# DavidLBick/espnet-1

Hardware: AMD Instinct MI355X
Metric: utterances/sec + step-time, Conformer-L T=1000 batch=32 @1/2/4/8 GPU (higher is better)
Workload: dtype bf16; 1 GPU; C3 Conformer-L (12x512, 8 heads, ff 2048, cnn 31) + 6-layer Transformer decoder, hybrid CTC/att 0.3/0.7, lsm 0.1, V=5000, T=1000 frames x 80, L=40, dropout 0.1, Adam+WarmupLR+clip 5; global_batch=32, seq_len=1000, parallelism=dp1

## Files before the change

espnet-1_amd/csrc/gemm_grouped.hip:

```cpp
#include "gemm_kern.h"

namespace {
struct GroupProbD {
  const bf16* A;
  const bf16* B;
  float* C;
  int lda, ldb, ldc;
  int M, N, K;
  int tiles_n, tile0;
  float beta;
};
constexpr int EA_GROUP_CHUNK = 60;
struct GroupChunk {
  int first, n;
  GroupProbD pr[EA_GROUP_CHUNK];
};
static_assert(sizeof(GroupChunk) <= 4000, "kernel argument space");

__global__ void group_upload(GroupChunk c, GroupProbD* table, int* map) {
  for (int i = threadIdx.x; i < c.n; i += blockDim.x) table[c.first + i] = c.pr[i];
  for (int i = 0; i < c.n; ++i) {
    const GroupProbD& d = c.pr[i];
    const int nt = ea_cdiv(d.M, 256) * d.tiles_n;
    for (int t = threadIdx.x; t < nt; t += blockDim.x) map[d.tile0 + t] = c.first + i;
  }
}

template <bool AK, bool BKM, int NS = 4>
__global__ __launch_bounds__(512, 1) void gemm_grouped(const GroupProbD* __restrict__ table,
                                                       const int* __restrict__ map, int ntiles, int xchunk) {
  using PC = PipeT<256, NS>;
  __shared__ __attribute__((aligned(1024))) char smem[PC::SMEM];
  const int nt = ntiles;
  const int bid = blockIdx.x;
  const int xcd = bid % 8;
  int t;
  if (xchunk > 0) {
    const int G = xchunk, full = nt / (8 * G) * (8 * G);
    const int j = bid / 8;
    t = bid < full ? ((j / G) * 8 + xcd) * G + j % G : bid;
  } else {
    const int q8 = nt / 8, r8 = nt % 8;
    t = (xcd < r8 ? xcd * (q8 + 1) : r8 * (q8 + 1) + (xcd - r8) * q8) + bid / 8;
  }
  const GroupProbD q = table[__builtin_amdgcn_readfirstlane(map[t])];
  const int lt = t - q.tile0;
  const int tm = lt / q.tiles_n, tn = lt - tm * q.tiles_n;
  const int m0 = tm * 256, n0 = tn * 256;
  GemmP p{};
  p.M = q.M; p.N = q.N; p.K = q.K;
  p.A = q.A; p.lda = q.lda;
  p.B = q.B; p.ldb = q.ldb;
  p.nh = 1; p.splitk = 1; p.kchunk = q.K;
  p.C = q.C; p.c_dtype = EA_F32; p.ldc = q.ldc;
  p.epi.kind = EA_EPI_STORE; p.epi.alpha = 1.f; p.epi.beta = q.beta; p.epi.post_scale = 1.f;
  p.epi.rscale = 1.f;
  p.vec_c = 1;
  p.vec8 = q.N % 8 == 0 && q.ldc % 8 == 0;
  const int lane = threadIdx.x & 63, w = threadIdx.x >> 6;
  const int wm = PC::wm(w), wn = PC::wn(w);
  f32x4 acc[8][4];
#pragma unroll
  for (int i = 0; i < 8; ++i)
#pragma unroll
    for (int j = 0; j < 4; ++j) acc[i][j] = (f32x4){0.f, 0.f, 0.f, 0.f};
  pipe_tile<AK, BKM, 0, 256, NS>(p, tile_ov(p), smem, q.A, q.B, m0, n0, 0, q.K, acc);
  const EpiK ek = make_epik(p);
  epi_wave<EA_EPI_STORE, 8, 4>(p, ek, smem, 0, 0, 0, m0 + wm, n0 + wn, lane, w, acc);
}

}

static int g_xcd_chunk = [] { const char* e = std::getenv("EA_GROUPED_XCD_CHUNK"); return e ? std::atoi(e) : 4; }();

extern "C" int ea_gemm_grouped_set_xcd_chunk(int chunk) {
  EA_ENTRY();
  EA_CHECK_ARG(chunk >= 0 && chunk <= 64);
  g_xcd_chunk = chunk;
  return 0;
}

static long grouped_ws_bytes(int n, long ntiles) { return (long)n * (long)sizeof(GroupProbD) + 4 * ntiles + 256; }

extern "C" int ea_gemm_grouped_ws_bytes(int n, long ntiles, long* bytes) {
  EA_CHECK_ARG(n >= 0 && ntiles >= 0 && bytes != nullptr);
  *bytes = grouped_ws_bytes(n, ntiles);
  return 0;
}

extern "C" int ea_gemm_grouped(int a_kmajor, int b_kmajor, int n, const ea_group_gemm* probs, void* ws,
                               long ws_bytes, void* stream) {
  EA_ENTRY();
  EA_CHECK_ARG(n >= 0 && (n == 0 || (probs != nullptr && ws != nullptr)));
  if (n == 0) return 0;
  hipStream_t st = (hipStream_t)stream;
  long ntiles = 0;
  for (int i = 0; i < n; ++i) {
    const ea_group_gemm& e = probs[i];
    EA_CHECK_ARG(e.M > 0 && e.N > 0 && e.K > 0 && e.A && e.B && e.C);
    EA_CHECK_ARG(e.lda % 8 == 0 && e.ldb % 8 == 0 && ((uintptr_t)e.A % 16) == 0 && ((uintptr_t)e.B % 16) == 0);
    EA_CHECK_ARG(e.N % 4 == 0 && e.ldc % 4 == 0 && ((uintptr_t)e.C % 16) == 0);
    EA_CHECK_ARG(e.ldc >= e.N && e.lda >= (a_kmajor ? e.K : e.M) && e.ldb >= (b_kmajor ? e.K : e.N));
    EA_CHECK_ARG(e.lda < (1L << 31) && e.ldb < (1L << 31) && e.ldc < (1L << 31));
    const double a_ext = 2.0 * ((a_kmajor ? (double)e.M : (double)e.K) * e.lda);
    const double b_ext = 2.0 * ((b_kmajor ? (double)e.N : (double)e.K) * e.ldb);
    EA_CHECK_ARG(a_ext < 4.0e9 && b_ext < 4.0e9);
    ntiles += (long)ea_cdiv(e.M, 256) * ea_cdiv(e.N, 256);
  }
  EA_CHECK_ARG(ntiles < (1L << 30) && grouped_ws_bytes(n, ntiles) <= ws_bytes);
  GroupProbD* table = (GroupProbD*)ws;
  int* map = (int*)((char*)ws + (long)n * sizeof(GroupProbD));
  GroupChunk c{};
  int tile0 = 0;
  for (int i = 0; i < n; ++i) {
    const ea_group_gemm& e = probs[i];
    GroupProbD& d = c.pr[c.n++];
    d.A = (const bf16*)e.A; d.B = (const bf16*)e.B; d.C = e.C;
    d.lda = (int)e.lda; d.ldb = (int)e.ldb; d.ldc = (int)e.ldc;
    d.M = e.M; d.N = e.N; d.K = e.K;
    d.tiles_n = ea_cdiv(e.N, 256);
    d.tile0 = tile0;
    d.beta = e.beta;
    tile0 += ea_cdiv(e.M, 256) * d.tiles_n;
    if (c.n == EA_GROUP_CHUNK || i == n - 1) {
      hipLaunchKernelGGL(group_upload, dim3(1), dim3(256), 0, st, c, table, map);
      EA_LAUNCH_CHECK();
      c.first += c.n;
      c.n = 0;
    }
  }
  const dim3 grid((unsigned)ntiles), block(512);
  if (a_kmajor && b_kmajor) hipLaunchKernelGGL((gemm_grouped<true, true>), grid, block, 0, st, table, map, (int)ntiles, g_xcd_chunk);
  else if (a_kmajor) hipLaunchKernelGGL((gemm_grouped<true, false>), grid, block, 0, st, table, map, (int)ntiles, g_xcd_chunk);
  else if (b_kmajor) hipLaunchKernelGGL((gemm_grouped<false, true>), grid, block, 0, st, table, map, (int)ntiles, g_xcd_chunk);
  else hipLaunchKernelGGL((gemm_grouped<false, false>), grid, block, 0, st, table, map, (int)ntiles, g_xcd_chunk);
  EA_LAUNCH_CHECK();
  return 0;
}
```

espnet-1_amd/csrc/gemm_kern.h:

```cpp
#pragma once
#include "common.h"


namespace eag {

constexpr int BM = 128, BN = 128, NT = 256;
constexpr int TILE_BYTES = 16384;

template <typename T> struct KCfg;
template <> struct KCfg<bf16> { static constexpr int KT = 64, KS = 32, E = 8, NKS = 2; };
template <> struct KCfg<float> { static constexpr int KT = 32, KS = 4, E = 4, NKS = 8; };

struct GemmP {
  int M, N, K;
  const void* A; long lda, sAb, sAh;
  const void* B; long ldb, sBb, sBh;
  int nh, splitk, kchunk;
  void* C; int c_dtype; long ldc, sCb, sCh;
  ea_epilogue epi;
  float* ws;
  int tiles_m, tiles_n;
  int vec_a, vec_b;
  int vec_c;
  int vec8;
// ... 864 lines not shown
        bk = (const char*)(B + ((long)(kh * 3 + kw) * p.g.C + c0) * p.g.C);
      }
    } else {
#pragma unroll
      for (int i = 0; i < ACH; ++i)
        __builtin_amdgcn_global_load_lds((__attribute__((address_space(1))) void*)(ak + aoff[i]),
                                         (__attribute__((address_space(3))) void*)(base + (i * NW + w) * 1024), 16, 0, 0);
    }
    if constexpr (MODE == EA_CONV_WGRAD) {
#pragma unroll
      for (int i = 0; i < BCH; ++i) {
        const int off = wpix[i] < p.g.P ? wbase[i] + ((wb[i] * wnI[i] + wt[i]) * wnJ[i] + wf[i]) * p.g.C
                                        : (int)p.g.zero + (lane & 63) * p.g.C + (wbase[i] % p.g.C);
        __builtin_amdgcn_global_load_lds((__attribute__((address_space(1))) void*)((const char*)B + (long)off * 2),
                                         (__attribute__((address_space(3))) void*)(base + A_BYTES + (i * NW + w) * 1024),
                                         16, 0, 0);
        wpix[i] += BK;
        wf[i] += dF;
        wt[i] += dT;
        if (wf[i] >= p.g.F2) { wf[i] -= p.g.F2; ++wt[i]; }
        while (wt[i] >= p.g.T2) { wt[i] -= p.g.T2; ++wb[i]; }
      }
    } else {
#pragma unroll
      for (int i = 0; i < BCH; ++i)
        __builtin_amdgcn_global_load_lds((__attribute__((address_space(1))) void*)(bk + boff[i]),
                                         (__attribute__((address_space(3))) void*)(base + A_BYTES + (i * NW + w) * 1024),
                                         16, 0, 0);
    }
  };

  f32x4 acc[MI][NJ];
#pragma unroll
  for (int i = 0; i < MI; ++i)
#pragma unroll
    for (int j = 0; j < NJ; ++j) acc[i][j] = (f32x4){0.f, 0.f, 0.f, 0.f};

  auto compute = [&](int stg) {
    const char* la = smem + stg * STAGE_BYTES;
    const char* lb = la + A_BYTES;
    if constexpr (DB) {
      bf16x8 fa0[MI], fb0[NJ], fa1[MI], fb1[NJ];
#pragma unroll
      for (int i = 0; i < MI; ++i) fa0[i] = frag_img<AK>(la, wm + i * 16, 0, lane);
#pragma unroll
      for (int j = 0; j < NJ; ++j) fb0[j] = frag_img<BKM>(lb, wn + j * 16, 0, lane);
#pragma unroll
      for (int i = 0; i < MI; ++i) fa1[i] = frag_img<AK>(la, wm + i * 16, 1, lane);
#pragma unroll
      for (int j = 0; j < NJ; ++j) fb1[j] = frag_img<BKM>(lb, wn + j * 16, 1, lane);
#pragma unroll
      for (int i = 0; i < MI; ++i)
#pragma unroll
        for (int j = 0; j < NJ; ++j)
          acc[i][j] = __builtin_amdgcn_mfma_f32_16x16x32_bf16(fa0[i], fb0[j], acc[i][j], 0, 0, 0);
#pragma unroll
      for (int i = 0; i < MI; ++i)
#pragma unroll
        for (int j = 0; j < NJ; ++j)
          acc[i][j] = __builtin_amdgcn_mfma_f32_16x16x32_bf16(fa1[i], fb1[j], acc[i][j], 0, 0, 0);
    } else {
#pragma unroll
      for (int ks = 0; ks < 2; ++ks) {
        bf16x8 fb[NJ];
#pragma unroll
        for (int j = 0; j < NJ; ++j) fb[j] = frag_img<BKM>(lb, wn + j * 16, ks, lane);
#pragma unroll
        for (int i = 0; i < MI; ++i) {
          const bf16x8 fa = frag_img<AK>(la, wm + i * 16, ks, lane);
#pragma unroll
          for (int j = 0; j < NJ; ++j)
            acc[i][j] = __builtin_amdgcn_mfma_f32_16x16x32_bf16(fa, fb[j], acc[i][j], 0, 0, 0);
        }
      }
    }
  };

  const int npre = min(STAGES - 1, nfull);
  for (int kt = 0; kt < npre; ++kt) issue(kt, kt);
  for (int kt = 0; kt < nfull; ++kt) {
    const int after = min(STAGES - 2, nfull - 1 - kt);
    if (after >= 2) wait_vmcnt<2 * GPT>();
    else if (after == 1) wait_vmcnt<GPT>();
    else wait_vmcnt<0>();
    lds_barrier();
    if (kt + STAGES - 1 < nfull) issue(kt + STAGES - 1, (kt + STAGES - 1) % STAGES);
    compute(kt % STAGES);
  }
  if (tail) {
    uint4 ra[BM_ * 8 / NTT], rb[BN_ * 8 / NTT];
    const int k0 = kbeg + nfull * BK;
    load_tile_r<AK, BM_, NTT>(A, p.lda, m0, p.M, k0, kend, ra);
    load_tile_r<BKM, BN_, NTT>(B, p.ldb, n0, p.N, k0, kend, rb);
    __syncthreads();
    char* base = smem + (nfull % STAGES) * STAGE_BYTES;
    store_tile_r<AK, BM_, NTT>(base, ra);
    store_tile_r<BKM, BN_, NTT>(base + A_BYTES, rb);
    __syncthreads();
    compute(nfull % STAGES);
  }

  __syncthreads();
  const EpiK ek = make_epik(p);
  switch (p.splitk > 1 ? EA_EPI_STORE : p.epi.kind) {
    case EA_EPI_STORE: epi_wave<EA_EPI_STORE, MI, NJ>(p, ek, smem, z, zb, zh, m0 + wm, n0 + wn, lane, w, acc, sk); break;
    case EA_EPI_ACT: epi_wave<EA_EPI_ACT, MI, NJ>(p, ek, smem, z, zb, zh, m0 + wm, n0 + wn, lane, w, acc, sk); break;
    case EA_EPI_RESID: epi_wave<EA_EPI_RESID, MI, NJ>(p, ek, smem, z, zb, zh, m0 + wm, n0 + wn, lane, w, acc, sk); break;
    default: epi_wave<EA_EPI_DACT, MI, NJ>(p, ek, smem, z, zb, zh, m0 + wm, n0 + wn, lane, w, acc, sk); break;
  }
  probe_end(p);
}

template <int OFF>
EA_DEV bf16x8 ds_read_b128_at(uint32_t addr) {
  bf16x8 v;
  asm volatile("ds_read_b128 %0, %1 offset:%2" : "=v"(v) : "v"(addr), "i"(OFF) : "memory");
  return v;
}

template <int S>
__global__ __launch_bounds__(512, 1) void gemm_k128(GemmP p) {
  constexpr int BK = 64, NTT = 512, NW = 8, MI = 4, NJ = 4;
  constexpr int A_BYTES = 128 * BK * 2, B_BYTES = 128 * BK * 2, STAGE = A_BYTES + B_BYTES;
  constexpr int ACH = A_BYTES / (NTT * 16), BCH = B_BYTES / (NTT * 16), G = ACH + BCH;
  constexpr int EPI_BYTES = 4 * 4 * 16 * EPI_LDT * 4;
  constexpr int HAND = EPI_BYTES;
  constexpr int SMEM = S * STAGE > HAND + 65536 ? S * STAGE : HAND + 65536;
  static_assert(S >= 3 && S <= 4, "ring depth");
  __shared__ __attribute__((aligned(1024))) char smem[SMEM];
  probe_start(p);

  const TileIdx ti = tile_index(p);
  const int m0 = ti.tm * 128, n0 = ti.tn * 128;
  const int z = ti.z, sk = ti.sk;
  const int zb = z / p.nh, zh = z % p.nh;
  const bf16* A = (const bf16*)p.A + zb * p.sAb + zh * p.sAh;
  const bf16* B = (const bf16*)p.B + zb * p.sBb + zh * p.sBh;
  const int kbeg = sk * p.kchunk;
  const int kend = min(p.K, kbeg + p.kchunk);
  const int nt = max(0, (kend - kbeg) / BK);
  const int tid = threadIdx.x, lane = tid & 63;
  const int w = __builtin_amdgcn_readfirstlane(tid >> 6);
  const int g = w >> 2, q = w & 3;
  const int wm = (q >> 1) * 64, wn = (q & 1) * 64;

  const __amdgpu_buffer_rsrc_t ra = __builtin_amdgcn_make_buffer_rsrc(
      (void*)(A + kbeg), (short)0, 0x7fffffff, 0x00020000);
  const __amdgpu_buffer_rsrc_t rb = __builtin_amdgcn_make_buffer_rsrc(
      (void*)(B + kbeg), (short)0, 0x7fffffff, 0x00020000);
  auto src = [&](long ld, int mn0, int MN, int ci) -> uint32_t {
    const int row = ci >> 3, c = (ci & 7) ^ swz_k(ci >> 3);
    return (uint32_t)(((long)min(mn0 + row, MN - 1) * ld + c * 8) * 2);
  };
  uint32_t aoff[ACH], boff[BCH];
#pragma unroll
  for (int i = 0; i < ACH; ++i) aoff[i] = src(p.lda, m0, p.M, (i * NW + w) * 64 + lane);
#pragma unroll
  for (int i = 0; i < BCH; ++i) boff[i] = src(p.ldb, n0, p.N, (i * NW + w) * 64 + lane);

  auto issue = [&](int t) {
    char* base = smem + (t % S) * STAGE;
    const int so = t * BK * 2;
#pragma unroll
    for (int i = 0; i < ACH; ++i)
      __builtin_amdgcn_raw_ptr_buffer_load_lds(ra, (__attribute__((address_space(3))) void*)(base + (i * NW + w) * 1024),
                                               16, aoff[i], so, 0, 0);
#pragma unroll
    for (int i = 0; i < BCH; ++i)
      __builtin_amdgcn_raw_ptr_buffer_load_lds(
          rb, (__attribute__((address_space(3))) void*)(base + A_BYTES + (i * NW + w) * 1024), 16, boff[i], so, 0, 0);
  };

  const int ch = g * 4 + (lane >> 4);
  const uint32_t lane_off = (uint32_t)((lane & 15) * 128 + ((ch ^ (((lane & 15) >> 1) & 7)) << 4));
  const uint32_t smem0 = (uint32_t)(uintptr_t)(const __attribute__((address_space(3))) char*)smem;
  const uint32_t a_off = smem0 + lane_off + wm * 128, b_off = smem0 + A_BYTES + lane_off + wn * 128;
  bf16x8 fa[MI], fb[NJ];
  auto rd = [&](int t) {
    const uint32_t sb = (uint32_t)((t % S) * STAGE);
    const uint32_t pa = a_off + sb, pb = b_off + sb;
    fa[0] = ds_read_b128_at<0>(pa);
    fa[1] = ds_read_b128_at<2048>(pa);
    fa[2] = ds_read_b128_at<4096>(pa);
    fa[3] = ds_read_b128_at<6144>(pa);
    fb[0] = ds_read_b128_at<0>(pb);
    fb[1] = ds_read_b128_at<2048>(pb);
    fb[2] = ds_read_b128_at<4096>(pb);
    fb[3] = ds_read_b128_at<6144>(pb);
  };

  f32x4 acc[MI][NJ];
#pragma unroll
  for (int i = 0; i < MI; ++i)
#pragma unroll
    for (int j = 0; j < NJ; ++j) acc[i][j] = (f32x4){0.f, 0.f, 0.f, 0.f};

  if (nt > 0) {
    const int npre = min(S - 1, nt);
    for (int t = 0; t < npre; ++t) issue(t);
    for (int t = 0; t < nt; ++t) {
      wait_newer<G, S - 2>(min(S - 2, nt - 1 - t));
      lds_barrier();
      if (t + S - 1 < nt) issue(t + S - 1);
      rd(t);
      asm volatile("s_waitcnt lgkmcnt(0)" ::: "memory");
      __builtin_amdgcn_sched_barrier(0);
      __builtin_amdgcn_s_setprio(1);
#pragma unroll
      for (int i = 0; i < MI; ++i)
#pragma unroll
        for (int j = 0; j < NJ; ++j) acc[i][j] = __builtin_amdgcn_mfma_f32_16x16x32_bf16(fa[i], fb[j], acc[i][j], 0, 0, 0);
      __builtin_amdgcn_s_setprio(0);
      __builtin_amdgcn_sched_barrier(0);
    }
  }
  __syncthreads();
  f32x4* hand = (f32x4*)(smem + HAND) + q * (MI * NJ * 64);
  if (g == 1) {
#pragma unroll
    for (int i = 0; i < MI; ++i)
#pragma unroll
      for (int j = 0; j < NJ; ++j) hand[(i * NJ + j) * 64 + lane] = acc[i][j];
  }
  __syncthreads();
  if (g == 0) {
#pragma unroll
    for (int i = 0; i < MI; ++i)
#pragma unroll
      for (int j = 0; j < NJ; ++j) acc[i][j] += hand[(i * NJ + j) * 64 + lane];
    const EpiK ek = make_epik(p);
    switch (p.splitk > 1 ? EA_EPI_STORE : p.epi.kind) {
      case EA_EPI_STORE: epi_wave<EA_EPI_STORE, MI, NJ>(p, ek, smem, z, zb, zh, m0 + wm, n0 + wn, lane, q, acc, sk); break;
      case EA_EPI_ACT: epi_wave<EA_EPI_ACT, MI, NJ>(p, ek, smem, z, zb, zh, m0 + wm, n0 + wn, lane, q, acc, sk); break;
      case EA_EPI_RESID: epi_wave<EA_EPI_RESID, MI, NJ>(p, ek, smem, z, zb, zh, m0 + wm, n0 + wn, lane, q, acc, sk); break;
      default: epi_wave<EA_EPI_DACT, MI, NJ>(p, ek, smem, z, zb, zh, m0 + wm, n0 + wn, lane, q, acc, sk); break;
    }
  }
  probe_end(p);
}

EA_DEV int swz32(int r) { return ((r >> 3) & 1) << 1; }

template <bool KMAJ>
EA_DEV int img32_off(int c) {
  if (KMAJ) {
    const int row = c >> 2, ch = c & 3;
    return row * 64 + ((ch ^ swz32(row)) << 4);
  } else {
    const int pnl = c >> 9, cj = c & 511, k = cj >> 4, ch = cj & 15;
    return pnl * 8192 + k * 256 + ((ch ^ swz_mn_bf16(k)) << 4);
  }
}

EA_DEV s16x4 tr_read_asm(const char* p) {
  s16x4 v;
  const uint32_t a = (uint32_t)(uintptr_t)(const __attribute__((address_space(3))) char*)p;
  asm volatile("ds_read_b64_tr_b16 %0, %1" : "=v"(v) : "v"(a) : "memory");
  return v;
}

template <bool KMAJ>
EA_DEV bf16x8 frag32(const char* img, int r, int lane) {
  if (KMAJ) {
    const int row = r + (lane & 15), ch = lane >> 4;
    return *(const bf16x8*)(img + row * 64 + ((ch ^ swz32(row)) << 4));
  }
  const char* pnl = img + (r >> 7) * 8192;
  const int i = lane & 15, q = i >> 2, pp = i & 3;
  const int col = (r & 127) + 4 * pp;
  const int ch = col >> 3, within = (col & 7) * 2;
  union { bf16x8 v; s16x4 h[2]; } out;
#pragma unroll
  for (int half = 0; half < 2; ++half) {
    const int row = 8 * (lane >> 4) + 4 * half + q;
    out.h[half] = tr_read_asm(pnl + row * 256 + ((ch ^ swz_mn_bf16(row)) << 4) + within);
  }
  return out.v;
}

template <int BT, int NS = 4>
struct PipeT {
  static constexpr int BK = 32, NSLOT = NS, NW = 8, NTT = 512;
  static constexpr int A_BYTES = BT * BK * 2, B_BYTES = BT * BK * 2, SLOT = A_BYTES + B_BYTES;
  static constexpr int RING = NSLOT * SLOT;
  static constexpr int MI = BT == 256 ? 8 : 2;
  static constexpr int EPI_BYTES = NW * (MI < 4 ? MI : 4) * 16 * EPI_LDT * 4;
  static constexpr int SMEM = RING > EPI_BYTES ? RING : EPI_BYTES;
  static constexpr int ACH = A_BYTES / (NTT * 16), BCH = B_BYTES / (NTT * 16);
  static constexpr int G = ACH + BCH;
  static constexpr int OCC = BT == 256 ? 1 : 2;
  static_assert(BT == 256 || BT == 128, "pipe tiles");
  static_assert(NS == 4, "ring depth: 4 slots (5- and 6/8-slot rings measured slower, round 3/4)");
  EA_DEV static int wm(int w) { return BT == 256 ? (w >> 2) * 128 : (w >> 2) * 64 + ((w >> 1) & 1) * 32; }
  EA_DEV static int wn(int w) { return BT == 256 ? (w & 3) * 64 : (w & 1) * 64; }
};

struct TileOv {
  int M, a, e;
  float* w1part;
  const uint8_t* w1pos;
};
EA_DEV TileOv tile_ov(const GemmP& p) { return TileOv{p.M, p.g.a, p.g.e, p.w1part, p.w1pos}; }

template <bool AK, bool BKM, int MODE = 0, int BT = 256, int NS = 4>
EA_DEV void pipe_tile(const GemmP& p, const TileOv& ov, char* smem, const bf16* A, const bf16* B, int m0, int n0, int kbeg,
                      int kend, f32x4 (&acc)[PipeT<BT, NS>::MI][4]) {
  static_assert(MODE == 0 || (MODE == EA_CONV_FWD && AK && BKM) || (MODE == EA_CONV_DGRAD && AK) ||
                (MODE == EA_CONV_WGRAD && !AK && !BKM), "conv gather layouts");
  static_assert(MODE == 0 || BT == 256, "conv gathers run on 256-wide tiles");
  using PC = PipeT<BT, NS>;
  constexpr int BK = PC::BK, NSLOT = PC::NSLOT, NW = PC::NW, NTT = PC::NTT, MI = PC::MI;
  constexpr int A_BYTES = PC::A_BYTES, B_BYTES = PC::B_BYTES, SLOT = PC::SLOT;
  constexpr int ACH = PC::ACH, BCH = PC::BCH, G = PC::G;
  const int tid = threadIdx.x, lane = tid & 63, w = tid >> 6;
  const int wm = PC::wm(w), wn = PC::wn(w);
  const int nsl = max(0, (kend - kbeg) / BK);
  const bool tail = kbeg + nsl * BK < kend;


  auto src = [&](long ld, int mn0, int MN, bool kmaj, int ci) -> uint32_t {
    if (kmaj) {
      const int row = ci >> 2, c = (ci & 3) ^ swz32(ci >> 2);
      return (uint32_t)(((long)min(mn0 + row, MN - 1) * ld + c * 8) * 2);
    }
    const int pnl = ci >> 9, cj = ci & 511, k = cj >> 4, c = (cj & 15) ^ swz_mn_bf16(k);
    return (uint32_t)(((long)k * ld + min((long)(mn0 + pnl * 128 + c * 8), (long)((MN - 1) & ~7))) * 2);
  };
  const char* abase = (const char*)(A + (AK ? (long)kbeg : (long)kbeg * p.lda));
  const char* bbase = (const char*)(B + (BKM ? (long)kbeg : (long)kbeg * p.ldb));
  uint32_t aoff[ACH], boff[BCH];
#pragma unroll
  for (int i = 0; i < ACH; ++i) aoff[i] = src(p.lda, m0, ov.M, AK, (i * NW + w) * 64 + lane);
#pragma unroll
  for (int i = 0; i < BCH; ++i) boff[i] = src(p.ldb, n0, p.N, BKM, (i * NW + w) * 64 + lane);
  const long astep = (AK ? BK : (long)BK * p.lda) * 2;
  const long bstep = (BKM ? BK : (long)BK * p.ldb) * 2;

  const int ksl0 = kbeg / BK;
  const int CS = MODE ? p.g.C / BK : 1;
  int gb[ACH], gt[ACH], gf[ACH], cur[ACH];
  if constexpr (MODE == EA_CONV_FWD || MODE == EA_CONV_DGRAD) {
    const int n2 = MODE == EA_CONV_FWD ? p.g.T2 : p.g.nI[ov.a];
    const int n3 = MODE == EA_CONV_FWD ? p.g.F2 : p.g.nJ[ov.e];
#pragma unroll
    for (int i = 0; i < ACH; ++i) {
      const int m = min(m0 + ((((i * NW + w) * 64 + lane)) >> 2), ov.M - 1);
      const int bt = fdiv(m, n3);
      gf[i] = m - bt * n3;
      gb[i] = fdiv(bt, n2);
      gt[i] = bt - gb[i] * n2;
      cur[i] = 0;
    }
  }
  auto a_tap = [&](int q) {
#pragma unroll
    for (int i = 0; i < ACH; ++i) {
      const int ci = (i * NW + w) * 64 + lane;
      const int cc = ((ci & 3) ^ swz32(ci >> 2)) * 8;
      if constexpr (MODE == EA_CONV_FWD) {
        const int kh = q / 3, kw = q - 3 * (q / 3);
        cur[i] = (int)x1p_row(p.g, gb[i], gt[i], gf[i], kh, kw) + cc;
      } else {
        int kh, kw;
        dgrad_tap2(ov.a, ov.e, q, kh, kw);
        const int t2 = gt[i] - (kh >> 1), f2 = gf[i] - (kw >> 1);
        cur[i] = (t2 >= 0 && t2 < p.g.T2 && f2 >= 0 && f2 < p.g.F2)
                     ? ((gb[i] * p.g.T2 + t2) * p.g.F2 + f2) * p.g.C + cc
                     : (int)p.g.zero + ((ci >> 2) & 63) * p.g.C + cc;
      }
    }
  };
  int wb[BCH], wt[BCH], wf[BCH], wpix[BCH], wbase[BCH], wnI[BCH], wnJ[BCH];
  if constexpr (MODE == EA_CONV_WGRAD) {
#pragma unroll
    for (int i = 0; i < BCH; ++i) {
      const int ci = (i * NW + w) * 64 + lane;
      const int pnl = ci >> 9, cj = ci & 511, k = cj >> 4, c = (cj & 15) ^ swz_mn_bf16(k);
      const int n = min(n0 + pnl * 128 + c * 8, p.N - 8);
      const int tap = n / p.g.C, cin = n - tap * p.g.C;
      const int kh = tap / 3, kw = tap - 3 * kh, a = kh & 1, e = kw & 1;
      wnI[i] = p.g.nI[a];
      wnJ[i] = p.g.nJ[e];
      wbase[i] = (int)p.g.plane[a * 2 + e] + ((kh >> 1) * wnJ[i] + (kw >> 1)) * p.g.C + cin;
      const int pix = ksl0 * BK + k;
      wpix[i] = pix;
      const int bt = fdiv(pix, p.g.F2);
      wf[i] = pix - bt * p.g.F2;
      wb[i] = fdiv(bt, p.g.T2);
      wt[i] = bt - wb[i] * p.g.T2;
    }
  }
  const int dF = BK % max(p.g.F2, 1), dT = BK / max(p.g.F2, 1);

  auto issue = [&](int sl) {
    char* base = smem + (sl % NSLOT) * SLOT;
    const char* ak = abase + sl * astep;
    const char* bk = bbase + sl * bstep;
    if constexpr (MODE == EA_CONV_FWD || MODE == EA_CONV_DGRAD) {
      const int ks = ksl0 + sl;
      int q, c0;
      bool newtap;
      if constexpr (MODE == EA_CONV_FWD) {
        const int cb = ks / 18, r = ks - 18 * cb;
        q = r >> 1;
        c0 = cb * 64 + (r & 1) * BK;
        newtap = (r & 1) == 0;
      } else {
        q = ks / CS;
        c0 = (ks - q * CS) * BK;
        newtap = c0 == 0;
      }
      if (newtap || sl == 0) a_tap(q);
#pragma unroll
      for (int i = 0; i < ACH; ++i)
        __builtin_amdgcn_global_load_lds((__attribute__((address_space(1))) void*)((const char*)A + (long)(cur[i] + c0) * 2),
                                         (__attribute__((address_space(3))) void*)(base + (i * NW + w) * 1024), 16, 0, 0);
      if constexpr (MODE == EA_CONV_DGRAD) {
        int kh, kw;
        dgrad_tap2(ov.a, ov.e, q, kh, kw);
        bk = BKM ? (const char*)(B + (long)(kh * 3 + kw) * p.g.C + c0)
                 : (const char*)(B + ((long)(kh * 3 + kw) * p.g.C + c0) * p.g.C);
      }
    } else {
#pragma unroll
      for (int i = 0; i < ACH; ++i)
        __builtin_amdgcn_global_load_lds((__attribute__((address_space(1))) void*)(ak + aoff[i]),
                                         (__attribute__((address_space(3))) void*)(base + (i * NW + w) * 1024), 16, 0, 0);
    }
    if constexpr (MODE == EA_CONV_WGRAD) {
#pragma unroll
      for (int i = 0; i < BCH; ++i) {
        const int off = wpix[i] < p.g.P ? wbase[i] + ((wb[i] * wnI[i] + wt[i]) * wnJ[i] + wf[i]) * p.g.C
                                        : (int)p.g.zero + (lane & 63) * p.g.C + (wbase[i] % p.g.C);
        __builtin_amdgcn_global_load_lds((__attribute__((address_space(1))) void*)((const char*)B + (long)off * 2),
                                         (__attribute__((address_space(3))) void*)(base + A_BYTES + (i * NW + w) * 1024),
                                         16, 0, 0);
        wpix[i] += BK;
        wf[i] += dF;
        wt[i] += dT;
        if (wf[i] >= p.g.F2) { wf[i] -= p.g.F2; ++wt[i]; }
        while (wt[i] >= p.g.T2) { wt[i] -= p.g.T2; ++wb[i]; }
      }
    } else {
#pragma unroll
      for (int i = 0; i < BCH; ++i)
        __builtin_amdgcn_global_load_lds((__attribute__((address_space(1))) void*)(bk + boff[i]),
                                         (__attribute__((address_space(3))) void*)(base + A_BYTES + (i * NW + w) * 1024),
                                         16, 0, 0);
    }
  };

  auto rd_b = [&](int sl, bf16x8 (&fb)[4]) {
    const char* lb = smem + (sl % NSLOT) * SLOT + A_BYTES;
#pragma unroll
    for (int j = 0; j < 4; ++j) fb[j] = frag32<BKM>(lb, wn + j * 16, lane);
  };
  auto rd_a = [&](int sl, bf16x8 (&fa)[MI]) {
    const char* la = smem + (sl % NSLOT) * SLOT;
#pragma unroll
    for (int i = 0; i < MI; ++i) fa[i] = frag32<AK>(la, wm + i * 16, lane);
  };

  const int g1 = w >> 2;
  const int npre = min(NSLOT - 1, nsl);
  for (int sl = 0; sl < npre; ++sl) issue(sl);
  wait_newer<G, NSLOT - 2>(npre - 1);
  lds_barrier();
  if (g1) lds_barrier();
  bf16x8 fa[MI], fb[4];
  for (int sl = 0; sl < nsl; ++sl) {
    __builtin_amdgcn_sched_barrier(0);
    rd_b(sl, fb);
    rd_a(sl, fa);
    if (sl + NSLOT - 1 < nsl) issue(sl + NSLOT - 1);
    wait_newer<G, NSLOT - 2>(min(NSLOT - 2, nsl - 2 - sl));
    if (!AK || !BKM) {
      asm volatile("s_waitcnt lgkmcnt(0)" ::: "memory");
      __builtin_amdgcn_sched_barrier(0);
    }
#pragma unroll
    for (int i = 0; i < MI; ++i) asm volatile("" ::"v"(fa[i]));
#pragma unroll
    for (int j = 0; j < 4; ++j) asm volatile("" ::"v"(fb[j]));
    __builtin_amdgcn_sched_barrier(0);
    lds_barrier();
    __builtin_amdgcn_sched_barrier(0);
    __builtin_amdgcn_s_setprio(1);
#pragma unroll
    for (int i = 0; i < MI; ++i)
#pragma unroll
      for (int j = 0; j < 4; ++j)
        acc[i][j] = __builtin_amdgcn_mfma_f32_16x16x32_bf16(fa[i], fb[j], acc[i][j], 0, 0, 0);
    __builtin_amdgcn_s_setprio(0);
    __builtin_amdgcn_sched_barrier(0);
    lds_barrier();
  }
  if (!g1) lds_barrier();
  if (tail) {
    constexpr int NCH = (A_BYTES + B_BYTES) / 16 / NTT;
    uint4 v[NCH];
    const int k0 = kbeg + nsl * BK;
#pragma unroll
    for (int i = 0; i < NCH; ++i) {
      const int c = tid + NTT * i;
      const bool isa = c < A_BYTES / 16;
      const int cc = isa ? c : c - A_BYTES / 16;
      const bool km = isa ? AK : BKM;
      const bf16* base = isa ? A : B;
      const long ld = isa ? p.lda : p.ldb;
      const int MN = isa ? ov.M : p.N, mn0 = isa ? m0 : n0;
      int mn, k;
      if (km) { mn = mn0 + (cc >> 2); k = k0 + (cc & 3) * 8; }
      else    { const int cj = cc & 511; k = k0 + (cj >> 4); mn = mn0 + (cc >> 9) * 128 + (cj & 15) * 8; }
      union { uint4 u; bf16 e[8]; } tv;
#pragma unroll
      for (int e = 0; e < 8; ++e) {
        const bool ok = km ? (mn < MN && k + e < kend) : (k < kend && mn + e < MN);
        tv.e[e] = ok ? (km ? base[(long)mn * ld + k + e] : base[(long)k * ld + mn + e]) : (bf16)0.f;
      }
      v[i] = tv.u;
    }
    __syncthreads();
#pragma unroll
    for (int i = 0; i < NCH; ++i) {
      const int c = tid + NTT * i;
      const bool isa = c < A_BYTES / 16;
      const int cc = isa ? c : c - A_BYTES / 16;
      const int off = isa ? (AK ? img32_off<true>(cc) : img32_off<false>(cc))
                          : A_BYTES + (BKM ? img32_off<true>(cc) : img32_off<false>(cc));
      *(uint4*)(smem + off) = v[i];
    }
    __syncthreads();
    rd_b(0, fb);
    rd_a(0, fa);
    asm volatile("s_waitcnt lgkmcnt(0)" ::: "memory");
    __builtin_amdgcn_sched_barrier(0);
#pragma unroll
    for (int i = 0; i < MI; ++i)
#pragma unroll
      for (int j = 0; j < 4; ++j)
        acc[i][j] = __builtin_amdgcn_mfma_f32_16x16x32_bf16(fa[i], fb[j], acc[i][j], 0, 0, 0);
  }

  __syncthreads();
}

constexpr int W1_TS = 264;
constexpr int W1_IMG = 16 * W1_TS * 2;
constexpr int W1_SMEM = PipeT<256>::SMEM + 2 * W1_IMG;

EA_DEV void w1_load_x(const GemmP& p, const TileOv& ov, int m0, float (&xv)[5]) {
  const int tid = threadIdx.x;
  const int row = tid >> 1, t0 = (tid & 1) * 5;
  const int m = m0 + row;
#pragma unroll
  for (int u = 0; u < 5; ++u) xv[u] = 0.f;
  if (m < ov.M) {
    const int a = ov.a, e = ov.e, nI = p.g.nI[a], nJ = p.g.nJ[e];
    const int bi = fdiv(m, nJ), j = m - bi * nJ;
    const int b = fdiv(bi, nI), i = bi - b * nI;
    const float* xp = p.w1x + ((long)b * p.w1T + 2 * (2 * i + a)) * p.w1F + 2 * (2 * j + e);
#pragma unroll
    for (int u = 0; u < 5; ++u) {
      const int t = t0 + u;
      xv[u] = t < 9 ? xp[(t / 3) * p.w1F + t % 3] : 1.f;
    }
  }
}
EA_DEV void w1_stage_x(char* xs, const float (&xv)[5]) {
  bf16* hi = (bf16*)xs;
  bf16* lo = (bf16*)(xs + W1_IMG);
  const int tid = threadIdx.x;
  const int row = tid >> 1, t0 = (tid & 1) * 5;
#pragma unroll
  for (int u = 0; u < 5; ++u) {
    const bf16 h = (bf16)xv[u];
    hi[(t0 + u) * W1_TS + row] = h;
    lo[(t0 + u) * W1_TS + row] = (bf16)(xv[u] - (float)h);
  }
  for (int q = tid; q < 6 * 256; q += 512) {
    const int t = 10 + (q >> 8), r = q & 255;
    hi[t * W1_TS + r] = (bf16)0.f;
    lo[t * W1_TS + r] = (bf16)0.f;
  }
}

EA_DEV void w1_epilogue(const GemmP& p, const TileOv& ov, char* smem, int m0, int n0, int wm, int wn, int lane, int w, int tm,
                        const f32x4 (&acc)[8][4]) {
  float* t = (float*)smem + w * 64 * EPI_LDT;
  const char* xh = smem + PipeT<256>::SMEM;
  const char* xl = xh + W1_IMG;
  const int g = lane >> 4, lc = lane & 15, rq = g * 4;
  const int lc8 = (lane & 7) * 8, rl = lane >> 3;
  const bf16* aux = (const bf16*)p.epi.aux;
  f32x4 out[4];
#pragma unroll
  for (int cb = 0; cb < 4; ++cb) out[cb] = (f32x4){0.f, 0.f, 0.f, 0.f};
#pragma unroll
  for (int ch = 0; ch < 2; ++ch) {
    if (ch) {
      __builtin_amdgcn_wave_barrier();
      asm volatile("" ::: "memory");
    }
#pragma unroll
    for (int i = 0; i < 4; ++i)
#pragma unroll
      for (int j = 0; j < 4; ++j)
#pragma unroll
        for (int rr = 0; rr < 4; ++rr) t[(i * 16 + rq + rr) * EPI_LDT + j * 16 + lc] = acc[ch * 4 + i][j][rr];
    __builtin_amdgcn_wave_barrier();
    asm volatile("" ::: "memory");
    const int rb = m0 + wm + ch * 64, col = n0 + wn + lc8;
    if (ov.w1pos) {
      uint32_t mb[8];
#pragma unroll
      for (int it = 0; it < 8; ++it)
        mb[it] = ov.w1pos[(long)min(rb + it * 8 + rl, ov.M - 1) * (p.N >> 3) + min(col, p.N - 8) / 8];
#pragma unroll
      for (int it = 0; it < 8; ++it) {
        float* tr = t + (it * 8 + rl) * EPI_LDT + lc8;
        float4 f0 = *(const float4*)tr, f1 = *(const float4*)(tr + 4);
        float v[8] = {f0.x, f0.y, f0.z, f0.w, f1.x, f1.y, f1.z, f1.w};
#pragma unroll
        for (int c = 0; c < 8; ++c) v[c] = (float)(bf16)(((mb[it] >> c) & 1u) ? v[c] : 0.f);
        *(float4*)tr = make_float4(v[0], v[1], v[2], v[3]);
        *(float4*)(tr + 4) = make_float4(v[4], v[5], v[6], v[7]);
      }
    } else {
#pragma unroll
      for (int h0 = 0; h0 < 8; h0 += 4) {
        float o[4][8];
#pragma unroll
        for (int it = 0; it < 4; ++it)
          ld8(aux, (long)min(rb + (h0 + it) * 8 + rl, ov.M - 1) * p.epi.ldaux + col, EA_BF16, o[it]);
#pragma unroll
        for (int it = 0; it < 4; ++it) {
          float* tr = t + ((h0 + it) * 8 + rl) * EPI_LDT + lc8;
          float4 f0 = *(const float4*)tr, f1 = *(const float4*)(tr + 4);
          float v[8] = {f0.x, f0.y, f0.z, f0.w, f1.x, f1.y, f1.z, f1.w};
#pragma unroll
          for (int c = 0; c < 8; ++c) v[c] = (float)(bf16)(o[it][c] > 0.f ? v[c] : 0.f);
          *(float4*)tr = make_float4(v[0], v[1], v[2], v[3]);
          *(float4*)(tr + 4) = make_float4(v[4], v[5], v[6], v[7]);
        }
      }
    }
    __builtin_amdgcn_wave_barrier();
    asm volatile("" ::: "memory");
#pragma unroll
    for (int ks = 0; ks < 2; ++ks) {
      const int pl = wm + ch * 64 + 32 * ks + 8 * g;
      const bf16x8 bh = *(const bf16x8*)(xh + (lc * W1_TS + pl) * 2);
      const bf16x8 bl = *(const bf16x8*)(xl + (lc * W1_TS + pl) * 2);
#pragma unroll
      for (int cb = 0; cb < 4; ++cb) {
        union { bf16x8 v; bf16 e[8]; } af;
#pragma unroll
        for (int e = 0; e < 8; ++e) af.e[e] = (bf16)t[(32 * ks + 8 * g + e) * EPI_LDT + 16 * cb + lc];
        out[cb] = __builtin_amdgcn_mfma_f32_16x16x32_bf16(af.v, bh, out[cb], 0, 0, 0);
        out[cb] = __builtin_amdgcn_mfma_f32_16x16x32_bf16(af.v, bl, out[cb], 0, 0, 0);
      }
    }
  }
  __syncthreads();
  float* cmb = (float*)smem;
  if (w >= 4) {
#pragma unroll
    for (int cb = 0; cb < 4; ++cb)
#pragma unroll
      for (int r = 0; r < 4; ++r) cmb[((w - 4) * 64 + 16 * cb + 4 * g + r) * 16 + lc] = out[cb][r];
  }
  __syncthreads();
  if (w < 4 && lc < 10) {
    float* prow = ov.w1part + (long)tm * 10 * p.N + (long)lc * p.N;
#pragma unroll
    for (int cb = 0; cb < 4; ++cb)
#pragma unroll
      for (int r = 0; r < 4; ++r) {
        const int co = n0 + wn + 16 * cb + 4 * g + r;
        if (co < p.N) prow[co] = out[cb][r] + cmb[(w * 64 + 16 * cb + 4 * g + r) * 16 + lc];
      }
  }
}

EA_DEV bool dgrad_class_item(const GemmP& p, TileOv& ov, TileIdx& ti) {
  const int bid = blockIdx.x, x = bid & 7, sq = bid >> 3, tn_n = p.tiles_n;
  const int item = ((sq / tn_n) * 8 + x) * tn_n + sq % tn_n;
  if (item >= p.cls_item0[p.ncls]) return false;
  int c = 0;
#pragma unroll
  for (int k = 1; k < 4; ++k) c += (k < p.ncls && item >= p.cls_item0[k]) ? 1 : 0;
  const int local = item - p.cls_item0[c];
  ov.M = p.cls_M[c];
  ov.a = p.cls_a[c];
  ov.e = p.cls_e[c];
  ov.w1part = p.w1part + (long)p.cls_tile0[c] * 10 * p.N;
  ov.w1pos = p.w1pos + p.cls_pos[c];
  ti.tm = local / tn_n;
  ti.tn = local % tn_n;
  ti.z = 0;
  ti.sk = p.cls_K[c];
  return true;
}

template <bool AK, bool BKM, int MODE, int BT, int NS>
EA_DEV void pipe_body(const GemmP& p, const TileOv& ov, const TileIdx& ti, char* smem) {
  using PC = PipeT<BT, NS>;
  constexpr int MI = PC::MI;
  const int tm = ti.tm, m0 = ti.tm * BT, n0 = ti.tn * BT;
  const bool cls = MODE == EA_CONV_DGRAD && p.ncls;
  const int z = ti.z, sk = cls ? 0 : ti.sk;
  const int zb = z / p.nh, zh = z % p.nh;
  const bf16* A = (const bf16*)p.A + zb * p.sAb + zh * p.sAh;
  const bf16* B = (const bf16*)p.B + zb * p.sBb + zh * p.sBh;
  const int kbeg = sk * p.kchunk;
  const int kend = cls ? ti.sk : min(p.K, kbeg + p.kchunk);
  const int tid = threadIdx.x, lane = tid & 63, w = tid >> 6;
  const int wm = PC::wm(w), wn = PC::wn(w);
  f32x4 acc[MI][4];
#pragma unroll
  for (int i = 0; i < MI; ++i)
#pragma unroll
    for (int j = 0; j < 4; ++j) acc[i][j] = (f32x4){0.f, 0.f, 0.f, 0.f};
  diag_stamp(p, 0);
  float w1x[5];
  if constexpr (MODE == EA_CONV_DGRAD) {
    if (p.w1part) w1_load_x(p, ov, m0, w1x);
  }
  pipe_tile<AK, BKM, MODE, BT, NS>(p, ov, smem, A, B, m0, n0, kbeg, kend, acc);
  diag_stamp(p, 1);
  if constexpr (MODE == EA_CONV_DGRAD) {
    if (p.w1part) {
      w1_stage_x(smem + PC::SMEM, w1x);
      __syncthreads();
      w1_epilogue(p, ov, smem, m0, n0, wm, wn, lane, w, tm, acc);
      return;
    }
  }
  const EpiK ek = make_epik(p);
  switch (p.splitk > 1 ? EA_EPI_STORE : p.epi.kind) {
    case EA_EPI_STORE: epi_wave<EA_EPI_STORE, MI, 4>(p, ek, smem, z, zb, zh, m0 + wm, n0 + wn, lane, w, acc, sk); break;
    case EA_EPI_ACT: epi_wave<EA_EPI_ACT, MI, 4>(p, ek, smem, z, zb, zh, m0 + wm, n0 + wn, lane, w, acc, sk); break;
    case EA_EPI_RESID: epi_wave<EA_EPI_RESID, MI, 4>(p, ek, smem, z, zb, zh, m0 + wm, n0 + wn, lane, w, acc, sk); break;
    default: epi_wave<EA_EPI_DACT, MI, 4>(p, ek, smem, z, zb, zh, m0 + wm, n0 + wn, lane, w, acc, sk); break;
  }
  if (p.diag) {
    __syncthreads();
    diag_stamp(p, 2);
  }
}

template <bool AK, bool BKM, int MODE = 0, int BT = 256, int NS = 4>
__global__ __launch_bounds__(512, (PipeT<BT, NS>::OCC)) void gemm_pipe(GemmP p) {
  using PC = PipeT<BT, NS>;
  __shared__ __attribute__((aligned(1024))) char smem[MODE == EA_CONV_DGRAD ? W1_SMEM : PC::SMEM];
  probe_start(p);
  TileOv ov = tile_ov(p);
  TileIdx ti;
  bool run = true;
  if (MODE == EA_CONV_DGRAD && p.ncls) run = dgrad_class_item(p, ov, ti);
  else ti = tile_index(p);
  if (run) pipe_body<AK, BKM, MODE, BT, NS>(p, ov, ti, smem);
  probe_end(p);
}

}
```

espnet-1_amd/espnet_amd/deferred.py:

```python
from __future__ import annotations

import contextlib
import ctypes
import os

import torch

from ._lib import ColsumProb, GroupGemm, ReduceProb, dt, lib
from .streams import WGRAD, on_side, scratch, stream

GRAD_READY = None

DEFER_WGRAD = os.environ.get("EA_DEFER_WGRAD", "1") != "0"
DEFER_BUDGET = int(float(os.environ.get("EA_DEFER_BUDGET_MB", "8192")) * 2 ** 20)


def _nbytes(t):
    return t.numel() * t.element_size()


class WgradQueue:

    def __init__(self):
        self.active = False
        self.items = []
        self.posts = []
        self.pending = 0
        self.side_events = []

    def add(self, dy, x, dw, *, M, N, K, lda, ldb, ldc, beta, post=None) -> bool:
        if not (dy.dtype == torch.bfloat16 and x.dtype == torch.bfloat16 and dw.dtype == torch.float32):
            return False
        if (lda % 8 or ldb % 8 or dy.data_ptr() % 16 or x.data_ptr() % 16 or N % 4 or ldc % 4
                or dw.data_ptr() % 16 or M <= 0 or N <= 0 or K <= 0):
            return False
        if 2.0 * K * lda >= 4.0e9 or 2.0 * K * ldb >= 4.0e9:
            return False
        lo = dw.data_ptr()
        hi = lo + ((M - 1) * ldc + N) * 4
        if any(lo < it[-1] and it[-2] < hi for it in self.items):
            self.flush()
        if on_side():
            ev = torch.cuda.Event()
            ev.record()
            self.side_events.append(ev)
        self.items.append((K, dy, x, dw, M, N, lda, ldb, ldc, beta, lo, hi))
        if post is not None:
            self.posts.append(post)
        self.pending += _nbytes(dy) + _nbytes(x)
        if self.pending > DEFER_BUDGET:
            self.flush()
        return True

    def flush(self):
        if not self.items:
            return
        if self.side_events:
            if not on_side():
                cur = torch.cuda.current_stream()
                for ev in self.side_events:
                    cur.wait_event(ev)
            self.side_events = []
        items = sorted(self.items, key=lambda t: -t[0])
        posts = self.posts
        self.items = []
        self.posts = []
        self.pending = 0
        n = len(items)
        cur = torch.cuda.current_stream()
        for it in items:
            for t in it[1:4]:
                t.record_stream(cur)
        arr = (GroupGemm * n)()
        ntiles = 0
        for i, (K, dy, x, dw, M, N, lda, ldb, ldc, beta, _, _) in enumerate(items):
            arr[i] = GroupGemm(dy.data_ptr(), x.data_ptr(), dw.data_ptr(), lda, ldb, ldc, M, N, K, beta)
            ntiles += ((M + 255) // 256) * ((N + 255) // 256)
        nbytes = ctypes.c_long(0)
        lib.ea_gemm_grouped_ws_bytes(n, ntiles, ctypes.addressof(nbytes))
        ws = scratch("ggemm", nbytes.value, items[0][1].device)
        lib.ea_gemm_grouped(0, 0, n, ctypes.addressof(arr), ws.data_ptr(), ws.numel(), stream())
        for post in posts:
            post()

    def tensors(self):
        return [t for it in self.items for t in (it[1], it[2])]


WGRAD_Q = WgradQueue()

DEFER_REDUCE = os.environ.get("EA_DEFER_REDUCE", "1") != "0"


class ReduceQueue:

    def __init__(self):
        self.active = False
        self.colsums = []
        self.reduces = []
        self.spans = []
        self.pending = 0

    def _account(self, t):
        self.pending += _nbytes(t)
        if self.pending > DEFER_BUDGET:
            self.flush()

    def _claim(self, out, n):
        lo = out.data_ptr()
        hi = lo + 4 * n
        if any(lo < h and l_ < hi for l_, h in self.spans):
            self.flush()
        self.spans.append((lo, hi))

    def add_colsum(self, x, rows, n, ld, out, accumulate) -> bool:
        if x.dtype not in (torch.bfloat16, torch.float32) or out.dtype != torch.float32 or not out.is_contiguous():
            return False
        if rows <= 0 or n % 4 or ld % 4 or x.data_ptr() % (8 if x.dtype == torch.bfloat16 else 16):
            return False
        self._claim(out, n)
        self.colsums.append((x, rows, n, ld, out, accumulate))
        self._account(x)
        return True

    def add_reduce(self, part, nparts, n, stride, out, accumulate=True):
        self._claim(out, n)
        self.reduces.append((part, nparts, n, stride, out, accumulate))
        self._account(part)

    def tensors(self):
        return [c[0] for c in self.colsums] + [r[0] for r in self.reduces]

    def flush(self):
        if not self.colsums and not self.reduces:
            return
        colsums, reduces = self.colsums, list(self.reduces)
        self.colsums, self.reduces, self.spans = [], [], []
        self.pending = 0
        cur = torch.cuda.current_stream()
        for t in [c[0] for c in colsums] + [r[0] for r in reduces]:
            t.record_stream(cur)
        dev = (colsums[0][0] if colsums else reduces[0][0]).device
        cb, rb = ctypes.c_long(0), ctypes.c_long(0)
        if colsums:
            rpps = [max(32, (c[1] + 127) // 128) for c in colsums]
            nrbs = [(c[1] + r - 1) // r for c, r in zip(colsums, rpps)]
            part = torch.empty(sum(nrb * c[2] for c, nrb in zip(colsums, nrbs)), dtype=torch.float32, device=dev)
            arr = (ColsumProb * len(colsums))()
            off = 0
            for i, ((x, rows, n, ld, out, acc), rpp, nrb) in enumerate(zip(colsums, rpps, nrbs)):
                arr[i] = ColsumProb(x.data_ptr(), part.data_ptr() + 4 * off, ld, rows, n, dt(x), rpp)
                reduces.append((part, nrb, n, n, out, acc, off))
                off += nrb * n
            lib.ea_grouped_table_bytes(len(colsums), ctypes.addressof(cb), ctypes.addressof(rb))
            ws = scratch("colsum", cb.value, dev)
            lib.ea_colsum_grouped(len(colsums), ctypes.addressof(arr), ws.data_ptr(), ws.numel(), stream())
        arr = (ReduceProb * len(reduces))()
        for i, r in enumerate(reduces):
            part, nparts, n, stride, out, acc = r[:6]
            off = r[6] if len(r) > 6 else 0
            arr[i] = ReduceProb(part.data_ptr() + 4 * off, out.data_ptr(), stride, nparts, n, int(acc))
        lib.ea_grouped_table_bytes(len(reduces), ctypes.addressof(cb), ctypes.addressof(rb))
        ws = scratch("reduce", rb.value, dev)
        lib.ea_reduce_grouped(len(reduces), ctypes.addressof(arr), ws.data_ptr(), ws.numel(), stream())


REDUCE_Q = ReduceQueue()


def wgrad(*tensors, after=None, launches=False):
    if not launches and WGRAD_Q.active and REDUCE_Q.active:
        return contextlib.nullcontext()
    return WGRAD(*tensors, after=after)


def fork_event():
    return None if GRAD_READY is not None else WGRAD.fork_point()


def join_wgrad():
    WGRAD.join()
    WGRAD_Q.side_events = []


def grad_ready(bound):
    if GRAD_READY is not None:
        GRAD_READY(bound.prefix)
        return
    join_wgrad()


def _side_flush_ok():
    return GRAD_READY is None and WGRAD.enabled and torch.cuda.is_available()


def flush_wgrad_side(after=None):
    if WGRAD_Q.active and WGRAD_Q.items and _side_flush_ok():
        with WGRAD(*WGRAD_Q.tensors(), after=after):
            WGRAD_Q.flush()


def flush_deferred():
    WGRAD_Q.flush()
    REDUCE_Q.flush()


def deferred_tensors():
    return WGRAD_Q.tensors() + REDUCE_Q.tensors()


class deferred_wgrad:

    def __enter__(self):
        self.prev = (WGRAD_Q.active, REDUCE_Q.active)
        WGRAD_Q.active = DEFER_WGRAD
        REDUCE_Q.active = DEFER_REDUCE
        return WGRAD_Q

    def __exit__(self, *exc):
        WGRAD_Q.active, REDUCE_Q.active = self.prev
        if exc[0] is None:
            if _side_flush_ok():
                with WGRAD(*REDUCE_Q.tensors()):
                    REDUCE_Q.flush()
                WGRAD_Q.flush()
            else:
                flush_deferred()
            if GRAD_READY is None:
                join_wgrad()
        else:
            WGRAD_Q.items, WGRAD_Q.posts = [], []
            REDUCE_Q.colsums, REDUCE_Q.reduces, REDUCE_Q.spans = [], [], []
        return False
```

espnet-1_amd/espnet_amd/hip_ops.py:

```python
from __future__ import annotations

import ctypes
import os
import sys
import types
import weakref

import torch

from . import deferred, streams
from ._lib import ACT_NONE, EPI_STORE, Epilogue, HipError, dt, lib
from .deferred import (REDUCE_Q, WGRAD_Q, deferred_tensors, deferred_wgrad, flush_deferred,
                       flush_wgrad_side, fork_event, grad_ready, join_wgrad, wgrad)
from .streams import aux, join_aux, mark_aux_fork, on_side, scratch, stream, take_aux_fork

_MOVED = {**dict.fromkeys(("DEBUG_DELAY_NS", "DEBUG_SERIAL", "OVERLAP_CTC_BWD"), streams),
          **dict.fromkeys(("GRAD_READY", "DEFER_WGRAD", "DEFER_REDUCE", "DEFER_BUDGET"), deferred)}


class _Ops(types.ModuleType):
    def __getattr__(self, name):
        if name in _MOVED:
            return getattr(_MOVED[name], name)
        raise AttributeError(f"module {self.__name__!r} has no attribute {name!r}")

    def __setattr__(self, name, value):
        if name in _MOVED:
            setattr(_MOVED[name], name, value)
        else:
            super().__setattr__(name, value)


sys.modules[__name__].__class__ = _Ops


class KernelProbe:

    TICK_MS = 1e-5

    def __init__(self, names, device=None):
        self.names = set(names)
        dev = device or torch.device("cuda", torch.cuda.current_device())
        self.slots = {n: torch.zeros(4, dtype=torch.int64, device=dev) for n in names}
        self.active = True

    def begin(self, name):
        if self.active and name in self.names:
            s = self.slots[name].data_ptr()
            lib.ea_probe_begin(s, stream())
            lib.ea_gemm_set_probe(s)

    def end(self, name):
        if self.active and name in self.names:
            lib.ea_gemm_set_probe(None)
            lib.ea_probe_end(self.slots[name].data_ptr(), stream())

    def reset(self):
        for t in self.slots.values():
            t.zero_()

    def mean_ms(self, name):
        tot, cnt = (int(x) for x in self.slots[name][2:4].tolist())
        return (tot / cnt * self.TICK_MS if cnt else float("nan")), cnt


class EventProbe:

    def __init__(self, names):
        self.names = set(names)
        self.pairs = {n: [] for n in names}
        self.active = True

    def begin(self, name):
        if self.active and name in self.names:
            ev = torch.cuda.Event(enable_timing=True)
            ev.record(torch.cuda.current_stream())
            self.pairs[name].append([ev, None])

    def end(self, name):
        if self.active and name in self.names:
            ev = torch.cuda.Event(enable_timing=True)
            ev.record(torch.cuda.current_stream())
            self.pairs[name][-1][1] = ev

    def reset(self):
        for v in self.pairs.values():
            v.clear()

    def mean_ms(self, name):
        torch.cuda.synchronize()
        ts = [a.elapsed_time(b) for a, b in self.pairs[name] if b is not None]
        return (sum(ts) / len(ts) if ts else float("nan")), len(ts)


PROBE = None


def ptr(t):
    return None if t is None else t.data_ptr()


SPLITK_WS = 1 << 25


def splitk_ws(device) -> torch.Tensor:
    return scratch("splitk", SPLITK_WS, device)


def f32_ws(device, numel=1 << 22):
    w = scratch("f32", numel, device)
    return w.data_ptr(), w.numel()


def make_epi(kind=EPI_STORE, *, alpha=1.0, beta=0.0, bias=None, post_scale=1.0, act=ACT_NONE,
             aux=None, resid=None, rscale=1.0, drop_p=0.0, seed=0):
    e = Epilogue()
    e.kind = kind
    e.act = act
    e.alpha = alpha
    e.beta = beta
    e.post_scale = post_scale
    e.rscale = rscale
    e.drop_p = drop_p
    e.seed = seed & 0xFFFFFFFFFFFFFFFF
    e.bias = ptr(bias)
    if aux is not None:
        e.aux = aux.data_ptr()
        e.aux_dtype = dt(aux)
        e.ldaux = aux.stride(-2)
    if resid is not None:
        e.resid = resid.data_ptr()
        e.ldr = resid.stride(-2)
    return e


MN_TAIL_COPIES = 0


def _mn_tail_guard(X, MN, K, ld, s, batch, nh):
    global MN_TAIL_COPIES
    if X.dtype != torch.bfloat16 or MN % 8 == 0 or K <= 0:
        return X
    esz = X.element_size()
    total = X.untyped_storage().nbytes() // esz
    off = X.storage_offset()
    last = off + (batch - 1) * s[0] + (nh - 1) * s[1] + (K - 1) * ld
    if last + (MN + 7) // 8 * 8 <= total:
        return X
    span = last + MN - off
    buf = torch.empty(span + 8, dtype=X.dtype, device=X.device)
    buf[:span].copy_(torch.as_strided(X, (span,), (1,), off))
    buf[span:].zero_()
    MN_TAIL_COPIES += 1
    return buf


def gemm(A, B, C, *, M, N, K, a_kmajor, b_kmajor, lda, ldb, ldc,
         batch=1, nh=1, sA=(0, 0), sB=(0, 0), sC=(0, 0), epi: Epilogue = None, splitk=True):
    if A.dtype != B.dtype:
        raise HipError(f"gemm operand dtypes differ: {A.dtype} vs {B.dtype}")
    if epi is None:
        epi = make_epi()
    if not a_kmajor:
        A = _mn_tail_guard(A, M, K, lda, sA, batch, nh)
    if not b_kmajor:
        B = _mn_tail_guard(B, N, K, ldb, sB, batch, nh)
    ws = splitk_ws(A.device) if splitk else None
    lib.ea_gemm(dt(A), int(a_kmajor), int(b_kmajor), M, N, K,
                A.data_ptr(), lda, sA[0], sA[1],
                B.data_ptr(), ldb, sB[0], sB[1],
                batch, nh,
                C.data_ptr(), dt(C), ldc, sC[0], sC[1],
                ctypes.byref(epi), ptr(ws), 0 if ws is None else ws.numel(), stream())
    return C


def _rows(x):
    if x.stride(-1) != 1:
        raise HipError("inner dimension must be contiguous")
    K = x.shape[-1]
    rows = x.numel() // K if K else 0
    ld = x.stride(-2) if x.dim() >= 2 else K
    if x.dim() > 2:
        exp = ld
        for d in range(x.dim() - 2, 0, -1):
            exp *= x.shape[d]
            if x.shape[d - 1] > 1 and x.stride(d - 1) != exp:
                raise HipError("leading dims do not collapse onto one row stride")
    return rows, K, ld


def linear(x, w, out, *, epi: Epilogue = None):
    M, K, lda = _rows(x)
    N = w.shape[0]
    _, _, ldc = _rows(out)
    return gemm(x, w, out, M=M, N=N, K=K, a_kmajor=1, b_kmajor=1, lda=lda, ldb=w.stride(0),
                ldc=ldc, epi=epi)


WT_SHADOW = os.environ.get("EA_WT_SHADOW", "1") != "0"
WT_MAX_KIN = 512
TSHADOWS = {}


class TransposedShadow:
    def __init__(self, shadow):
        self.shadow = shadow
        self.items = {}
        self.tiles = self.probs = None
        self.ntiles = 0
        self.frozen = False

    def _rebuild(self):
        probs, tiles = [], []
        for pi, ((off, R, C), dst) in enumerate(self.items.items()):
            probs.append((off, dst.data_ptr(), R | (C << 32)))
            tiles += [(pi, tr, tc, 0) for tr in range((R + 63) // 64) for tc in range((C + 63) // 64)]
        dev = self.shadow.device
        self.probs = torch.tensor(probs, dtype=torch.int64).to(dev)
        self.tiles = torch.tensor(tiles, dtype=torch.int32).to(dev)
        self.ntiles = len(tiles)

    def get(self, w):
        off = (w.data_ptr() - self.shadow.data_ptr()) // w.element_size()
        key = (off, int(w.shape[0]), int(w.shape[1]))
        wt = self.items.get(key)
        if wt is None:
            if self.frozen or torch.cuda.is_current_stream_capturing():
                return None
            wt = torch.empty(key[2], key[1], dtype=w.dtype, device=w.device)
            self.items[key] = wt
            self._rebuild()
            self.refresh()
        return wt

    def refresh(self):
        if torch.cuda.is_current_stream_capturing():
            self.frozen = True
        if self.ntiles:
            lib.ea_transpose_bf16_grouped(self.ntiles, self.tiles.data_ptr(), self.probs.data_ptr(),
                                          self.shadow.data_ptr(), stream())


def attach_transposed_shadow(shadow):
    if not WT_SHADOW or shadow is None or shadow.dtype != torch.bfloat16:
        return None
    ts = TransposedShadow(shadow)
    TSHADOWS[shadow.untyped_storage().data_ptr()] = weakref.ref(ts)
    return ts


def _transposed(w):
    if not TSHADOWS or w.dtype != torch.bfloat16 or w.dim() != 2 or w.shape[1] > WT_MAX_KIN:
        return None
    if w.stride(1) != 1 or w.stride(0) != w.shape[1] or w.shape[0] % 8 or w.shape[1] % 8:
        return None
    ref = TSHADOWS.get(w.untyped_storage().data_ptr())
    ts = None if ref is None else ref()
    if ts is None or ts.shadow.untyped_storage().data_ptr() != w.untyped_storage().data_ptr():
        return None
    return ts.get(w)


def linear_dx(dy, w, out, *, epi: Epilogue = None):
    M, N, lda = _rows(dy)
    K = w.shape[1]
    _, _, ldc = _rows(out)
    wt = _transposed(w)
    if wt is not None:
        return gemm(dy, wt, out, M=M, N=K, K=N, a_kmajor=1, b_kmajor=1, lda=lda, ldb=wt.stride(0),
                    ldc=ldc, epi=epi)
    return gemm(dy, w, out, M=M, N=K, K=N, a_kmajor=1, b_kmajor=0, lda=lda, ldb=w.stride(0),
                ldc=ldc, epi=epi)


def linear_dw(dy, x, dw, *, accumulate=False, post=None):
    R, N, lddy = _rows(dy)
    R2, K, ldx = _rows(x)
    if R != R2:
        raise HipError("row mismatch in linear_dw")
    beta = 1.0 if accumulate else 0.0
    if WGRAD_Q.active and WGRAD_Q.add(dy, x, dw, M=N, N=K, K=R, lda=lddy, ldb=ldx, ldc=dw.stride(0), beta=beta,
                                      post=post):
        return dw
    gemm(dy, x, dw, M=N, N=K, K=R, a_kmajor=0, b_kmajor=0, lda=lddy, ldb=ldx,
         ldc=dw.stride(0), epi=make_epi(beta=beta))
    if post is not None:
        post()
    return dw


def layernorm_fwd(x, gamma, beta, y, mean, rstd, eps=1e-12):
    rows, d, ldx = _rows(x)
    lib.ea_layernorm_fwd(rows, d, x.data_ptr(), ldx, gamma.data_ptr(), beta.data_ptr(), eps,
                         y.data_ptr(), dt(y), y.stride(-2) if y.dim() > 1 else d,
                         mean.data_ptr(), rstd.data_ptr(), stream())


def linear_ln(x, gamma, beta, w, out, *, epi=None, eps=1e-12):
    rows, K, ldx = _rows(x)
    N = w.shape[0]
    if epi is None:
        epi = make_epi()
    lib.ea_gemm_ln(rows, N, K, x.data_ptr(), ldx, gamma.data_ptr(), beta.data_ptr(), ctypes.c_float(eps),
                   w.data_ptr(), w.stride(0), out.data_ptr(), dt(out), out.stride(0), ctypes.byref(epi), stream())
    return out


def layernorm_bwd(dy, x, gamma, mean, rstd, dx, dgamma, dbeta, accumulate=True, drop=None):
    rows, d, ldx = _rows(x)
    _, _, lddy = _rows(dy)
    _, _, lddx = _rows(dx)
    if drop is not None:
        y, ysc, yp, yseed = drop[:4]
        ycol = drop[4] if len(drop) > 4 else None
        _, _, ldy = _rows(y)
        dargs = (y.data_ptr(), dt(y), ldy, float(ysc), float(yp), yseed & 0xFFFFFFFFFFFFFFFF,
                 0 if ycol is None else ycol.data_ptr())
    if REDUCE_Q.active and rows > 0 and dbeta.data_ptr() == dgamma.data_ptr() + 4 * d:
        vec8 = (d % 8 == 0 and d <= 1024 and lddy % 8 == 0 and ldx % 4 == 0 and lddx % 4 == 0
                and x.data_ptr() % 16 == 0 and dy.data_ptr() % 16 == 0 and dx.data_ptr() % 16 == 0
                and gamma.data_ptr() % 16 == 0)
        nparts_max = (rows + 15) // 16 if vec8 else max((rows + 15) // 16, 128)
        part = torch.empty(nparts_max * (3 if drop is not None else 2) * d, dtype=torch.float32, device=x.device)
        np_ = ctypes.c_int(0)
        if drop is not None:
            yparts = ctypes.c_int(0)
            lib.ea_layernorm_bwd_partials_drop(rows, d, dy.data_ptr(), dt(dy), lddy, x.data_ptr(), ldx,
                                               gamma.data_ptr(), mean.data_ptr(), rstd.data_ptr(), dx.data_ptr(),
                                               lddx, int(accumulate), part.data_ptr(), part.numel(),
                                               ctypes.addressof(np_), *dargs, ctypes.addressof(yparts), stream())
            if yparts.value:
                npv = np_.value
                REDUCE_Q.add_reduce(part[npv * 2 * d:], npv, d, d, ycol, accumulate=True)
        else:
            lib.ea_layernorm_bwd_partials(rows, d, dy.data_ptr(), dt(dy), lddy, x.data_ptr(), ldx, gamma.data_ptr(),
                                          mean.data_ptr(), rstd.data_ptr(), dx.data_ptr(), lddx, int(accumulate),
                                          part.data_ptr(), part.numel(), ctypes.addressof(np_), stream())
        REDUCE_Q.add_reduce(part, np_.value, 2 * d, 2 * d, dgamma, accumulate=True)
        return
    w, n = f32_ws(x.device, max(1 << 22, 1024 * d))
    if drop is not None:
        lib.ea_layernorm_bwd_drop(rows, d, dy.data_ptr(), dt(dy), lddy, x.data_ptr(), ldx, gamma.data_ptr(),
                                  mean.data_ptr(), rstd.data_ptr(), dx.data_ptr(), lddx, int(accumulate),
                                  dgamma.data_ptr(), dbeta.data_ptr(), 1, w, n, *dargs, stream())
        return
    lib.ea_layernorm_bwd(rows, d, dy.data_ptr(), dt(dy), lddy, x.data_ptr(), ldx, gamma.data_ptr(),
                         mean.data_ptr(), rstd.data_ptr(), dx.data_ptr(), lddx, int(accumulate),
                         dgamma.data_ptr(), dbeta.data_ptr(), 1, w, n, stream())


def reduce_rows(part, nparts, n, stride, out, accumulate=True):
    if REDUCE_Q.active:
        REDUCE_Q.add_reduce(part, nparts, n, stride, out, accumulate)
        return
    lib.ea_reduce_partials(nparts, n, part.data_ptr(), stride, out.data_ptr(), int(accumulate), stream())


def colsum(x, out, accumulate=True, defer=True):
    rows, n, ld = _rows(x)
    if defer and REDUCE_Q.active and REDUCE_Q.add_colsum(x, rows, n, ld, out, accumulate):
        return
    w, wn = f32_ws(x.device)
    lib.ea_colsum(rows, n, x.data_ptr(), dt(x), ld, out.data_ptr(), int(accumulate), w, wn, stream())


def batchnorm_fwd(y, gamma, beta, mean, rstd, run_mean, run_var, nbt, z, training, act,
                  eps=1e-5, momentum=0.1):
    rows, C, _ = _rows(y)
    w, wn = f32_ws(y.device, (min(rows // 16 + 1, 256) + 2) * 2 * C)
    lib.ea_batchnorm_fwd(rows, C, y.data_ptr(), gamma.data_ptr(), beta.data_ptr(), eps, momentum,
                         int(training), mean.data_ptr(), rstd.data_ptr(), ptr(run_mean), ptr(run_var),
                         ptr(nbt), act, z.data_ptr(), dt(z), w, wn, stream())


def batchnorm_bwd(dz, y, mean, rstd, gamma, beta, act, dy, dgamma, dbeta):
    rows, C, _ = _rows(y)
    w, wn = f32_ws(y.device, (min(rows // 16 + 1, 256) + 2) * 2 * C)
    lib.ea_batchnorm_bwd(rows, C, dz.data_ptr(), dt(dz), y.data_ptr(), mean.data_ptr(), rstd.data_ptr(),
                         gamma.data_ptr(), beta.data_ptr(), act, dy.data_ptr(), dgamma.data_ptr(),
                         dbeta.data_ptr(), 1, w, wn, stream())


def scale_dropout(x, y, scale=1.0, p=0.0, seed=0):
    rows, cols, ldx = _rows(x)
    _, _, ldy = _rows(y)
    lib.ea_scale_dropout(rows, cols, x.data_ptr(), dt(x), ldx, y.data_ptr(), dt(y), ldy,
                         float(scale), float(p), seed & 0xFFFFFFFFFFFFFFFF, stream())
    return y


def scale_dropout_colsum(x, y, out, scale=1.0, p=0.0, seed=0, accumulate=True):
    scale_dropout(x, y, scale=scale, p=p, seed=seed)
    with wgrad(y):
        colsum(y, out, accumulate=accumulate)
    return y


def cast(x, dtype):
    if x.dtype == dtype:
        return x
    y = torch.empty(x.shape, dtype=dtype, device=x.device)
    scale_dropout(x.reshape(-1, x.shape[-1]), y.view(-1, y.shape[-1]))
    return y


def permute3(src, dst, A, Bd, Cd, accumulate=False):
    lib.ea_permute3(A, Bd, Cd, src.data_ptr(), dt(src), dst.data_ptr(), dt(dst), int(accumulate), stream())
```

espnet-1_amd/espnet_amd/layers/conformer.py:

```python
from __future__ import annotations

import ctypes
import os

import torch
from torch import nn

from .common import (ACT_SWISH, EPI_ACT, EPI_DACT, EPI_RESID, EPI_STORE, F32, Bound, attn_bwd, attn_dmask, dbd_layout,
                     attn_fused_bwd, attn_fwd, empty, fused_attn_ok, lib, ln_bwd, ln_fwd, math, ops, rup,
                     site_seed, dv_buf, drop_arg, site_dv, REL_LATEST, REL_LEGACY)



FUSE_DW_GLU = os.environ.get("EA_FUSE_DW_GLU", "1") != "0"
GLU_IN_CONV = os.environ.get("EA_GLU_IN_CONV", "1") != "0"
BN_STATS_IN_CONV = os.environ.get("EA_BN_STATS_IN_CONV", "1") != "0"


def _glu_in_conv(K, g2, d):
    return (GLU_IN_CONV and FUSE_DW_GLU and K in (3, 5, 7, 15, 31)
            and g2.dtype == torch.bfloat16 and d % 4 == 0 and g2.data_ptr() % 8 == 0 and torch.cuda.is_available())

class PositionwiseFeedForward(nn.Module):

    def __init__(self, idim, hidden_units, dropout_rate, activation="swish"):
        super().__init__()
        self.w_1 = nn.Linear(idim, hidden_units)
        self.w_2 = nn.Linear(hidden_units, idim)
        self.dropout_rate = dropout_rate
        self.activation = activation


class MultiHeadedAttention(nn.Module):

    def __init__(self, n_head, n_feat, dropout_rate):
        super().__init__()
        assert n_feat % n_head == 0
        self.d_k = n_feat // n_head
        self.h = n_head
        self.linear_q = nn.Linear(n_feat, n_feat)
        self.linear_k = nn.Linear(n_feat, n_feat)
        self.linear_v = nn.Linear(n_feat, n_feat)
        self.linear_out = nn.Linear(n_feat, n_feat)
        self.dropout_rate = dropout_rate


class RelPositionMultiHeadedAttention(MultiHeadedAttention):

    def __init__(self, n_head, n_feat, dropout_rate, zero_triu=False, legacy=False):
        super().__init__(n_head, n_feat, dropout_rate)
        if zero_triu:
            raise NotImplementedError("zero_triu=True is not on the ASR hot path")
        self.rel_mode = REL_LEGACY if legacy else REL_LATEST
        self.linear_pos = nn.Linear(n_feat, n_feat, bias=False)
        self.pos_bias_u = nn.Parameter(torch.Tensor(self.h, self.d_k))
        self.pos_bias_v = nn.Parameter(torch.Tensor(self.h, self.d_k))
        torch.nn.init.xavier_uniform_(self.pos_bias_u)
        torch.nn.init.xavier_uniform_(self.pos_bias_v)


class ConvolutionModule(nn.Module):

    def __init__(self, channels, kernel_size, activation="swish", bias=True):
        super().__init__()
        assert (kernel_size - 1) % 2 == 0
        self.pointwise_conv1 = nn.Conv1d(channels, 2 * channels, 1, 1, 0, bias=bias)
        self.depthwise_conv = nn.Conv1d(channels, channels, kernel_size, 1, (kernel_size - 1) // 2,
                                        groups=channels, bias=bias)
        self.norm = nn.BatchNorm1d(channels)
        self.pointwise_conv2 = nn.Conv1d(channels, channels, 1, 1, 0, bias=bias)
        self.kernel_size = kernel_size


def LayerNorm(n):
    return nn.LayerNorm(n, eps=1e-12)


class EncoderLayer(nn.Module):

    def __init__(self, size, self_attn, feed_forward, feed_forward_macaron, conv_module,
                 dropout_rate, normalize_before=True, concat_after=False, stochastic_depth_rate=0.0):
        super().__init__()
        if not normalize_before or concat_after or stochastic_depth_rate > 0:
            raise NotImplementedError("only normalize_before=True, concat_after=False, "
                                      "stochastic_depth_rate=0 (the ASR recipes) are implemented")
        if conv_module is None:
            raise NotImplementedError("use_cnn_module=False is not on the hot path")
        self.self_attn = self_attn
        self.feed_forward = feed_forward
        self.feed_forward_macaron = feed_forward_macaron
        self.conv_module = conv_module
        self.norm_ff = LayerNorm(size)
        self.norm_mha = LayerNorm(size)
        if feed_forward_macaron is not None:
            self.norm_ff_macaron = LayerNorm(size)
            self.ff_scale = 0.5
        else:
            self.ff_scale = 1.0
        self.norm_conv = LayerNorm(size)
        self.norm_final = LayerNorm(size)
        self.size = size
        self.dropout_rate = dropout_rate
        self.layer_idx = 0
        self._b = None

    def bind(self, arena, prefix, cd):
        self._b = Bound(arena, prefix, cd)

    @staticmethod
    def arena_groups(prefix):
        a = prefix + "self_attn."
        return [[a + "linear_q.weight", a + "linear_k.weight", a + "linear_v.weight"],
                [a + "linear_q.bias", a + "linear_k.bias", a + "linear_v.bias"]]

    def forward(self, x, pos_emb, olens, seed):
        return ConformerBlockFn.apply(x, pos_emb, olens, self, seed, self.training)


def _ffn_fwd(L, b, x_in, pre, ln_name, p, seed_in, seed_out):
    cd = b.cd
    N, d = x_in.shape
    Fh = L.feed_forward.w_1.out_features
    xn, mu, rs = ln_fwd(x_in, b, ln_name, cd)
    h = empty(N, Fh, dtype=cd, device=x_in.device)
    a = empty(N, Fh, dtype=cd, device=x_in.device)
    ops.linear(xn, b.w(pre + ".w_1.weight"), a,
               epi=ops.make_epi(EPI_ACT, bias=b.f(pre + ".w_1.bias"), act=ACT_SWISH, aux=h,
                                drop_p=p, seed=seed_in))
    x_out = empty(N, d, device=x_in.device)
    ops.linear(a, b.w(pre + ".w_2.weight"), x_out,
               epi=ops.make_epi(EPI_RESID, bias=b.f(pre + ".w_2.bias"), resid=x_in,
                                rscale=L.ff_scale, drop_p=p, seed=seed_out))
    return x_out, (xn, mu, rs, h, a)


def _ffn_bwd(L, b, dx, x_in, saved, pre, ln_name, p, seed_in, seed_out, dv_in=None, next_drop=None):
    cd = b.cd
    xn, mu, rs, h, a = saved
    N, d = dx.shape
    dv = site_dv(dx, dv_in, b.g(pre + ".w_2.bias"), L.ff_scale, p, seed_out, cd)
    with ops.wgrad(dv, a):
        ops.linear_dw(dv, a, b.g(pre + ".w_2.weight"), accumulate=True)
    dh = empty(*h.shape, dtype=cd, device=dx.device)
    ops.linear_dx(dv, b.w(pre + ".w_2.weight"), dh,
                  epi=ops.make_epi(EPI_DACT, act=ACT_SWISH, aux=h, drop_p=p, seed=seed_in))
    with ops.wgrad(dh, xn):
        ops.colsum(dh, b.g(pre + ".w_1.bias"))
        ops.linear_dw(dh, xn, b.g(pre + ".w_1.weight"), accumulate=True)
    dxn = empty(N, d, dtype=cd, device=dx.device)
    ops.linear_dx(dh, b.w(pre + ".w_1.weight"), dxn)
    ln_bwd(dxn, x_in, b, ln_name, mu, rs, dx, accumulate=True, drop=next_drop)


class ConformerBlockFn(torch.autograd.Function):
    @staticmethod
    def forward(ctx, x, pos, olens, L: EncoderLayer, seed, training):
        b = L._b
        cd = b.cd
        B, T, d = x.shape
        N = B * T
        dev = x.device
        H = L.self_attn.h
        dk = d // H
        P2 = 2 * T - 1
        p = L.dropout_rate if training else 0.0
        pa = L.self_attn.dropout_rate if training else 0.0
        li = L.layer_idx
        sd = lambda s: site_seed(seed, li, s)
        x0 = x.reshape(N, d)
        x1, s_ff1 = _ffn_fwd(L, b, x0, "feed_forward_macaron", "norm_ff_macaron", p, sd(1), sd(2))
        xn2, mu2, rs2 = ln_fwd(x1, b, "norm_mha", cd)
        A = "self_attn."
        qkv = empty(N, 3 * d, dtype=cd, device=dev)
        ops.linear(xn2, b.w(A + "linear_q.weight", A + "linear_k.weight", A + "linear_v.weight",
                            shape=(3 * d, d)), qkv,
                   epi=ops.make_epi(bias=b.f(A + "linear_q.bias", A + "linear_k.bias",
                                             A + "linear_v.bias", shape=(3 * d,))))
        mode = L.self_attn.rel_mode
        fused = fused_attn_ok(cd, dk, T, T)
        if mode == REL_LEGACY and fused:
            shift = dbd_layout(T)[0]
            pp_full = empty(shift + P2, d, dtype=cd, device=dev)
            pp_full[:shift].zero_()
            pp = pp_full[shift:]
        else:
            pp_full = None
            pp = empty(P2, d, dtype=cd, device=dev)
        if mode == REL_LEGACY:
            assert pos.shape[0] == T
            pT = empty(T, d, dtype=cd, device=dev)
            ops.linear(pos, b.w(A + "linear_pos.weight"), pT)
            lib.ea_legacy_pext(T, d, pT.data_ptr(), d, pp.data_ptr(), d, ops.dt(pp), ops.stream())
        else:
            ops.linear(pos, b.w(A + "linear_pos.weight"), pp)
        scale = 1.0 / math.sqrt(dk)
        if fused:
            O = empty(N, d, dtype=cd, device=dev)
            lse = empty(B * H * T, device=dev)
            dmask, ldm = attn_dmask(B * H * T, T, pa, dev)
            lib.ea_attn_fused_fwd2_mode(B, H, T, T, dk, qkv.data_ptr(), 3 * d, qkv[:, d:].data_ptr(), 3 * d,
                                        qkv[:, 2 * d:].data_ptr(), 3 * d, b.f(A + "pos_bias_u").data_ptr(),
                                        b.f(A + "pos_bias_v").data_ptr(), pp.data_ptr(), d, olens.data_ptr(), 0,
                                        scale, float(pa), sd(3), O.data_ptr(), d, lse.data_ptr(), ops.ptr(dmask), ldm,
                                        mode, ops.stream())
            ldT = 0
            s_core = ("fused", lse, dmask, ldm, pp_full)
        else:
            qu = empty(N, d, dtype=cd, device=dev)
            qv = empty(N, d, dtype=cd, device=dev)
            lib.ea_add_pos_bias(N, H, dk, qkv.data_ptr(), 3 * d, b.f(A + "pos_bias_u").data_ptr(),
                                b.f(A + "pos_bias_v").data_ptr(), qu.data_ptr(), qv.data_ptr(),
                                ops.dt(qu), ops.stream())
            ldbd = rup(P2, 8)
            bd = empty(H * B * T * ldbd, device=dev)
            ops.gemm(qv, pp, bd, M=T, N=P2, K=dk, a_kmajor=1, b_kmajor=1, lda=d, ldb=d, ldc=ldbd,
                     batch=B, nh=H, sA=(T * d, dk), sB=(0, dk), sC=(T * ldbd, B * T * ldbd), splitk=False)
            O, P, Pd, ldT = attn_fwd(qu, qkv[:, d:], qkv[:, 2 * d:], B=B, H=H, T1=T, T2=T, dk=dk,
                                     ldq=d, ldk=3 * d, ldv=3 * d, klen=olens, causal=False, scale=scale,
                                     p=pa, seed=sd(3), cd=cd, bd=bd, ldbd=ldbd, rel_mode=mode)
            del bd
            s_core = ("unfused", qu, qv, P, Pd)
        x2 = empty(N, d, device=dev)
        ops.linear(O, b.w(A + "linear_out.weight"), x2,
                   epi=ops.make_epi(EPI_RESID, bias=b.f(A + "linear_out.bias"), resid=x1,
                                    drop_p=p, seed=sd(4)))
        C = "conv_module."
        K = L.conv_module.kernel_size
        xn3, mu3, rs3 = ln_fwd(x2, b, "norm_conv", cd)
        g2 = empty(N, 2 * d, dtype=cd, device=dev)
        ops.linear(xn3, b.w(C + "pointwise_conv1.weight", shape=(2 * d, d)), g2,
                   epi=ops.make_epi(bias=b.f(C + "pointwise_conv1.bias")))
        y = empty(N, d, device=dev)
        bn_part = None
        if _glu_in_conv(K, g2, d):
            glu = None
            if training and BN_STATS_IN_CONV:
                npart = ctypes.c_int(0)
                lib.ea_dwconv_stats_parts(B, T, ctypes.addressof(npart))
                bn_part = (empty(npart.value * 2 * d, device=dev), npart.value)
                lib.ea_dwconv_fwd_glu_stats(B, T, d, K, g2.data_ptr(), b.f(C + "depthwise_conv.weight").data_ptr(),
                                            b.f(C + "depthwise_conv.bias").data_ptr(), y.data_ptr(),
                                            bn_part[0].data_ptr(), ops.stream())
            else:
                lib.ea_dwconv_fwd_glu(B, T, d, K, g2.data_ptr(), b.f(C + "depthwise_conv.weight").data_ptr(),
                                      b.f(C + "depthwise_conv.bias").data_ptr(), y.data_ptr(), ops.stream())
        else:
            glu = empty(N, d, device=dev)
            lib.ea_glu_fwd(N, d, g2.data_ptr(), ops.dt(g2), glu.data_ptr(), 0, ops.stream())
            lib.ea_dwconv_fwd(B, T, d, K, glu.data_ptr(), b.f(C + "depthwise_conv.weight").data_ptr(),
                              b.f(C + "depthwise_conv.bias").data_ptr(), y.data_ptr(), ops.stream())
        z = empty(N, d, dtype=cd, device=dev)
        bn_mean = empty(d, device=dev)
        bn_rstd = empty(d, device=dev)
        bn = L.conv_module.norm
        if bn_part is not None:
            lib.ea_batchnorm_fwd_parts(N, d, y.data_ptr(), bn_part[0].data_ptr(), bn_part[1],
                                       b.f(C + "depthwise_conv.bias").data_ptr(), b.f(C + "norm.weight").data_ptr(),
                                       b.f(C + "norm.bias").data_ptr(), float(bn.eps), float(bn.momentum),
                                       bn_mean.data_ptr(), bn_rstd.data_ptr(), ops.ptr(bn.running_mean),
                                       ops.ptr(bn.running_var), ops.ptr(bn.num_batches_tracked), ACT_SWISH,
                                       z.data_ptr(), ops.dt(z), ops.stream())
        else:
            ops.batchnorm_fwd(y, b.f(C + "norm.weight"), b.f(C + "norm.bias"), bn_mean, bn_rstd,
                              bn.running_mean, bn.running_var, bn.num_batches_tracked, z,
                              training, ACT_SWISH, eps=bn.eps, momentum=bn.momentum)
        x3 = empty(N, d, device=dev)
        ops.linear(z, b.w(C + "pointwise_conv2.weight", shape=(d, d)), x3,
                   epi=ops.make_epi(EPI_RESID, bias=b.f(C + "pointwise_conv2.bias"), resid=x2,
                                    drop_p=p, seed=sd(5)))
        x4, s_ff2 = _ffn_fwd(L, b, x3, "feed_forward", "norm_ff", p, sd(6), sd(7))
        out, mu5, rs5 = ln_fwd(x4, b, "norm_final", F32)
        ctx.L = L
        ctx.meta = (B, T, d, H, dk, p, pa, seed, scale, ldT, mode)
        ctx.save = (x0, x1, x2, x3, x4, s_ff1, (xn2, mu2, rs2, qkv, pp, O, s_core),
                    (xn3, mu3, rs3, g2, glu, y, z, bn_mean, bn_rstd), s_ff2, (mu5, rs5), pos, olens)
        return out.view(B, T, d)

    @staticmethod
    def backward(ctx, dout):
        L = ctx.L
        b = L._b
        cd = b.cd
        B, T, d, H, dk, p, pa, seed, scale, ldT, mode = ctx.meta
        (x0, x1, x2, x3, x4, s_ff1, s_att, s_conv, s_ff2, (mu5, rs5), pos, olens) = ctx.save
        ctx.save = None
        li = L.layer_idx
        sd = lambda s: site_seed(seed, li, s)
        N = B * T
        dev = dout.device
        P2 = 2 * T - 1
        dx = empty(N, d, device=dev)
        dv_ff2 = dv_buf(N, d, cd, dev)
        ln_bwd(dout.reshape(N, d).contiguous(), x4, b, "norm_final", mu5, rs5, dx, accumulate=False,
               drop=drop_arg(dv_ff2, L.ff_scale, p, sd(7), b.g("feed_forward.w_2.bias")))
        dv_conv = dv_buf(N, d, cd, dev)
        _ffn_bwd(L, b, dx, x3, s_ff2, "feed_forward", "norm_ff", p, sd(6), sd(7), dv_in=dv_ff2,
                 next_drop=drop_arg(dv_conv, 1.0, p, sd(5), b.g("conv_module.pointwise_conv2.bias")))
        C = "conv_module."
        K = L.conv_module.kernel_size
        xn3, mu3, rs3, g2, glu, y, z, bn_mean, bn_rstd = s_conv
        dv = site_dv(dx, dv_conv, b.g(C + "pointwise_conv2.bias"), 1.0, p, sd(5), cd)
        with ops.wgrad(dv, z):
            ops.linear_dw(dv, z, b.g(C + "pointwise_conv2.weight", shape=(d, d)), accumulate=True)
        dz = empty(N, d, dtype=cd, device=dev)
        ops.linear_dx(dv, b.w(C + "pointwise_conv2.weight", shape=(d, d)), dz)
        dy = empty(N, d, device=dev)
        ops.batchnorm_bwd(dz, y, bn_mean, bn_rstd, b.f(C + "norm.weight"), b.f(C + "norm.bias"),
                          ACT_SWISH, dy, b.g(C + "norm.weight"), b.g(C + "norm.bias"))
        dg2 = empty(N, 2 * d, dtype=cd, device=dev)
        fuse = FUSE_DW_GLU and K in (3, 5, 7, 15, 31) and g2.dtype == torch.bfloat16
        if fuse:
            w, wn = ops.f32_ws(dev, B * ((T + 31) // 32) * d * (K + 1) + 1024)
            lib.ea_dwconv_glu_bwd(B, T, d, K, ops.ptr(glu), b.f(C + "depthwise_conv.weight").data_ptr(),
                                  dy.data_ptr(), g2.data_ptr(), dg2.data_ptr(),
                                  b.g(C + "depthwise_conv.weight").data_ptr(),
                                  b.g(C + "depthwise_conv.bias").data_ptr(), 1, w, wn, ops.stream())
        else:
            if glu is None:
                glu = empty(N, d, device=dev)
                lib.ea_glu_fwd(N, d, g2.data_ptr(), ops.dt(g2), glu.data_ptr(), 0, ops.stream())
            dglu = empty(N, d, device=dev)
            w, wn = ops.f32_ws(dev, B * ((T + 31) // 32) * d * (K + 1) + 1024)
            lib.ea_dwconv_bwd(B, T, d, K, glu.data_ptr(), b.f(C + "depthwise_conv.weight").data_ptr(),
                              dy.data_ptr(), dglu.data_ptr(), b.g(C + "depthwise_conv.weight").data_ptr(),
                              b.g(C + "depthwise_conv.bias").data_ptr(), 1, w, wn, ops.stream())
            lib.ea_glu_bwd(N, d, g2.data_ptr(), ops.dt(g2), dglu.data_ptr(), dg2.data_ptr(), ops.stream())
        with ops.wgrad(dg2, xn3):
            ops.colsum(dg2, b.g(C + "pointwise_conv1.bias"))
            ops.linear_dw(dg2, xn3, b.g(C + "pointwise_conv1.weight", shape=(2 * d, d)), accumulate=True)
        dxn3 = empty(N, d, dtype=cd, device=dev)
        ops.linear_dx(dg2, b.w(C + "pointwise_conv1.weight", shape=(2 * d, d)), dxn3)
        dv_att = dv_buf(N, d, cd, dev)
        ln_bwd(dxn3, x2, b, "norm_conv", mu3, rs3, dx, accumulate=True,
               drop=drop_arg(dv_att, 1.0, p, sd(4), b.g("self_attn.linear_out.bias")))
        A = "self_attn."
        xn2, mu2, rs2, qkv, pp, O, s_core = s_att
        dv = site_dv(dx, dv_att, b.g(A + "linear_out.bias"), 1.0, p, sd(4), cd)
        with ops.wgrad(dv, O):
            ops.linear_dw(dv, O, b.g(A + "linear_out.weight"), accumulate=True)
        dO = empty(N, d, dtype=cd, device=dev)
        ops.linear_dx(dv, b.w(A + "linear_out.weight"), dO)
        dqkv = empty(N, 3 * d, dtype=cd, device=dev)
        ldbd, shift = rup(P2, 8), 0
        if s_core[0] == "fused":
            _, lse, dmask, ldm, pp_full = s_core
            legacy = mode == REL_LEGACY
            shift, ldbd = dbd_layout(T)
            dbd = empty(H * B * T * ldbd, dtype=cd, device=dev)
            qv = empty(N, d, dtype=cd, device=dev)
            nqb = (T + 63) // 64
            part = empty(2 * B * nqb * d, device=dev)
            attn_fused_bwd(B=B, H=H, T1=T, T2=T, q=qkv, ldq=3 * d, k=qkv[:, d:], ldk=3 * d, v=qkv[:, 2 * d:],
                           ldv=3 * d, bu=b.f(A + "pos_bias_u"), bv=b.f(A + "pos_bias_v"), pp=pp, ldp=d,
                           klen=olens, causal=False, scale=scale, p=pa, seed=sd(3), O=O, ldo=d, lse=lse, dO=dO,
                           lddo=d, dq=dqkv, lddq=3 * d, dk=dqkv[:, d:], lddk=3 * d, dv=dqkv[:, 2 * d:],
                           lddv=3 * d, dbd=dbd, ldbd=ldbd, part=part, ldpart=d, qv_out=qv, ldqv=d, dmask=dmask,
                           ldm=ldm, flags=2 if legacy else 1 | 2, rel_mode=mode)
            ops.reduce_rows(part[:B * nqb * d], B * nqb, d, d, b.g(A + "pos_bias_u", shape=(d,)))
            if legacy:
                raw = dbd
                dbd = empty(H * B * T * ldbd, dtype=cd, device=dev)
                lib.ea_attn_legacy_band(H * B, T, raw.data_ptr(), dbd.data_ptr(), ldbd, ops.stream())
                del raw
                dqv = empty(N, d, dtype=cd, device=dev)
                ops.gemm(dbd, pp_full, dqv, M=T, N=dk, K=shift + P2, a_kmajor=1, b_kmajor=0, lda=ldbd, ldb=d, ldc=d,
                         batch=B, nh=H, sA=(T * ldbd, B * T * ldbd), sB=(0, dk), sC=(T * d, dk), splitk=False)
                ops.colsum(dqv, b.g(A + "pos_bias_v", shape=(d,)))
                lib.ea_add_2d(N, d, dqv.data_ptr(), ops.dt(dqv), d, dqkv.data_ptr(), ops.dt(dqkv), 3 * d, 1.0,
                              ops.stream())
            else:
                ops.reduce_rows(part[B * nqb * d:], B * nqb, d, d, b.g(A + "pos_bias_v", shape=(d,)))
        else:
            _, qu, qv, P, Pd = s_core
            dbd = empty(H * B * T * ldbd, dtype=cd, device=dev)
            attn_bwd(dO, qu, qkv[:, d:], qkv[:, 2 * d:], P, Pd, ldT, B=B, H=H, T1=T, T2=T, dk=dk,
                     ldq=d, ldk=3 * d, ldv=3 * d, scale=scale, p=pa, seed=sd(3), cd=cd,
                     dq=dqkv, lddq=3 * d, dk_=dqkv[:, d:], lddk=3 * d, dv=dqkv[:, 2 * d:], lddv=3 * d,
                     dbd=dbd, ldbd=ldbd, rel_mode=mode)
            dqv = empty(N, d, dtype=cd, device=dev)
            ops.gemm(dbd, pp, dqv, M=T, N=dk, K=P2, a_kmajor=1, b_kmajor=0, lda=ldbd, ldb=d, ldc=d,
                     batch=B, nh=H, sA=(T * ldbd, B * T * ldbd), sB=(0, dk), sC=(T * d, dk), splitk=False)
            ops.colsum(dqkv[:, :d], b.g(A + "pos_bias_u", shape=(d,)), defer=False)
            ops.colsum(dqv, b.g(A + "pos_bias_v", shape=(d,)))
            lib.ea_add_2d(N, d, dqv.data_ptr(), ops.dt(dqv), d, dqkv.data_ptr(), ops.dt(dqkv), 3 * d, 1.0,
                          ops.stream())
        qkv_w = b.w(A + "linear_q.weight", A + "linear_k.weight", A + "linear_v.weight", shape=(3 * d, d))

        def dpp_wgrad(after=None):
            with ops.wgrad(dbd, qv, pos, after=after, launches=True):
                Mp = P2 + shift if shift else P2
                dpp_full = empty(Mp, d, dtype=cd, device=dev)
                ops.gemm(dbd, qv, dpp_full, M=Mp, N=dk, K=B * T, a_kmajor=0, b_kmajor=0, lda=ldbd, ldb=d, ldc=d,
                         batch=1, nh=H, sA=(0, B * T * ldbd), sB=(0, dk), sC=(0, dk))
                dpp = dpp_full[shift:]
                if mode == REL_LEGACY:
                    dpp = empty(T, d, dtype=cd, device=dev)
                    lib.ea_legacy_pext_fold(T, d, dpp_full[shift:].data_ptr(), d, dpp.data_ptr(), d, ops.dt(dpp),
                                            ops.stream())
                ops.linear_dw(dpp, pos, b.g(A + "linear_pos.weight"), accumulate=True)

        fork = ops.fork_event()
        if fork is None:
            dpp_wgrad()
        with ops.wgrad(dqkv, xn2):
            ops.colsum(dqkv, b.g(A + "linear_q.bias", A + "linear_k.bias", A + "linear_v.bias", shape=(3 * d,)))
            ops.linear_dw(dqkv, xn2, b.g(A + "linear_q.weight", A + "linear_k.weight", A + "linear_v.weight",
                                          shape=(3 * d, d)), accumulate=True)
        dxn2 = empty(N, d, dtype=cd, device=dev)
        ops.linear_dx(dqkv, qkv_w, dxn2)
        if fork is not None:
            dpp_wgrad(after=fork)
        del dbd
        dv_ff1 = dv_buf(N, d, cd, dev)
        ln_bwd(dxn2, x1, b, "norm_mha", mu2, rs2, dx, accumulate=True,
               drop=drop_arg(dv_ff1, L.ff_scale, p, sd(2), b.g("feed_forward_macaron.w_2.bias")))
        _ffn_bwd(L, b, dx, x0, s_ff1, "feed_forward_macaron", "norm_ff_macaron", p, sd(1), sd(2), dv_in=dv_ff1)
        ops.grad_ready(b)
        return dx.view(B, T, d), None, None, None, None, None
```

espnet-1_amd/espnet_amd/layers/decoder.py:

```python
from __future__ import annotations

import math

import torch
from torch import nn

from .common import (ACT_RELU, EPI_ACT, EPI_DACT, EPI_RESID, EPI_STORE, F32, Bound, attn_bwd,
                     attn_dmask, attn_fused_bwd, attn_fwd, empty, fused_attn_ok, lib, ln_bwd, ln_fwd, ops,
                     site_seed, dv_buf, drop_arg, site_dv)


def _mha_fwd(q, k, v, *, B, H, T1, T2, dk, ldq, ldk, ldv, klen, causal, scale, p, seed, cd):
    if fused_attn_ok(cd, dk, T1, T2):
        O = empty(B * T1, H * dk, dtype=cd, device=q.device)
        lse = empty(B * H * T1, device=q.device)
        dmask, ldm = attn_dmask(B * H * T1, T2, p, q.device)
        lib.ea_attn_fused_fwd2(B, H, T1, T2, dk, q.data_ptr(), ldq, k.data_ptr(), ldk, v.data_ptr(), ldv,
                               None, None, None, 0, klen.data_ptr(), int(causal), scale, float(p), seed,
                               O.data_ptr(), H * dk, lse.data_ptr(), ops.ptr(dmask), ldm, ops.stream())
        return O, ("fused", O, lse, dmask, ldm)
    O, P, Pd, ldT = attn_fwd(q, k, v, B=B, H=H, T1=T1, T2=T2, dk=dk, ldq=ldq, ldk=ldk, ldv=ldv, klen=klen,
                             causal=causal, scale=scale, p=p, seed=seed, cd=cd)
    return O, ("unfused", P, Pd, ldT)


def _mha_bwd(st, dO, q, k, v, *, B, H, T1, T2, dk, ldq, ldk, ldv, klen, causal, scale, p, seed, cd,
             dq, lddq, dk_, lddk, dv, lddv):
    if st[0] == "fused":
        _, O, lse, dmask, ldm = st
        attn_fused_bwd(B=B, H=H, T1=T1, T2=T2, q=q, ldq=ldq, k=k, ldk=ldk, v=v, ldv=ldv, bu=None, bv=None, pp=None,
                       ldp=0, klen=klen, causal=causal, scale=scale, p=p, seed=seed, O=O, ldo=H * dk, lse=lse,
                       dO=dO, lddo=H * dk, dq=dq, lddq=lddq, dk=dk_, lddk=lddk, dv=dv, lddv=lddv, dmask=dmask,
                       ldm=ldm)
        return
    _, P, Pd, ldT = st
    attn_bwd(dO, q, k, v, P, Pd, ldT, B=B, H=H, T1=T1, T2=T2, dk=dk, ldq=ldq, ldk=ldk, ldv=ldv, scale=scale,
             p=p, seed=seed, cd=cd, dq=dq, lddq=lddq, dk_=dk_, lddk=lddk, dv=dv, lddv=lddv)
from .conformer import LayerNorm, MultiHeadedAttention, PositionwiseFeedForward


def sinusoid_table(n, d):
    pe = torch.zeros(n, d)
    pos = torch.arange(0, n, dtype=torch.float32).unsqueeze(1)
    div = torch.exp(torch.arange(0, d, 2, dtype=torch.float32) * -(math.log(10000.0) / d))
    pe[:, 0::2] = torch.sin(pos * div)
    pe[:, 1::2] = torch.cos(pos * div)
    return pe


class PositionalEncoding(nn.Module):

    absolute = True

    def __init__(self, d_model, dropout_rate, max_len=5000):
        super().__init__()
        self.d_model = d_model
        self.xscale = math.sqrt(d_model)
        self.dropout_rate = dropout_rate
        self.max_len = max_len
        self._pe = None

    def table(self, L, device):
        if self._pe is None or self._pe.shape[0] < L or self._pe.device != device:
            self._pe = sinusoid_table(max(self.max_len, L), self.d_model).to(device)
        return self._pe


class DecoderLayer(nn.Module):

    def __init__(self, size, self_attn, src_attn, feed_forward, dropout_rate,
                 normalize_before=True, concat_after=False):
        super().__init__()
        if not normalize_before or concat_after:
            raise NotImplementedError("only normalize_before=True, concat_after=False")
        self.size = size
        self.self_attn = self_attn
        self.src_attn = src_attn
        self.feed_forward = feed_forward
        self.norm1 = LayerNorm(size)
        self.norm2 = LayerNorm(size)
        self.norm3 = LayerNorm(size)
        self.dropout_rate = dropout_rate


def decoder_arena_groups(prefix, num_blocks):
    g = []
    for i in range(num_blocks):
        a = f"{prefix}decoders.{i}.self_attn."
        g.append([a + "linear_q.weight", a + "linear_k.weight", a + "linear_v.weight"])
        g.append([a + "linear_q.bias", a + "linear_k.bias", a + "linear_v.bias"])
    kw, kb = [], []
    for i in range(num_blocks):
        a = f"{prefix}decoders.{i}.src_attn."
        kw += [a + "linear_k.weight", a + "linear_v.weight"]
        kb += [a + "linear_k.bias", a + "linear_v.bias"]
    return g + [kw, kb]


def _kv_names(nb):
    w, b = [], []
    for i in range(nb):
        a = f"decoders.{i}.src_attn."
        w += [a + "linear_k.weight", a + "linear_v.weight"]
        b += [a + "linear_k.bias", a + "linear_v.bias"]
    return w, b


class DecoderFn(torch.autograd.Function):
    @staticmethod
    def forward(ctx, memory, hlens, ys_in, ys_in_lens, dec, seed, training):
        b = dec._b
        cd = b.cd
        B, Tm, d = memory.shape
        L = ys_in.shape[1]
        N, Nm = B * L, B * Tm
        nb = len(dec.decoders)
        H = dec.decoders[0].self_attn.h
        dk = d // H
        V = dec.output_layer.out_features
        dev = memory.device
        p = dec.dropout_rate if training else 0.0
        p_sa = dec.self_attention_dropout_rate if training else 0.0
        p_src = dec.src_attention_dropout_rate if training else 0.0
        p_pos = dec.embed[1].dropout_rate if training else 0.0
        sd = lambda l, s: site_seed(seed, 100 + l, s)
        scale = 1.0 / math.sqrt(dk)
        mem = ops.cast(memory.reshape(Nm, d), cd)
        kvw, kvb = _kv_names(nb)
        kv = empty(Nm, 2 * d * nb, dtype=cd, device=dev)
        ops.linear(mem, b.w(*kvw, shape=(2 * d * nb, d)), kv,
                   epi=ops.make_epi(bias=b.f(*kvb, shape=(2 * d * nb,))))
        pe = dec.embed[1]
        x = empty(N, d, device=dev)
        lib.ea_embed_fwd(N, d, L, ys_in.data_ptr(), b.f("embed.0.weight").data_ptr(), pe.xscale,
                         pe.table(L, dev).data_ptr(), p_pos, sd(0, 0), x.data_ptr(), ops.stream())
        saved = []
        ldkv = 2 * d * nb
        for l in range(nb):
            n = f"decoders.{l}."
            sa, xa = n + "self_attn.", n + "src_attn."
            xn1, mu1, rs1 = ln_fwd(x, b, n + "norm1", cd)
            qkv = empty(N, 3 * d, dtype=cd, device=dev)
            ops.linear(xn1, b.w(sa + "linear_q.weight", sa + "linear_k.weight", sa + "linear_v.weight",
                                shape=(3 * d, d)), qkv,
                       epi=ops.make_epi(bias=b.f(sa + "linear_q.bias", sa + "linear_k.bias",
                                                 sa + "linear_v.bias", shape=(3 * d,))))
            O1, st1 = _mha_fwd(qkv, qkv[:, d:], qkv[:, 2 * d:], B=B, H=H, T1=L, T2=L, dk=dk,
                               ldq=3 * d, ldk=3 * d, ldv=3 * d, klen=ys_in_lens, causal=True,
                               scale=scale, p=p_sa, seed=sd(l, 1), cd=cd)
            x1 = empty(N, d, device=dev)
            ops.linear(O1, b.w(sa + "linear_out.weight"), x1,
                       epi=ops.make_epi(EPI_RESID, bias=b.f(sa + "linear_out.bias"), resid=x,
                                        drop_p=p, seed=sd(l, 2)))
            xn2, mu2, rs2 = ln_fwd(x1, b, n + "norm2", cd)
            q2 = empty(N, d, dtype=cd, device=dev)
            ops.linear(xn2, b.w(xa + "linear_q.weight"), q2, epi=ops.make_epi(bias=b.f(xa + "linear_q.bias")))
            k2 = kv[:, 2 * d * l:]
            v2 = kv[:, 2 * d * l + d:]
            O2, st2 = _mha_fwd(q2, k2, v2, B=B, H=H, T1=L, T2=Tm, dk=dk, ldq=d, ldk=ldkv,
                               ldv=ldkv, klen=hlens, causal=False, scale=scale, p=p_src,
                               seed=sd(l, 3), cd=cd)
            x2 = empty(N, d, device=dev)
            ops.linear(O2, b.w(xa + "linear_out.weight"), x2,
                       epi=ops.make_epi(EPI_RESID, bias=b.f(xa + "linear_out.bias"), resid=x1,
                                        drop_p=p, seed=sd(l, 4)))
            xn3, mu3, rs3 = ln_fwd(x2, b, n + "norm3", cd)
            Fh = dec.decoders[l].feed_forward.w_1.out_features
            h = empty(N, Fh, dtype=cd, device=dev)
            a = empty(N, Fh, dtype=cd, device=dev)
            ff = n + "feed_forward."
            ops.linear(xn3, b.w(ff + "w_1.weight"), a,
                       epi=ops.make_epi(EPI_ACT, bias=b.f(ff + "w_1.bias"), act=ACT_RELU, aux=h,
                                        drop_p=p, seed=sd(l, 5)))
            x3 = empty(N, d, device=dev)
            ops.linear(a, b.w(ff + "w_2.weight"), x3,
                       epi=ops.make_epi(EPI_RESID, bias=b.f(ff + "w_2.bias"), resid=x2,
                                        drop_p=p, seed=sd(l, 6)))
            saved.append((x, x1, x2, (xn1, mu1, rs1, qkv, O1, st1),
                          (xn2, mu2, rs2, q2, O2, st2), (xn3, mu3, rs3, h, a)))
            x = x3
        xf, muf, rsf = ln_fwd(x, b, "after_norm", cd)
        logits = empty(N, V, device=dev)
        ops.linear(xf, b.w("output_layer.weight"), logits,
                   epi=ops.make_epi(bias=b.f("output_layer.bias")))
        ctx.dec = dec
        ctx.meta = (B, Tm, L, d, H, dk, nb, p, p_sa, p_src, p_pos, seed, scale)
        ctx.save = (mem, kv, ys_in, saved, x, xf, muf, rsf, hlens, ys_in_lens)
        return logits.view(B, L, V)

    @staticmethod
    def backward(ctx, dlogits):
        dec = ctx.dec
        b = dec._b
        cd = b.cd
        B, Tm, L, d, H, dk, nb, p, p_sa, p_src, p_pos, seed, scale = ctx.meta
        mem, kv, ys_in, saved, xlast, xf, muf, rsf, hlens, ys_in_lens = ctx.save
        ctx.save = None
        sd = lambda l, s: site_seed(seed, 100 + l, s)
        N, Nm = B * L, B * Tm
        V = dlogits.shape[-1]
        dev = dlogits.device
        dlog = ops.cast(dlogits.reshape(N, V).contiguous(), cd)
        with ops.wgrad(dlog, xf):
            ops.colsum(dlog, b.g("output_layer.bias"))
            ops.linear_dw(dlog, xf, b.g("output_layer.weight"), accumulate=True)
        dxf = empty(N, d, dtype=cd, device=dev)
        ops.linear_dx(dlog, b.w("output_layer.weight"), dxf)
        dx = empty(N, d, device=dev)
        dv_ff = dv_buf(N, d, cd, dev) if nb > 0 else None
        ln_bwd(dxf, xlast, b, "after_norm", muf, rsf, dx, accumulate=False,
               drop=None if dv_ff is None else
               drop_arg(dv_ff, 1.0, p, sd(nb - 1, 6), b.g(f"decoders.{nb - 1}.feed_forward.w_2.bias")))
        ldkv = 2 * d * nb
        dkv = empty(Nm, ldkv, dtype=cd, device=dev)
        for l in reversed(range(nb)):
            n = f"decoders.{l}."
            sa, xa, ff = n + "self_attn.", n + "src_attn.", n + "feed_forward."
            x0, x1, x2, s1, s2, s3 = saved[l]
            xn3, mu3, rs3, h, a = s3
            dv = site_dv(dx, dv_ff, b.g(ff + "w_2.bias"), 1.0, p, sd(l, 6), cd)
            with ops.wgrad(dv, a):
                ops.linear_dw(dv, a, b.g(ff + "w_2.weight"), accumulate=True)
            fork = ops.fork_event() if l < nb - 1 else None
            dh = empty(*h.shape, dtype=cd, device=dev)
            ops.linear_dx(dv, b.w(ff + "w_2.weight"), dh,
                          epi=ops.make_epi(EPI_DACT, act=ACT_RELU, aux=h, drop_p=p, seed=sd(l, 5)))
            if fork is not None:
                ops.flush_wgrad_side(after=fork)
            with ops.wgrad(dh, xn3):
                ops.colsum(dh, b.g(ff + "w_1.bias"))
                ops.linear_dw(dh, xn3, b.g(ff + "w_1.weight"), accumulate=True)
            dxn = empty(N, d, dtype=cd, device=dev)
            ops.linear_dx(dh, b.w(ff + "w_1.weight"), dxn)
            dv_src = dv_buf(N, d, cd, dev)
            ln_bwd(dxn, x2, b, n + "norm3", mu3, rs3, dx, accumulate=True,
                   drop=drop_arg(dv_src, 1.0, p, sd(l, 4), b.g(xa + "linear_out.bias")))
            xn2, mu2, rs2, q2, O2, st2 = s2
            dv = site_dv(dx, dv_src, b.g(xa + "linear_out.bias"), 1.0, p, sd(l, 4), cd)
            with ops.wgrad(dv, O2):
                ops.linear_dw(dv, O2, b.g(xa + "linear_out.weight"), accumulate=True)
            dO = empty(N, d, dtype=cd, device=dev)
            ops.linear_dx(dv, b.w(xa + "linear_out.weight"), dO)
            dq = empty(N, d, dtype=cd, device=dev)
            _mha_bwd(st2, dO, q2, kv[:, 2 * d * l:], kv[:, 2 * d * l + d:], B=B, H=H, T1=L, T2=Tm, dk=dk,
                     ldq=d, ldk=ldkv, ldv=ldkv, klen=hlens, causal=False, scale=scale, p=p_src,
                     seed=sd(l, 3), cd=cd, dq=dq, lddq=d, dk_=dkv[:, 2 * d * l:], lddk=ldkv,
                     dv=dkv[:, 2 * d * l + d:], lddv=ldkv)
            with ops.wgrad(dq, xn2):
                ops.colsum(dq, b.g(xa + "linear_q.bias"))
                ops.linear_dw(dq, xn2, b.g(xa + "linear_q.weight"), accumulate=True)
            dxn = empty(N, d, dtype=cd, device=dev)
            ops.linear_dx(dq, b.w(xa + "linear_q.weight"), dxn)
            dv_self = dv_buf(N, d, cd, dev)
            ln_bwd(dxn, x1, b, n + "norm2", mu2, rs2, dx, accumulate=True,
                   drop=drop_arg(dv_self, 1.0, p, sd(l, 2), b.g(sa + "linear_out.bias")))
            xn1, mu1, rs1, qkv, O1, st1 = s1
            dv = site_dv(dx, dv_self, b.g(sa + "linear_out.bias"), 1.0, p, sd(l, 2), cd)
            with ops.wgrad(dv, O1):
                ops.linear_dw(dv, O1, b.g(sa + "linear_out.weight"), accumulate=True)
            dO = empty(N, d, dtype=cd, device=dev)
            ops.linear_dx(dv, b.w(sa + "linear_out.weight"), dO)
            dqkv = empty(N, 3 * d, dtype=cd, device=dev)
            _mha_bwd(st1, dO, qkv, qkv[:, d:], qkv[:, 2 * d:], B=B, H=H, T1=L, T2=L, dk=dk,
                     ldq=3 * d, ldk=3 * d, ldv=3 * d, klen=ys_in_lens, causal=True, scale=scale, p=p_sa,
                     seed=sd(l, 1), cd=cd, dq=dqkv, lddq=3 * d, dk_=dqkv[:, d:], lddk=3 * d,
                     dv=dqkv[:, 2 * d:], lddv=3 * d)
            wn = (sa + "linear_q.weight", sa + "linear_k.weight", sa + "linear_v.weight")
            bn = (sa + "linear_q.bias", sa + "linear_k.bias", sa + "linear_v.bias")
            with ops.wgrad(dqkv, xn1):
                ops.colsum(dqkv, b.g(*bn, shape=(3 * d,)))
                ops.linear_dw(dqkv, xn1, b.g(*wn, shape=(3 * d, d)), accumulate=True)
            dxn = empty(N, d, dtype=cd, device=dev)
            ops.linear_dx(dqkv, b.w(*wn, shape=(3 * d, d)), dxn)
            dv_ff = dv_buf(N, d, cd, dev) if l > 0 else None
            ln_bwd(dxn, x0, b, n + "norm1", mu1, rs1, dx, accumulate=True,
                   drop=None if dv_ff is None else
                   drop_arg(dv_ff, 1.0, p, sd(l - 1, 6), b.g(f"decoders.{l - 1}.feed_forward.w_2.bias")))
        pe = dec.embed[1]
        lib.ea_embed_bwd(N, d, ys_in.data_ptr(), dx.data_ptr(), pe.xscale, p_pos, sd(0, 0),
                         b.g("embed.0.weight").data_ptr(), ops.stream())
        kvw, kvb = _kv_names(nb)
        with ops.wgrad(dkv, mem):
            ops.colsum(dkv, b.g(*kvb, shape=(ldkv,)))
            ops.linear_dw(dkv, mem, b.g(*kvw, shape=(ldkv, d)), accumulate=True)
        dmem = empty(Nm, d, device=dev)
        ops.linear_dx(dkv, b.w(*kvw, shape=(ldkv, d)), dmem)
        ops.grad_ready(b)
        return dmem.view(B, Tm, d), None, None, None, None, None, None
```

espnet-1_amd/espnet_amd/layers/ebranchformer.py:

```python
from __future__ import annotations

import ctypes

import torch
from torch import nn

from .common import (EPI_RESID, EPI_STORE, F32, Bound, attn_bwd, attn_dmask, attn_fused_bwd, attn_fwd, dbd_layout,
                     drop_arg, dv_buf, empty, fused_attn_ok, lib, ln_bwd, ln_fwd, math, ops, rup, site_dv, site_seed)
from .conformer import LayerNorm, _ffn_bwd, _ffn_fwd

CONV_KERNELS = (3, 5, 7, 15, 31)


class ConvolutionalSpatialGatingUnit(nn.Module):

    def __init__(self, size, kernel_size, dropout_rate, use_linear_after_conv, gate_activation):
        super().__init__()
        if use_linear_after_conv:
            raise NotImplementedError("use_linear_after_conv=True is not on the HIP hot path")
        if gate_activation != "identity":
            raise NotImplementedError(f"gate_activation={gate_activation} is not on the HIP hot path")
        n_channels = size // 2
        self.norm = LayerNorm(n_channels)
        self.conv = nn.Conv1d(n_channels, n_channels, kernel_size, 1, (kernel_size - 1) // 2, groups=n_channels)
        self.linear = None
        self.kernel_size = kernel_size
        self.dropout_rate = dropout_rate


class ConvolutionalGatingMLP(nn.Module):

    def __init__(self, size, linear_units, kernel_size, dropout_rate, use_linear_after_conv, gate_activation):
        super().__init__()
        self.channel_proj1 = nn.Sequential(nn.Linear(size, linear_units), nn.GELU())
        self.csgu = ConvolutionalSpatialGatingUnit(linear_units, kernel_size, dropout_rate, use_linear_after_conv,
                                                   gate_activation)
        self.channel_proj2 = nn.Linear(linear_units // 2, size)
        self.linear_units = linear_units


class EBranchformerEncoderLayer(nn.Module):

    def __init__(self, size, attn, cgmlp, feed_forward, feed_forward_macaron, dropout_rate, merge_conv_kernel=3):
        super().__init__()
        if feed_forward is None:
            raise NotImplementedError("use_ffn=False is not on the HIP hot path")
        self.size = size
        self.attn = attn
        self.cgmlp = cgmlp
        self.feed_forward = feed_forward
        self.feed_forward_macaron = feed_forward_macaron
        self.ff_scale = 1.0
        if self.feed_forward is not None:
            self.norm_ff = LayerNorm(size)
        if self.feed_forward_macaron is not None:
            self.ff_scale = 0.5
            self.norm_ff_macaron = LayerNorm(size)
        self.norm_mha = LayerNorm(size)
        self.norm_mlp = LayerNorm(size)
        self.norm_final = LayerNorm(size)
        self.dropout_rate = dropout_rate
        self.depthwise_conv_fusion = nn.Conv1d(size + size, size + size, kernel_size=merge_conv_kernel, stride=1,
                                               padding=(merge_conv_kernel - 1) // 2, groups=size + size, bias=True)
        self.merge_proj = nn.Linear(size + size, size)
        self.merge_conv_kernel = merge_conv_kernel
        self.layer_idx = 0
        self._b = None

    def bind(self, arena, prefix, cd):
        self._b = Bound(arena, prefix, cd)

    @staticmethod
    def arena_groups(prefix):
        a = prefix + "attn."
        return [[a + "linear_q.weight", a + "linear_k.weight", a + "linear_v.weight"],
                [a + "linear_q.bias", a + "linear_k.bias", a + "linear_v.bias"]]

    def forward(self, x, pos_emb, olens, seed):
        return EBranchformerBlockFn.apply(x, pos_emb, olens, self, seed, self.training)


def _attn_fwd(L, b, xn, pos, olens, B, T, pa, seed3):
    cd = b.cd
    N, d = xn.shape
    dev = xn.device
    H = L.attn.h
    dk = d // H
    P2 = 2 * T - 1
    A = "attn."
    qkv = empty(N, 3 * d, dtype=cd, device=dev)
    ops.linear(xn, b.w(A + "linear_q.weight", A + "linear_k.weight", A + "linear_v.weight", shape=(3 * d, d)), qkv,
               epi=ops.make_epi(bias=b.f(A + "linear_q.bias", A + "linear_k.bias", A + "linear_v.bias",
                                         shape=(3 * d,))))
    pp = empty(P2, d, dtype=cd, device=dev)
    ops.linear(pos, b.w(A + "linear_pos.weight"), pp)
    scale = 1.0 / math.sqrt(dk)
    if fused_attn_ok(cd, dk, T, T):
        O = empty(N, d, dtype=cd, device=dev)
        lse = empty(B * H * T, device=dev)
        dmask, ldm = attn_dmask(B * H * T, T, pa, dev)
        lib.ea_attn_fused_fwd2(B, H, T, T, dk, qkv.data_ptr(), 3 * d, qkv[:, d:].data_ptr(), 3 * d,
                               qkv[:, 2 * d:].data_ptr(), 3 * d, b.f(A + "pos_bias_u").data_ptr(),
                               b.f(A + "pos_bias_v").data_ptr(), pp.data_ptr(), d, olens.data_ptr(), 0,
                               scale, float(pa), seed3, O.data_ptr(), d, lse.data_ptr(), ops.ptr(dmask), ldm,
                               ops.stream())
        ldT = 0
        s_core = ("fused", lse, dmask, ldm)
    else:
        qu = empty(N, d, dtype=cd, device=dev)
        qv = empty(N, d, dtype=cd, device=dev)
        lib.ea_add_pos_bias(N, H, dk, qkv.data_ptr(), 3 * d, b.f(A + "pos_bias_u").data_ptr(),
                            b.f(A + "pos_bias_v").data_ptr(), qu.data_ptr(), qv.data_ptr(), ops.dt(qu), ops.stream())
        ldbd = rup(P2, 8)
        bd = empty(H * B * T * ldbd, device=dev)
        ops.gemm(qv, pp, bd, M=T, N=P2, K=dk, a_kmajor=1, b_kmajor=1, lda=d, ldb=d, ldc=ldbd,
                 batch=B, nh=H, sA=(T * d, dk), sB=(0, dk), sC=(T * ldbd, B * T * ldbd), splitk=False)
        O, P, Pd, ldT = attn_fwd(qu, qkv[:, d:], qkv[:, 2 * d:], B=B, H=H, T1=T, T2=T, dk=dk,
                                 ldq=d, ldk=3 * d, ldv=3 * d, klen=olens, causal=False, scale=scale,
                                 p=pa, seed=seed3, cd=cd, bd=bd, ldbd=ldbd)
        del bd
        s_core = ("unfused", qu, qv, P, Pd)
    return O, (qkv, pp, s_core, scale, ldT)


def _attn_bwd(L, b, dO, xn, O, saved, pos, olens, B, T, pa, seed3):
    cd = b.cd
    N, d = xn.shape
    dev = dO.device
    H = L.attn.h
    dk = d // H
    P2 = 2 * T - 1
    A = "attn."
    qkv, pp, s_core, scale, ldT = saved
    dqkv = empty(N, 3 * d, dtype=cd, device=dev)
    ldbd, shift = rup(P2, 8), 0
    if s_core[0] == "fused":
        _, lse, dmask, ldm = s_core
        shift, ldbd = dbd_layout(T)
        dbd = empty(H * B * T * ldbd, dtype=cd, device=dev)
        qv = empty(N, d, dtype=cd, device=dev)
        nqb = (T + 63) // 64
        part = empty(2 * B * nqb * d, device=dev)
        attn_fused_bwd(B=B, H=H, T1=T, T2=T, q=qkv, ldq=3 * d, k=qkv[:, d:], ldk=3 * d, v=qkv[:, 2 * d:],
                       ldv=3 * d, bu=b.f(A + "pos_bias_u"), bv=b.f(A + "pos_bias_v"), pp=pp, ldp=d,
                       klen=olens, causal=False, scale=scale, p=pa, seed=seed3, O=O, ldo=d, lse=lse, dO=dO,
                       lddo=d, dq=dqkv, lddq=3 * d, dk=dqkv[:, d:], lddk=3 * d, dv=dqkv[:, 2 * d:],
                       lddv=3 * d, dbd=dbd, ldbd=ldbd, part=part, ldpart=d, qv_out=qv, ldqv=d, dmask=dmask,
                       ldm=ldm, flags=1 | 2)
        ops.reduce_rows(part[:B * nqb * d], B * nqb, d, d, b.g(A + "pos_bias_u", shape=(d,)))
        ops.reduce_rows(part[B * nqb * d:], B * nqb, d, d, b.g(A + "pos_bias_v", shape=(d,)))
    else:
        _, qu, qv, P, Pd = s_core
        dbd = empty(H * B * T * ldbd, dtype=cd, device=dev)
        attn_bwd(dO, qu, qkv[:, d:], qkv[:, 2 * d:], P, Pd, ldT, B=B, H=H, T1=T, T2=T, dk=dk,
                 ldq=d, ldk=3 * d, ldv=3 * d, scale=scale, p=pa, seed=seed3, cd=cd,
                 dq=dqkv, lddq=3 * d, dk_=dqkv[:, d:], lddk=3 * d, dv=dqkv[:, 2 * d:], lddv=3 * d,
                 dbd=dbd, ldbd=ldbd)
        dqv = empty(N, d, dtype=cd, device=dev)
        ops.gemm(dbd, pp, dqv, M=T, N=dk, K=P2, a_kmajor=1, b_kmajor=0, lda=ldbd, ldb=d, ldc=d,
                 batch=B, nh=H, sA=(T * ldbd, B * T * ldbd), sB=(0, dk), sC=(T * d, dk), splitk=False)
        ops.colsum(dqkv[:, :d], b.g(A + "pos_bias_u", shape=(d,)), defer=False)
        ops.colsum(dqv, b.g(A + "pos_bias_v", shape=(d,)))
        lib.ea_add_2d(N, d, dqv.data_ptr(), ops.dt(dqv), d, dqkv.data_ptr(), ops.dt(dqkv), 3 * d, 1.0, ops.stream())
    qkv_w = b.w(A + "linear_q.weight", A + "linear_k.weight", A + "linear_v.weight", shape=(3 * d, d))

    def dpp_wgrad(after=None):
        with ops.wgrad(dbd, qv, pos, after=after, launches=True):
            Mp = P2 + shift if shift else P2
            dpp_full = empty(Mp, d, dtype=cd, device=dev)
            ops.gemm(dbd, qv, dpp_full, M=Mp, N=dk, K=B * T, a_kmajor=0, b_kmajor=0, lda=ldbd, ldb=d, ldc=d,
                     batch=1, nh=H, sA=(0, B * T * ldbd), sB=(0, dk), sC=(0, dk))
            ops.linear_dw(dpp_full[shift:], pos, b.g(A + "linear_pos.weight"), accumulate=True)

    fork = ops.fork_event()
    if fork is None:
        dpp_wgrad()
    with ops.wgrad(dqkv, xn):
        ops.colsum(dqkv, b.g(A + "linear_q.bias", A + "linear_k.bias", A + "linear_v.bias", shape=(3 * d,)))
        ops.linear_dw(dqkv, xn, b.g(A + "linear_q.weight", A + "linear_k.weight", A + "linear_v.weight",
                                    shape=(3 * d, d)), accumulate=True)
    dxn = empty(N, d, dtype=cd, device=dev)
    ops.linear_dx(dqkv, qkv_w, dxn)
    if fork is not None:
        dpp_wgrad(after=fork)
    return dxn


def _long(v=0):
    return ctypes.c_long(v)


class EBranchformerBlockFn(torch.autograd.Function):
    @staticmethod
    def forward(ctx, x, pos, olens, L: EBranchformerEncoderLayer, seed, training):
        b = L._b
        cd = b.cd
        B, T, d = x.shape
        N = B * T
        dev = x.device
        p = L.dropout_rate if training else 0.0
        pa = L.attn.dropout_rate if training else 0.0
        pg = L.cgmlp.csgu.dropout_rate if training else 0.0
        li = L.layer_idx
        sd = lambda s: site_seed(seed, li, s)
        macaron = L.feed_forward_macaron is not None
        x0 = x.reshape(N, d)
        if macaron:
            x1, s_ff1 = _ffn_fwd(L, b, x0, "feed_forward_macaron", "norm_ff_macaron", p, sd(1), sd(2))
        else:
            x1, s_ff1 = x0, None
        xc = empty(N, 2 * d, dtype=cd, device=dev)
        xna, mua, rsa = ln_fwd(x1, b, "norm_mha", cd)
        O, s_core = _attn_fwd(L, b, xna, pos, olens, B, T, pa, sd(3))
        ops.linear(O, b.w("attn.linear_out.weight"), xc[:, :d],
                   epi=ops.make_epi(EPI_STORE, bias=b.f("attn.linear_out.bias"), drop_p=p, seed=sd(4)))
        G = "cgmlp."
        U = L.cgmlp.linear_units
        C = U // 2
        Kc = L.cgmlp.csgu.kernel_size
        xnm, mum, rsm = ln_fwd(x1, b, "norm_mlp", cd)
        h = empty(N, U, dtype=cd, device=dev)
        ops.linear(xnm, b.w(G + "channel_proj1.0.weight"), h, epi=ops.make_epi(bias=b.f(G + "channel_proj1.0.bias")))
        gmu = empty(N, device=dev)
        grs = empty(N, device=dev)
        lib.ea_csgu_stats(N, U, h.data_ptr(), ops.dt(h), 1e-12, gmu.data_ptr(), grs.data_ptr(), ops.stream())
        gout = empty(N, C, dtype=cd, device=dev)
        lib.ea_csgu_fwd(B, T, U, Kc, h.data_ptr(), ops.dt(h), gmu.data_ptr(), grs.data_ptr(),
                        b.f(G + "csgu.norm.weight").data_ptr(), b.f(G + "csgu.norm.bias").data_ptr(),
                        b.f(G + "csgu.conv.weight").data_ptr(), b.f(G + "csgu.conv.bias").data_ptr(),
                        float(pg), sd(5), gout.data_ptr(), ops.stream())
        ops.linear(gout, b.w(G + "channel_proj2.weight"), xc[:, d:],
                   epi=ops.make_epi(EPI_STORE, bias=b.f(G + "channel_proj2.bias"), drop_p=p, seed=sd(6)))
        Km = L.merge_conv_kernel
        m = empty(N, 2 * d, dtype=cd, device=dev)
        lib.ea_merge_conv_fwd(B, T, 2 * d, Km, xc.data_ptr(), ops.dt(xc), b.f("depthwise_conv_fusion.weight").data_ptr(),
                              b.f("depthwise_conv_fusion.bias").data_ptr(), m.data_ptr(), ops.stream())
        x2 = empty(N, d, device=dev)
        ops.linear(m, b.w("merge_proj.weight"), x2,
                   epi=ops.make_epi(EPI_RESID, bias=b.f("merge_proj.bias"), resid=x1, drop_p=p, seed=sd(7)))
        x3, s_ff2 = _ffn_fwd(L, b, x2, "feed_forward", "norm_ff", p, sd(8), sd(9))
        out, muf, rsf = ln_fwd(x3, b, "norm_final", F32)
        ctx.L = L
        ctx.meta = (B, T, d, p, pa, pg, seed)
        ctx.save = (x0, x1, x2, x3, s_ff1, (xna, mua, rsa, O, s_core), (xnm, mum, rsm, h, gmu, grs, gout), (xc, m),
                    s_ff2, (muf, rsf), pos, olens)
        return out.view(B, T, d)

    @staticmethod
    def backward(ctx, dout):
        L = ctx.L
        b = L._b
        cd = b.cd
        B, T, d, p, pa, pg, seed = ctx.meta
        (x0, x1, x2, x3, s_ff1, s_att, s_mlp, (xc, m), s_ff2, (muf, rsf), pos, olens) = ctx.save
        ctx.save = None
        li = L.layer_idx
        sd = lambda s: site_seed(seed, li, s)
        macaron = L.feed_forward_macaron is not None
        N = B * T
        dev = dout.device
        dx = empty(N, d, device=dev)
        dv_ff2 = dv_buf(N, d, cd, dev)
        ln_bwd(dout.reshape(N, d).contiguous(), x3, b, "norm_final", muf, rsf, dx, accumulate=False,
               drop=drop_arg(dv_ff2, L.ff_scale, p, sd(9), b.g("feed_forward.w_2.bias")))
        dv_mg = dv_buf(N, d, cd, dev)
        _ffn_bwd(L, b, dx, x2, s_ff2, "feed_forward", "norm_ff", p, sd(8), sd(9), dv_in=dv_ff2,
                 next_drop=drop_arg(dv_mg, 1.0, p, sd(7), b.g("merge_proj.bias")))
        dv = site_dv(dx, dv_mg, b.g("merge_proj.bias"), 1.0, p, sd(7), cd)
        with ops.wgrad(dv, m):
            ops.linear_dw(dv, m, b.g("merge_proj.weight"), accumulate=True)
        dm = empty(N, 2 * d, dtype=cd, device=dev)
        ops.linear_dx(dv, b.w("merge_proj.weight"), dm)
        del m
        Km = L.merge_conv_kernel
        n_ws = _long()
        lib.ea_merge_conv_bwd_ws_elems(B, T, 2 * d, Km, ctypes.addressof(n_ws))
        w, wn = ops.f32_ws(dev, n_ws.value)
        dxc = empty(N, 2 * d, dtype=cd, device=dev)
        lib.ea_merge_conv_bwd(B, T, 2 * d, Km, xc.data_ptr(), dm.data_ptr(), ops.dt(dm),
                              b.f("depthwise_conv_fusion.weight").data_ptr(), float(p), sd(4), sd(6), dxc.data_ptr(),
                              b.g("depthwise_conv_fusion.weight").data_ptr(),
                              b.g("depthwise_conv_fusion.bias").data_ptr(), 1, w, wn, ops.stream())
        del dm, xc
        G = "cgmlp."
        U = L.cgmlp.linear_units
        C = U // 2
        Kc = L.cgmlp.csgu.kernel_size
        xnm, mum, rsm, h, gmu, grs, gout = s_mlp
        dv2 = dxc[:, d:]
        with ops.wgrad(dxc, gout):
            ops.colsum(dv2, b.g(G + "channel_proj2.bias"))
            ops.linear_dw(dv2, gout, b.g(G + "channel_proj2.weight"), accumulate=True)
        dgout = empty(N, C, dtype=cd, device=dev)
        ops.linear_dx(dv2, b.w(G + "channel_proj2.weight"), dgout)
        n_dln, n_ws = _long(), _long()
        lib.ea_csgu_bwd_ws_elems(B, T, U, Kc, ctypes.addressof(n_dln), ctypes.addressof(n_ws))
        dln = empty(n_dln.value, device=dev)
        w, wn = ops.f32_ws(dev, n_ws.value)
        dh = empty(N, U, dtype=cd, device=dev)
        lib.ea_csgu_bwd(B, T, U, Kc, dgout.data_ptr(), h.data_ptr(), ops.dt(h), gmu.data_ptr(), grs.data_ptr(),
                        b.f(G + "csgu.norm.weight").data_ptr(), b.f(G + "csgu.norm.bias").data_ptr(),
                        b.f(G + "csgu.conv.weight").data_ptr(), b.f(G + "csgu.conv.bias").data_ptr(),
                        float(pg), sd(5), dh.data_ptr(),
                        b.g(G + "csgu.norm.weight").data_ptr(), b.g(G + "csgu.norm.bias").data_ptr(),
                        b.g(G + "csgu.conv.weight").data_ptr(), b.g(G + "csgu.conv.bias").data_ptr(), 1,
                        dln.data_ptr(), w, wn, ops.stream())
        del dln, dgout
        with ops.wgrad(dh, xnm):
            ops.colsum(dh, b.g(G + "channel_proj1.0.bias"))
            ops.linear_dw(dh, xnm, b.g(G + "channel_proj1.0.weight"), accumulate=True)
        dxnm = empty(N, d, dtype=cd, device=dev)
        ops.linear_dx(dh, b.w(G + "channel_proj1.0.weight"), dxnm)
        ln_bwd(dxnm, x1, b, "norm_mlp", mum, rsm, dx, accumulate=True)
        xna, mua, rsa, O, s_core = s_att
        dv1 = dxc[:, :d]
        with ops.wgrad(dxc, O):
            ops.colsum(dv1, b.g("attn.linear_out.bias"))
            ops.linear_dw(dv1, O, b.g("attn.linear_out.weight"), accumulate=True)
        dO = empty(N, d, dtype=cd, device=dev)
        ops.linear_dx(dv1, b.w("attn.linear_out.weight"), dO)
        dxna = _attn_bwd(L, b, dO, xna, O, s_core, pos, olens, B, T, pa, sd(3))
        if macaron:
            dv_ff1 = dv_buf(N, d, cd, dev)
            ln_bwd(dxna, x1, b, "norm_mha", mua, rsa, dx, accumulate=True,
                   drop=drop_arg(dv_ff1, L.ff_scale, p, sd(2), b.g("feed_forward_macaron.w_2.bias")))
            _ffn_bwd(L, b, dx, x0, s_ff1, "feed_forward_macaron", "norm_ff_macaron", p, sd(1), sd(2), dv_in=dv_ff1)
        else:
            ln_bwd(dxna, x1, b, "norm_mha", mua, rsa, dx, accumulate=True)
        ops.grad_ready(b)
        return dx.view(B, T, d), None, None, None, None, None
```

espnet-1_amd/espnet_amd/layers/interctc.py:

```python
from __future__ import annotations

import torch

from .common import EPI_RESID, F32, empty, lib, ln_bwd, ln_fwd, ops
from .losses import _g


class TapState:

    def __init__(self):
        self.deferred = False

    def arm(self, on: bool, *modules):
        self.deferred = on
        for m in modules:
            if m is not None:
                m._ready_deferred = on


class InterCTCTapFn(torch.autograd.Function):

    @staticmethod
    def forward(ctx, x, hlens, ys, ylens, enc, ctc, Lmax, first):
        bn, bc = enc.after_norm._b, ctc._b
        cd = bc.cd
        B, T, d = x.shape
        V = ctc.ctc_lo.out_features
        N = B * T
        dev = x.device
        cond = bool(enc.interctc_use_conditioning)
        x2 = x.reshape(N, d)
        y, mu, rs = ln_fwd(x2, bn, "", F32)
        h = ops.cast(y, cd)
        logits = empty(N, V, device=dev)
        ops.linear(h, bc.w("ctc_lo.weight"), logits, epi=ops.make_epi(bias=bc.f("ctc_lo.bias")))
        lse = empty(N, device=dev)
        p = empty(N, V, dtype=cd, device=dev)
        lib.ea_softmax_lse_rows(N, V, logits.data_ptr(), V, lse.data_ptr(), p.data_ptr(), ops.dt(p), V, ops.stream())
        loss = empty((), device=dev)
        lat = None
        if ys is not None:
            S = 2 * Lmax + 1
            alpha = torch.empty(N * S, dtype=torch.float64, device=dev)
            beta = torch.empty(N * S, dtype=torch.float64, device=dev)
            nll = torch.empty(B, dtype=torch.float64, device=dev)
            loss_utt = empty(B, device=dev)
            with ops.aux(logits, lse, hlens, ys, ylens, alpha, beta, nll, loss_utt, loss):
                lib.ea_ctc_loss_fwd_lse(B, T, V, logits.data_ptr(), V, hlens.data_ptr(), ys.data_ptr(), ys.stride(0),
                                        ylens.data_ptr(), Lmax, lse.data_ptr(), alpha.data_ptr(), beta.data_ptr(),
                                        nll.data_ptr(), loss_utt.data_ptr(), loss.data_ptr(), ops.stream())
            lat = (alpha, beta, nll, hlens, ys, ylens)
        else:
            loss.zero_()
        if cond:
            be = enc.conditioning_layer._b
            xo = empty(N, d, device=dev)
            ops.linear(p, be.w("weight"), xo, epi=ops.make_epi(EPI_RESID, bias=be.f("bias"), resid=x2))
        else:
            xo = x2
        if torch.is_grad_enabled() or x.requires_grad:
            ctx.save = (x2, mu, rs, h, logits, lse, p if cond else None, lat)
            ctx.mods = (enc, ctc)
            ctx.meta = (B, T, d, V, Lmax, cond, first)
        yv = y.view(B, T, d)
        ctx.mark_non_differentiable(yv)
        return xo.view(B, T, d), loss, yv

    @staticmethod
    def backward(ctx, gx, gl, gy):
        x2, mu, rs, h, logits, lse, p, lat = ctx.save
        ctx.save = None
        enc, ctc = ctx.mods
        B, T, d, V, Lmax, cond, first = ctx.meta
        bn, bc = enc.after_norm._b, ctc._b
        cd = bc.cd
        N = B * T
        dev = gx.device
        dxo = gx.reshape(N, d)
        if dxo.dtype != F32:
            raise RuntimeError("the residual-stream gradient must be float32")
        dxo = dxo.contiguous()
        dp = None
        if cond:
            be = enc.conditioning_layer._b
            dxc = ops.cast(dxo, cd)
            with ops.wgrad(dxc, p):
                ops.colsum(dxc, be.g("bias"))
                ops.linear_dw(dxc, p, be.g("weight"), accumulate=True)
            dp = empty(N, V, dtype=cd, device=dev)
            ops.linear_dx(dxc, be.w("weight"), dp)
        if lat is None and dp is None:
            if first:
                _report_shared(enc, ctc)
            return gx, None, None, None, None, None, None, None
        dl = empty(N, V, dtype=cd, device=dev)
        if lat is not None:
            alpha, beta, nll, hlens, ys, ylens = lat
            gl = _g(gl)
            lib.ea_interctc_dlogits(B, T, V, logits.data_ptr(), V, hlens.data_ptr(), ys.data_ptr(), ys.stride(0),
                                    ylens.data_ptr(), Lmax, lse.data_ptr(), alpha.data_ptr(), beta.data_ptr(),
                                    nll.data_ptr(), gl.data_ptr(), 1.0 / B, ops.ptr(dp), V, dl.data_ptr(), ops.dt(dl),
                                    V, ops.stream())
        else:
            lib.ea_interctc_dlogits(B, T, V, logits.data_ptr(), V, None, None, 0, None, 0, lse.data_ptr(), None, None,
                                    None, None, 0.0, dp.data_ptr(), V, dl.data_ptr(), ops.dt(dl), V, ops.stream())
        with ops.wgrad(dl, h):
            ops.colsum(dl, bc.g("ctc_lo.bias"))
            ops.linear_dw(dl, h, bc.g("ctc_lo.weight"), accumulate=True)
        dy = empty(N, d, device=dev)
        ops.linear_dx(dl, bc.w("ctc_lo.weight"), dy)
        dx = dxo.clone()
        ln_bwd(dy, x2, bn, "", mu, rs, dx, accumulate=True)
        if first:
            _report_shared(enc, ctc)
        return dx.view(B, T, d), None, None, None, None, None, None, None


def _report_shared(enc, ctc):
    if not enc._taps.deferred:
        return
    ops.grad_ready(ctc._b)
    ops.grad_ready(enc.after_norm._b)
    if enc.conditioning_layer is not None:
        ops.grad_ready(enc.conditioning_layer._b)


class InterCTCMixFn(torch.autograd.Function):

    @staticmethod
    def forward(ctx, w, loss_ctc, *loss_ics):
        dev = loss_ctc.device
        st = ops.stream()
        K = len(loss_ics)
        s = loss_ics[0]
        for l in loss_ics[1:]:
            t = empty((), device=dev)
            lib.ea_axpby_scalar(s.data_ptr(), 1.0, l.data_ptr(), 1.0, t.data_ptr(), st)
            s = t
        out = empty((), device=dev)
        lib.ea_axpby_scalar(loss_ctc.data_ptr(), 1.0 - w, s.data_ptr(), w / K, out.data_ptr(), st)
        ctx.wk = (w, K)
        return out

    @staticmethod
    def backward(ctx, g):
        w, K = ctx.wk
        g = _g(g)
        st = ops.stream()
        ga = empty((), device=g.device)
        gb = empty((), device=g.device)
        lib.ea_axpby_scalar(g.data_ptr(), 1.0 - w, 0, 0.0, ga.data_ptr(), st)
        lib.ea_axpby_scalar(g.data_ptr(), w / K, 0, 0.0, gb.data_ptr(), st)
        return (None, ga) + (gb,) * K
```

espnet-1_amd/espnet_amd/layers/losses.py:

```python
from __future__ import annotations

import contextlib

import torch

from .common import F32, empty, lib, ops, shared_grad_ready


def _g(t):
    t = t.contiguous()
    if t.dtype != F32:
        raise RuntimeError("loss gradients must be float32")
    return t


CTC_BWD_IN_FWD = True
_ONE = {}


def _one(dev):
    t = _ONE.get(dev)
    if t is None:
        t = _ONE[dev] = torch.ones((), dtype=torch.float32, device=dev)
    return t


class CTCFn(torch.autograd.Function):
    @staticmethod
    def forward(ctx, hs, hlens, ys, ylens, ctc, Lmax):
        b = ctc._b
        cd = b.cd
        B, T, d = hs.shape
        V = ctc.ctc_lo.out_features
        dev = hs.device
        N = B * T
        h = empty(N, d, dtype=cd, device=dev)
        logits = empty(N, V, device=dev)
        S = 2 * Lmax + 1
        lse = empty(N, device=dev)
        alpha = torch.empty(B * T * S, dtype=torch.float64, device=dev)
        beta = torch.empty(B * T * S, dtype=torch.float64, device=dev)
        nll = torch.empty(B, dtype=torch.float64, device=dev)
        loss_utt = empty(B, device=dev)
        loss = empty((), device=dev)
        def head():
            ops.scale_dropout(hs.reshape(N, d), h, p=ctc.dropout_rate, seed=ctc._seed)
            ops.linear(h, b.w("ctc_lo.weight"), logits, epi=ops.make_epi(bias=b.f("ctc_lo.bias")))

        pre = CTC_BWD_IN_FWD and ctx.needs_input_grad[0]
        with (ops.aux(hs, h, logits, hlens, ys, ylens, lse, alpha, beta, nll, loss_utt, loss) if ctc._overlap
              else contextlib.nullcontext()):
            head()
            lib.ea_ctc_loss_fwd(B, T, V, logits.data_ptr(), V, hlens.data_ptr(), ys.data_ptr(), ys.stride(0),
                                ylens.data_ptr(), Lmax, lse.data_ptr(), alpha.data_ptr(), beta.data_ptr(),
                                nll.data_ptr(), loss_utt.data_ptr(), loss.data_ptr(), ops.stream())
            if pre:
                dl = empty(N, V, dtype=cd, device=dev)
                lib.ea_ctc_loss_bwd(B, T, V, logits.data_ptr(), V, hlens.data_ptr(), ys.data_ptr(), ys.stride(0),
                                    ylens.data_ptr(), Lmax, lse.data_ptr(), alpha.data_ptr(), beta.data_ptr(),
                                    nll.data_ptr(), _one(dev).data_ptr(), 1.0 / B, dl.data_ptr(), ops.dt(dl), V,
                                    ops.stream())
                dW = empty(V, d, device=dev)
                db = empty(V, device=dev)
                ops.linear_dw(dl, h, dW, accumulate=False)
                ops.colsum(dl, db, accumulate=False, defer=False)
                dh = empty(N, d, device=dev)
                ops.linear_dx(dl, b.w("ctc_lo.weight"), dh)
                if ctc.dropout_rate > 0:
                    ops.scale_dropout(dh, dh, p=ctc.dropout_rate, seed=ctc._seed)
                del dl
        ctx.ctc = ctc
        ctx.meta = (B, T, V, Lmax, d)
        ctx.pre = pre
        if pre:
            main = torch.cuda.current_stream()
            for t in (dh, dW, db):
                t.record_stream(main)
            ctx.save = (dh, dW, db)
        else:
            ctx.save = (h, logits, lse, alpha, beta, nll, hlens, ys, ylens)

        return loss

    @staticmethod
    def backward(ctx, gl):
        ctc = ctx.ctc
        b = ctc._b
        cd = b.cd
        B, T, V, Lmax, d = ctx.meta
        if ctx.pre:
            dh, dW, db = ctx.save
            ctx.save = None
            gl = _g(gl)
            ops.take_aux_fork()
            st = ops.stream()
            lib.ea_scale_by_scalar(dh.numel(), dh.data_ptr(), gl.data_ptr(), 1.0, st)
            lib.ea_axpy_dev(dW.numel(), dW.data_ptr(), b.g("ctc_lo.weight").data_ptr(), gl.data_ptr(), 1.0, st)
            lib.ea_axpy_dev(V, db.data_ptr(), b.g("ctc_lo.bias").data_ptr(), gl.data_ptr(), 1.0, st)
            shared_grad_ready(ctc)
            return dh.view(B, T, d), None, None, None, None, None
        h, logits, lse, alpha, beta, nll, hlens, ys, ylens = ctx.save
        ctx.save = None
        N = B * T
        dev = gl.device
        gl = _g(gl)
        fork = ops.take_aux_fork() if ctc._overlap else None
        with (ops.aux(gl, logits, hlens, ys, ylens, lse, alpha, beta, nll, h, after=fork)
              if fork is not None else contextlib.nullcontext()):
            dl = empty(N, V, dtype=cd, device=dev)
            dh = empty(N, d, device=dev)
            lib.ea_ctc_loss_bwd(B, T, V, logits.data_ptr(), V, hlens.data_ptr(), ys.data_ptr(), ys.stride(0),
                                ylens.data_ptr(), Lmax, lse.data_ptr(), alpha.data_ptr(), beta.data_ptr(),
                                nll.data_ptr(), gl.data_ptr(), 1.0 / B, dl.data_ptr(), ops.dt(dl), V,
                                ops.stream())
            with ops.wgrad(dl, h):
                ops.colsum(dl, b.g("ctc_lo.bias"))
                ops.linear_dw(dl, h, b.g("ctc_lo.weight"), accumulate=True)
            ops.linear_dx(dl, b.w("ctc_lo.weight"), dh)
            if ctc.dropout_rate > 0:
                ops.scale_dropout(dh, dh, p=ctc.dropout_rate, seed=ctc._seed)
        if fork is not None:
            ops.join_aux()
            dh.record_stream(torch.cuda.current_stream())
        shared_grad_ready(ctc)
        return dh.view(B, T, d), None, None, None, None, None


class LabelSmoothingLossFn(torch.autograd.Function):

    @staticmethod
    def forward(ctx, x, target, crit):
        B, L, V = x.shape
        rows = B * L
        dev = x.device
        x2 = x.reshape(rows, V)
        lse = empty(rows, device=dev)
        loss_row = torch.empty(rows, dtype=torch.float64, device=dev)
        stat = torch.empty(2, dtype=torch.int32, device=dev)
        loss = empty((), device=dev)
        acc = empty((), device=dev)
        inv = empty(1, device=dev)
        tgt = target.reshape(rows).contiguous()
        lib.ea_lsm_loss_fwd(rows, V, x2.data_ptr(), V, tgt.data_ptr(), crit.smoothing, crit.padding_idx,
                            int(crit.normalize_length), float(B), lse.data_ptr(), loss_row.data_ptr(),
                            stat.data_ptr(), loss.data_ptr(), acc.data_ptr(), inv.data_ptr(), ops.stream())
        ctx.save = (x2, tgt, lse, inv, crit)
        ctx.shape = (B, L, V)
        ctx.mark_non_differentiable(acc)
        return loss, acc

    @staticmethod
    def backward(ctx, gloss, gacc):
        x2, tgt, lse, inv, crit = ctx.save
        ctx.save = None
        B, L, V = ctx.shape
        grad = empty(B, L, V, device=x2.device)
        lib.ea_lsm_loss_bwd(B * L, V, x2.data_ptr(), V, tgt.data_ptr(), crit.smoothing, crit.padding_idx,
                            lse.data_ptr(), _g(gloss).data_ptr(), inv.data_ptr(), 1.0, grad.data_ptr(),
                            0, V, ops.stream())
        return grad, None, None


class CombineFn(torch.autograd.Function):

    @staticmethod
    def forward(ctx, a, b, w):
        out = empty((), device=a.device)
        lib.ea_axpby_scalar(a.data_ptr(), w, b.data_ptr(), 1.0 - w, out.data_ptr(), ops.stream())
        ctx.w = w
        return out

    @staticmethod
    def backward(ctx, g):
        g = _g(g)
        ga = empty((), device=g.device)
        gb = empty((), device=g.device)
        lib.ea_axpby_scalar(g.data_ptr(), ctx.w, 0, 0.0, ga.data_ptr(), ops.stream())
        lib.ea_axpby_scalar(g.data_ptr(), 1.0 - ctx.w, 0, 0.0, gb.data_ptr(), ops.stream())
        ops.mark_aux_fork()
        return ga, gb, None
```

espnet-1_amd/espnet_amd/layers/transformer.py:

```python
from __future__ import annotations

import math

import torch
from torch import nn

from .common import (ACT_RELU, EPI_ACT, EPI_DACT, EPI_RESID, Bound, empty, ln_bwd, ln_fwd, ops, site_dv,
                     site_seed)
from .conformer import LayerNorm
from .decoder import _mha_bwd, _mha_fwd


class TransformerEncoderLayer(nn.Module):

    def __init__(self, size, self_attn, feed_forward, dropout_rate, normalize_before=True, concat_after=False,
                 stochastic_depth_rate=0.0):
        super().__init__()
        if not normalize_before or concat_after or stochastic_depth_rate > 0:
            raise NotImplementedError("only normalize_before=True, concat_after=False, "
                                      "stochastic_depth_rate=0 are implemented")
        self.self_attn = self_attn
        self.feed_forward = feed_forward
        self.norm1 = LayerNorm(size)
        self.norm2 = LayerNorm(size)
        self.size = size
        self.dropout_rate = dropout_rate
        self.layer_idx = 0
        self._b = None

    def bind(self, arena, prefix, cd):
        self._b = Bound(arena, prefix, cd)

    @staticmethod
    def arena_groups(prefix):
        a = prefix + "self_attn."
        return [[a + "linear_q.weight", a + "linear_k.weight", a + "linear_v.weight"],
                [a + "linear_q.bias", a + "linear_k.bias", a + "linear_v.bias"]]

    def forward(self, x, olens, seed):
        return TransformerBlockFn.apply(x, olens, self, seed, self.training)


_QKV_W = ("self_attn.linear_q.weight", "self_attn.linear_k.weight", "self_attn.linear_v.weight")
_QKV_B = ("self_attn.linear_q.bias", "self_attn.linear_k.bias", "self_attn.linear_v.bias")


class TransformerBlockFn(torch.autograd.Function):
    @staticmethod
    def forward(ctx, x, olens, L: TransformerEncoderLayer, seed, training):
        b = L._b
        cd = b.cd
        B, T, d = x.shape
        N = B * T
        dev = x.device
        H = L.self_attn.h
        dk = d // H
        p = L.dropout_rate if training else 0.0
        pa = L.self_attn.dropout_rate if training else 0.0
        p_ff = L.feed_forward.dropout_rate if training else 0.0
        sd = lambda s: site_seed(seed, 50 + L.layer_idx, s)
        scale = 1.0 / math.sqrt(dk)
        x0 = x.reshape(N, d)
        xn1, mu1, rs1 = ln_fwd(x0, b, "norm1", cd)
        qkv = empty(N, 3 * d, dtype=cd, device=dev)
        ops.linear(xn1, b.w(*_QKV_W, shape=(3 * d, d)), qkv, epi=ops.make_epi(bias=b.f(*_QKV_B, shape=(3 * d,))))
        O, st = _mha_fwd(qkv, qkv[:, d:], qkv[:, 2 * d:], B=B, H=H, T1=T, T2=T, dk=dk, ldq=3 * d, ldk=3 * d,
                         ldv=3 * d, klen=olens, causal=getattr(L, "causal", False), scale=scale, p=pa, seed=sd(1), cd=cd)
        x1 = empty(N, d, device=dev)
        ops.linear(O, b.w("self_attn.linear_out.weight"), x1,
                   epi=ops.make_epi(EPI_RESID, bias=b.f("self_attn.linear_out.bias"), resid=x0, drop_p=p,
                                    seed=sd(2)))
        xn2, mu2, rs2 = ln_fwd(x1, b, "norm2", cd)
        Fh = L.feed_forward.w_1.out_features
        h = empty(N, Fh, dtype=cd, device=dev)
        a = empty(N, Fh, dtype=cd, device=dev)
        ops.linear(xn2, b.w("feed_forward.w_1.weight"), a,
                   epi=ops.make_epi(EPI_ACT, bias=b.f("feed_forward.w_1.bias"), act=ACT_RELU, aux=h, drop_p=p_ff,
                                    seed=sd(3)))
        x2 = empty(N, d, device=dev)
        ops.linear(a, b.w("feed_forward.w_2.weight"), x2,
                   epi=ops.make_epi(EPI_RESID, bias=b.f("feed_forward.w_2.bias"), resid=x1, drop_p=p, seed=sd(4)))
        ctx.L = L
        ctx.meta = (B, T, d, H, dk, p, pa, p_ff, seed, scale)
        ctx.save = (x0, x1, (xn1, mu1, rs1, qkv, O, st), (xn2, mu2, rs2, h, a), olens)
        return x2.view(B, T, d)

    @staticmethod
    def backward(ctx, dout):
        L = ctx.L
        b = L._b
        cd = b.cd
        B, T, d, H, dk, p, pa, p_ff, seed, scale = ctx.meta
        x0, x1, s_att, s_ff, olens = ctx.save
        ctx.save = None
        sd = lambda s: site_seed(seed, 50 + L.layer_idx, s)
        N = B * T
        dev = dout.device
        dx = dout.reshape(N, d).contiguous().clone()
        xn2, mu2, rs2, h, a = s_ff
        dv = site_dv(dx, None, b.g("feed_forward.w_2.bias"), 1.0, p, sd(4), cd)
        with ops.wgrad(dv, a):
            ops.linear_dw(dv, a, b.g("feed_forward.w_2.weight"), accumulate=True)
        dh = empty(*h.shape, dtype=cd, device=dev)
        ops.linear_dx(dv, b.w("feed_forward.w_2.weight"), dh,
                      epi=ops.make_epi(EPI_DACT, act=ACT_RELU, aux=h, drop_p=p_ff, seed=sd(3)))
        with ops.wgrad(dh, xn2):
            ops.colsum(dh, b.g("feed_forward.w_1.bias"))
            ops.linear_dw(dh, xn2, b.g("feed_forward.w_1.weight"), accumulate=True)
        dxn = empty(N, d, dtype=cd, device=dev)
        ops.linear_dx(dh, b.w("feed_forward.w_1.weight"), dxn)
        ln_bwd(dxn, x1, b, "norm2", mu2, rs2, dx, accumulate=True)
        xn1, mu1, rs1, qkv, O, st = s_att
        dv = site_dv(dx, None, b.g("self_attn.linear_out.bias"), 1.0, p, sd(2), cd)
        with ops.wgrad(dv, O):
            ops.linear_dw(dv, O, b.g("self_attn.linear_out.weight"), accumulate=True)
        dO = empty(N, d, dtype=cd, device=dev)
        ops.linear_dx(dv, b.w("self_attn.linear_out.weight"), dO)
        dqkv = empty(N, 3 * d, dtype=cd, device=dev)
        _mha_bwd(st, dO, qkv, qkv[:, d:], qkv[:, 2 * d:], B=B, H=H, T1=T, T2=T, dk=dk, ldq=3 * d, ldk=3 * d,
                 ldv=3 * d, klen=olens, causal=getattr(L, "causal", False), scale=scale, p=pa, seed=sd(1), cd=cd, dq=dqkv, lddq=3 * d,
                 dk_=dqkv[:, d:], lddk=3 * d, dv=dqkv[:, 2 * d:], lddv=3 * d)
        with ops.wgrad(dqkv, xn1):
            ops.colsum(dqkv, b.g(*_QKV_B, shape=(3 * d,)))
            ops.linear_dw(dqkv, xn1, b.g(*_QKV_W, shape=(3 * d, d)), accumulate=True)
        dxn = empty(N, d, dtype=cd, device=dev)
        ops.linear_dx(dqkv, b.w(*_QKV_W, shape=(3 * d, d)), dxn)
        ln_bwd(dxn, x0, b, "norm1", mu1, rs1, dx, accumulate=True)
        ops.grad_ready(b)
        return dx.view(B, T, d), None, None, None, None
```

include/espnet_amd.h:

```cpp
#ifndef ESPNET_AMD_H
#define ESPNET_AMD_H

#include <stddef.h>

#ifdef __cplusplus
extern "C" {
#endif

enum { EA_F32 = 0, EA_BF16 = 1 };
enum { EA_OK = 0, EA_ERR_BAD_ARG = 1000 };
enum { EA_ACT_NONE = 0, EA_ACT_SWISH = 1, EA_ACT_RELU = 2 };

enum { EA_EPI_STORE = 0, EA_EPI_ACT = 1, EA_EPI_RESID = 2, EA_EPI_DACT = 3 };

typedef struct ea_epilogue {
  int kind;
  int act;
  float alpha, beta, post_scale, rscale, drop_p;
  unsigned long long seed;
  const float* bias;
  void* aux;
  int aux_dtype;
  long ldaux;
  const float* resid;
  long ldr;
} ea_epilogue;

int ea_gemm(int dtype, int a_kmajor, int b_kmajor, int M, int N, int K,
            const void* A, long lda, long sAb, long sAh,
            const void* B, long ldb, long sBb, long sBh,
            int batch, int nh,
            void* C, int c_dtype, long ldc, long sCb, long sCh,
            const ea_epilogue* epi, float* workspace, long ws_elems, void* stream);


enum { EA_CONV_FWD = 1, EA_CONV_DGRAD = 2, EA_CONV_WGRAD = 3 };
typedef struct ea_conv_geo {
  int mode;
  int B, T2, F2, C, P;
  int nI[2], nJ[2];
  int a, e;
  long plane[4];
  long zero;
} ea_conv_geo;
int ea_gemm_conv(const ea_conv_geo* geo, int a_kmajor, int b_kmajor, int M, int N, int K,
                 const void* A, long lda, const void* B, long ldb, void* C, int c_dtype, long ldc,
                 const ea_epilogue* epi, float* workspace, long ws_elems, void* stream);
int ea_gemm_conv_w1(const ea_conv_geo* geo, int M, int N, int K, const void* A, long lda, const void* B,
                    long ldb, const ea_epilogue* epi, const float* x, int T, int Fin, float* part,
                    void* stream);
int ea_gemm_conv_w1b(const ea_conv_geo* geo, int M, int N, int K, const void* A, long lda, const void* B,
                     long ldb, const ea_epilogue* epi, const float* x, int T, int Fin, float* part,
                     const unsigned char* pos, void* stream);
int ea_gemm_conv_w1b_all(const ea_conv_geo* geo, int N, const void* A, long lda, const void* B, long ldb,
                         const ea_epilogue* epi, const float* x, int T, int Fin, float* part,
                         const unsigned char* pos, void* stream);
int ea_conv1_wgrad_reduce(int ntiles, int C, const float* part, float* dw, float* dbias, void* stream);

int ea_gemm_set_pipeline(int stages);

int ea_gemm_set_tile(int bm, int bn);
int ea_gemm_set_pipe(int on);
int ea_gemm_set_k128(int mode, int slots);
int ea_gemm_set_skinny(int max_m);
int ea_gemm_ln(int M, int N, int K, const float* x, long ldx, const float* gamma, const float* beta, float eps,
               const void* W, long ldw, void* C, int c_dtype, long ldc, const ea_epilogue* epi, void* stream);

typedef struct ea_group_gemm {
  const void* A;
  const void* B;
  float* C;
  long lda, ldb, ldc;
  int M, N, K;
  float beta;
} ea_group_gemm;
int ea_gemm_grouped(int a_kmajor, int b_kmajor, int n, const ea_group_gemm* probs, void* ws, long ws_bytes,
                    void* stream);
int ea_gemm_grouped_ws_bytes(int n, long ntiles, long* bytes);
int ea_gemm_grouped_set_xcd_chunk(int chunk);

int ea_gemm_set_probe(unsigned long long* slots);
int ea_gemm_set_diag(unsigned long long* buf);
int ea_phase_stamp(unsigned long long* state, float* ring, int cap, int phase, const float* extra, void* stream);
struct ea_opt_state;
int ea_phase_stamp_opt(unsigned long long* state, float* ring, int cap, int phase, const struct ea_opt_state* opt,
                       void* stream);
int ea_probe_begin(unsigned long long* slots, void* stream);
int ea_probe_end(unsigned long long* slots, void* stream);
int ea_debug_spin(long ns, void* stream);
void* ea_guard_malloc(size_t size, int device, void* stream);
void ea_guard_free(void* ptr, size_t size, int device, void* stream);


int ea_layernorm_fwd(int rows, int d, const float* x, long ldx, const float* gamma,
                     const float* beta, float eps, void* y, int y_dtype, long ldy,
                     float* mean, float* rstd, void* stream);

int ea_layernorm_bwd(int rows, int d, const void* dy, int dy_dtype, long lddy, const float* x,
                     long ldx, const float* gamma, const float* mean, const float* rstd,
                     float* dx, long lddx, int accumulate, float* dgamma, float* dbeta,
                     int accumulate_params, float* workspace, long ws_elems, void* stream);

int ea_reduce_partials(int nparts, int n, const float* part, long stride, float* out,
                       int accumulate, void* stream);

int ea_colsum(int rows, int n, const void* x, int x_dtype, long ld, float* out, int accumulate,
              float* workspace, long ws_elems, void* stream);

int ea_layernorm_bwd_partials(int rows, int d, const void* dy, int dy_dtype, long lddy, const float* x,
                              long ldx, const float* gamma, const float* mean, const float* rstd,
                              float* dx, long lddx, int accumulate, float* part, long part_elems,
                              int* nparts, void* stream);

int ea_layernorm_bwd_drop(int rows, int d, const void* dy, int dy_dtype, long lddy, const float* x,
                          long ldx, const float* gamma, const float* mean, const float* rstd, float* dx,
                          long lddx, int accumulate, float* dgamma, float* dbeta, int accumulate_params,
                          float* workspace, long ws_elems, void* y, int y_dtype, long ldy, float yscale,
                          float p, unsigned long long seed, float* ycol, void* stream);
int ea_layernorm_bwd_partials_drop(int rows, int d, const void* dy, int dy_dtype, long lddy,
                                   const float* x, long ldx, const float* gamma, const float* mean,
                                   const float* rstd, float* dx, long lddx, int accumulate, float* part,
                                   long part_elems, int* nparts, void* y, int y_dtype, long ldy,
                                   float yscale, float p, unsigned long long seed, float* ycol,
                                   int* ycol_parts, void* stream);

typedef struct ea_colsum_prob {
  const void* x;
  float* part;
  long ld;
  int rows, n, dtype, rpp;
} ea_colsum_prob;
typedef struct ea_reduce_prob {
  const float* part;
  float* out;
  long stride;
  int nparts, n, accumulate;
} ea_reduce_prob;
int ea_colsum_grouped(int n, const ea_colsum_prob* probs, void* ws, long ws_bytes, void* stream);
int ea_reduce_grouped(int n, const ea_reduce_prob* probs, void* ws, long ws_bytes, void* stream);
int ea_grouped_table_bytes(int n, long* colsum_bytes, long* reduce_bytes);

int ea_batchnorm_fwd(int rows, int C, const float* y, const float* gamma, const float* beta,
                     float eps, float momentum, int training, float* mean, float* rstd,
                     float* running_mean, float* running_var, long long* num_batches_tracked,
                     int act, void* z, int z_dtype, float* workspace, long ws_elems, void* stream);

int ea_batchnorm_fwd_parts(int rows, int C, const float* y, const float* part, int nparts, const float* shift,
                           const float* gamma, const float* beta, float eps, float momentum, float* mean,
                           float* rstd, float* running_mean, float* running_var, long long* num_batches_tracked,
                           int act, void* z, int z_dtype, void* stream);

int ea_batchnorm_bwd(int rows, int C, const void* dz, int dz_dtype, const float* y, const float* mean,
                     const float* rstd, const float* gamma, const float* beta, int act, float* dy,
                     float* dgamma, float* dbeta, int accumulate_params, float* workspace,
                     long ws_elems, void* stream);


int ea_utterance_mvn(int B, int T, int F, const float* x, const long long* lens, float* y, void* stream);
int ea_utterance_mvn_ws_bytes(int B, int T, int F, long* bytes);
int ea_utterance_mvn2(int B, int T, int F, const float* x, const long long* lens, float* y, void* ws,
                      long ws_bytes, void* stream);

int ea_stft_frames(int B, long Ns, int nF, int n_fft, int hop, int center, const float* x,
                   const float* window, float* frames, void* stream);
int ea_power_spectrum(long M, int nF, int nbins, const float* spec, long ld_spec, const long long* flens,
                      float* power, long ld_power, void* stream);
int ea_logmel_mvn(long M, int nF, int n_mels, const float* mel, long ld_mel, const long long* flens,
                  const float* mean, const float* std, float* y, void* stream);
int ea_global_mvn(int B, int T, int D, const float* x, const long long* lens, const float* mean,
                  const float* std, float* y, void* stream);

int ea_specaug(int B, int T, int F, const float* x, const long long* lengths, const int* warp, int per_utt,
               const int* fmask, int nf, const int* tmask, int nt, float* y, void* stream);

int ea_subsample_lens(int B, int T, const long long* ilens, long long* olens, void* stream);

int ea_add_sos_eos(int B, int L, const long long* ys, long ldys, const long long* ylens, int sos,
                   int eos, int ignore_id, long long* ys_in, long long* ys_out,
                   long long* ys_in_lens, void* stream);

int ea_scale_dropout(long rows, int cols, const void* x, int x_dtype, long ldx, void* y,
                     int y_dtype, long ldy, float scale, float p, unsigned long long seed,
                     void* stream);

int ea_scale_dropout_colsum(long rows, int cols, const float* x, long ldx, void* y, int y_dtype, long ldy,
                            float scale, float p, unsigned long long seed, float* colsum, int accumulate,
                            float* workspace, long ws_elems, void* stream);

int ea_add_2d(long rows, int cols, const void* x, int x_dtype, long ldx, void* y, int y_dtype,
              long ldy, float alpha, void* stream);

int ea_permute3(int A, int Bd, int Cd, const void* src, int src_dtype, void* dst, int dst_dtype,
                int accumulate, void* stream);

int ea_im2col_conv1(int B, int T, int F, const float* x, void* col, int col_dtype, void* stream);
int ea_im2col_conv2(int B, int T1, int F1, int C, const void* x1, void* col, int dtype, void* stream);
int ea_col2im_conv2(int B, int T1, int F1, int C, const void* dcol, int dcol_dtype, const void* x1,
                    void* dx1, int dtype, void* stream);

int ea_conv1_fwd(int B, int T, int F, int C, const float* x, const float* w, const float* bias,
                 void* x1p, int dtype, void* stream);
int ea_conv1_fwd2(int B, int T, int F, int C, const float* x, const float* w, const float* bias,
                  void* x1p, int dtype, unsigned char* pos, void* stream);
int ea_conv1_wgrad(int B, int T, int F, int C, const float* x, const void* dh, int dtype, float* dw,
                   float* dbias, float* workspace, long ws_elems, void* stream);

int ea_glu_fwd(long rows, int C, const void* x, int x_dtype, void* y, int y_dtype, void* stream);
int ea_glu_bwd(long rows, int C, const void* x, int x_dtype, const float* dy, void* dx, void* stream);

int ea_dwconv_fwd(int B, int T, int C, int K, const float* x, const float* w, const float* bias,
                  float* y, void* stream);
int ea_dwconv_bwd(int B, int T, int C, int K, const float* x, const float* w, const float* dy,
                  float* dx, float* dw, float* dbias, int accumulate_params, float* workspace,
                  long ws_elems, void* stream);
int ea_dwconv_glu_bwd(int B, int T, int C, int K, const float* x, const float* w, const float* dy,
                      const void* g2, void* dg2, float* dw, float* dbias, int accumulate_params,
                      float* workspace, long ws_elems, void* stream);
int ea_dwconv_fwd_glu(int B, int T, int C, int K, const void* g2, const float* w, const float* bias,
                      float* y, void* stream);
int ea_dwconv_fwd_glu_stats(int B, int T, int C, int K, const void* g2, const float* w, const float* bias,
                            float* y, float* part, void* stream);
int ea_dwconv_stats_parts(int B, int T, int* nparts);
int ea_add_pos_bias(long N, int H, int dk, const void* q, long ldq, const float* u, const float* v,
                    void* qu, void* qv, int dtype, void* stream);

int ea_embed_fwd(long rows, int d, int L, const long long* tok, const float* E, float xscale,
                 const float* pe, float p, unsigned long long seed, float* y, void* stream);
int ea_add_pe_dropout(long rows, int d, int L, const float* pe, float p, unsigned long long seed, float* y,
                      void* stream);
int ea_embed_bwd(long rows, int d, const long long* tok, const float* dy, float xscale, float p,
                 unsigned long long seed, float* dE, void* stream);

int ea_set_rng_salt(const unsigned long long* salt);
int ea_rng_advance(unsigned long long* salt, void* stream);

int ea_argmax_rows(long rows, int V, const float* x, long ld, long long* out, void* stream);


int ea_attn_softmax_fwd(int B, int H, int T1, int T2, float scale, const float* S, long ldS,
                        const float* BD, long ldBD, const long long* klen, int causal, float p,
                        unsigned long long seed, float* P, long ldP, void* Pd, int pd_dtype,
                        long ldPd, void* stream);

int ea_attn_softmax_bwd(int B, int H, int T1, int T2, float scale, const float* dPd, long ldd,
                        const float* P, long ldP, float p, unsigned long long seed, void* dS,
                        int ds_dtype, long ldS, void* dBD, long ldBD, void* stream);

enum { EA_REL_LATEST = 0, EA_REL_LEGACY = 1 };
int ea_attn_softmax_fwd_mode(int B, int H, int T1, int T2, float scale, const float* S, long ldS,
                             const float* BD, long ldBD, const long long* klen, int causal, float p,
                             unsigned long long seed, float* P, long ldP, void* Pd, int pd_dtype,
                             long ldPd, int rel_mode, void* stream);
int ea_attn_softmax_bwd_mode(int B, int H, int T1, int T2, float scale, const float* dPd, long ldd,
                             const float* P, long ldP, float p, unsigned long long seed, void* dS,
                             int ds_dtype, long ldS, void* dBD, long ldBD, int rel_mode, void* stream);
int ea_legacy_pext(int T, int d, const void* p, long ldp, void* pext, long ldx, int dtype, void* stream);
int ea_legacy_pext_fold(int T, int d, const void* dpext, long ldx, void* dp, long ldp, int dtype,
                        void* stream);

int ea_attn_fused_fwd(int B, int H, int T1, int T2, int dk, const void* q, long ldq, const void* k,
                      long ldk, const void* v, long ldv, const float* bu, const float* bv,
                      const void* pp, long ldp, const long long* klen, int causal, float scale, float p,
                      unsigned long long seed, void* o, long ldo, float* lse, void* stream);
int ea_attn_fused_fwd2(int B, int H, int T1, int T2, int dk, const void* q, long ldq, const void* k,
                       long ldk, const void* v, long ldv, const float* bu, const float* bv,
                       const void* pp, long ldp, const long long* klen, int causal, float scale, float p,
                       unsigned long long seed, void* o, long ldo, float* lse, unsigned* dmask, int ldm,
                       void* stream);
int ea_attn_fused_fwd2_mode(int B, int H, int T1, int T2, int dk, const void* q, long ldq, const void* k,
                            long ldk, const void* v, long ldv, const float* bu, const float* bv,
                            const void* pp, long ldp, const long long* klen, int causal, float scale,
                            float p, unsigned long long seed, void* o, long ldo, float* lse,
                            unsigned* dmask, int ldm, int rel_mode, void* stream);
int ea_attn_fused_bwd_ws_bytes(int B, int H, int T1, long* bytes);
int ea_attn_dbd_layout(int T1, int* shift, long* lddbd);
int ea_attn_fused_bwd2(int B, int H, int T1, int T2, int dk, const void* q, long ldq, const void* k,
                       long ldk, const void* v, long ldv, const float* bu, const float* bv,
                       const void* pp, long ldp, const long long* klen, int causal, float scale, float p,
                       unsigned long long seed, const void* o, long ldo, const float* lse, const void* dO,
                       long lddo, void* dq, long lddq, void* dkout, long lddk, void* dvout, long lddv,
                       void* dbd, long lddbd, float* bias_part, long ldpart, void* qv_out, long ldqv,
                       const unsigned* dmask, int ldm, void* ws, long ws_bytes, int flags, void* stream);
int ea_attn_fused_bwd2_mode(int B, int H, int T1, int T2, int dk, const void* q, long ldq, const void* k,
                       long ldk, const void* v, long ldv, const float* bu, const float* bv,
                       const void* pp, long ldp, const long long* klen, int causal, float scale, float p,
                       unsigned long long seed, const void* o, long ldo, const float* lse, const void* dO,
                       long lddo, void* dq, long lddq, void* dkout, long lddk, void* dvout, long lddv,
                       void* dbd, long lddbd, float* bias_part, long ldpart, void* qv_out, long ldqv,
                       const unsigned* dmask, int ldm, void* ws, long ws_bytes, int flags, int rel_mode, void* stream);
int ea_attn_legacy_band(long nhb, int T1, const void* dbd, void* out, long lddbd, void* stream);


int ea_ctc_loss_fwd(int B, int T, int V, const float* logits, long ldt, const long long* hlens,
                    const long long* ys, long ldys, const long long* ylens, int Lmax, float* lse,
                    double* alpha, double* beta, double* nll, float* loss_utt, float* loss,
                    void* stream);

int ea_ctc_loss_bwd(int B, int T, int V, const float* logits, long ldt, const long long* hlens,
                    const long long* ys, long ldys, const long long* ylens, int Lmax, const float* lse,
                    const double* alpha, const double* beta, const double* nll,
                    const float* gscale, float coef, void* grad, int grad_dtype, long ldg,
                    void* stream);

int ea_softmax_lse_rows(long rows, int V, const float* logits, long ld, float* lse, void* probs,
                        int probs_dtype, long ldp, void* stream);

int ea_ctc_loss_fwd_lse(int B, int T, int V, const float* logits, long ldt, const long long* hlens,
                        const long long* ys, long ldys, const long long* ylens, int Lmax,
                        const float* lse, double* alpha, double* beta, double* nll, float* loss_utt,
                        float* loss, void* stream);

int ea_interctc_dlogits(int B, int T, int V, const float* logits, long ldt, const long long* hlens,
                        const long long* ys, long ldys, const long long* ylens, int Lmax,
                        const float* lse, const double* alpha, const double* beta, const double* nll,
                        const float* gscale, float coef, const void* dp, long lddp, void* grad,
                        int grad_dtype, long ldg, void* stream);

int ea_lsm_loss_fwd(long rows, int V, const float* x, long ldx, const long long* tgt, float smoothing,
                    int ignore_id, int normalize_length, float batch, float* lse, double* loss_row,
                    int* stat, float* loss, float* acc, float* inv_denom, void* stream);
int ea_lsm_loss_bwd(long rows, int V, const float* x, long ldx, const long long* tgt, float smoothing,
                    int ignore_id, const float* lse, const float* gscale, const float* inv_denom,
                    float coef, void* grad, int grad_dtype, long ldg, void* stream);


int ea_sqnorm(long n, const float* x, double* workspace, float* norm, void* stream);

int ea_adam_step(long n, float* params, const float* grads, float* exp_avg, float* exp_avg_sq,
                 void* params_bf16, float lr, float beta1, float beta2, float eps, float weight_decay,
                 long step, const float* grad_norm, float max_norm, void* stream);

enum { EA_SCHED_CONSTANT = 0, EA_SCHED_WARMUP = 1 };
typedef struct ea_lr_schedule {
  int kind;
  float warmup_steps;
  double base_lr;
} ea_lr_schedule;
typedef struct ea_opt_state {
  long long step;
  float lr;
  float bc1, bc2_sqrt;
  float coef;
  float last_norm;
  int skip;
  float next_lr;
  int pad;
} ea_opt_state;
int ea_adam_step_dev(long n, float* params, const float* grads, float* exp_avg, float* exp_avg_sq,
                     void* params_bf16, const ea_lr_schedule* sched, float beta1, float beta2, float eps,
                     float weight_decay, ea_opt_state* state, const float* grad_norm, float max_norm,
                     void* stream);

int ea_cast_f32_bf16(long n, const float* x, void* y, void* stream);
int ea_relu_f32_inplace(long n, float* x, void* stream);
int ea_transpose_bf16_grouped(int ntiles, const int* tiles, const void* probs, const void* src, void* stream);
int ea_scale_by_scalar(long n, float* x, const float* s, float c, void* stream);
int ea_axpy_dev(long n, const float* x, float* y, const float* s, float c, void* stream);
int ea_axpby_scalar(const float* a, float wa, const float* b, float wb, float* out, void* stream);



int ea_softmax_rows(long rows, int V, const float* logits, long ld, float* out, int log, void* stream);

int ea_ctc_prefix_init(int T, int V, const float* logits, long ld_logits, int blank, float* logp,
                       float* r0, void* stream);

int ea_ctc_prefix_score(int T, int V, int blank, int eos, int n_hyp, int n_cand, const float* logp,
                        const unsigned long long* r_prev, const int* meta, float* log_psi, float* r_new,
                        void* stream);

int ea_ctc_prefix_score_dev(int T, int V, int blank, int eos, int n_hyp, int n_cand, const float* logp,
                            const unsigned long long* r_prev, int out_len, const int* last, const int* cand,
                            float* log_psi, float* r_new, void* stream);

int ea_ctc_prefix_score_win(int T, int V, int blank, int eos, int n_hyp, int n_cand, const float* logp,
                            const unsigned long long* r_prev, const int* meta, int start, int end,
                            float* log_psi, float* r_new, void* stream);
// ... 50 lines not shown
```

Baseline: 1880 utterances/s.

## Fuse bias-gradient column sums into grouped weight-gradient GEMM via MFMA row sums

Bias gradients were computed by separate colsum kernels before each deferred weight-gradient GEMM. The grouped wgrad kernel now computes the A-operand row sums itself: in the first N-tile of each M-block it issues extra MFMA ops against a ones vector and writes the bias gradient. This removes a separate pass over dy for every linear layer. In exchange it adds MFMA work in those tiles, new overlap checks and flush logic between the colsum and wgrad queues, and a smaller chunk size for the argument upload.

```diff
diff --git a/espnet-1_amd/csrc/gemm_grouped.hip b/espnet-1_amd/csrc/gemm_grouped.hip
--- a/espnet-1_amd/csrc/gemm_grouped.hip
+++ b/espnet-1_amd/csrc/gemm_grouped.hip
@@ -9,8 +9,9 @@
   int M, N, K;
   int tiles_n, tile0;
   float beta;
+  float* a_sum;
 };
-constexpr int EA_GROUP_CHUNK = 60;
+constexpr int EA_GROUP_CHUNK = 55;
 struct GroupChunk {
   int first, n;
   GroupProbD pr[EA_GROUP_CHUNK];
@@ -64,7 +65,25 @@
   for (int i = 0; i < 8; ++i)
 #pragma unroll
     for (int j = 0; j < 4; ++j) acc[i][j] = (f32x4){0.f, 0.f, 0.f, 0.f};
-  pipe_tile<AK, BKM, 0, 256, NS>(p, tile_ov(p), smem, q.A, q.B, m0, n0, 0, q.K, acc);
+  if (q.a_sum != nullptr && tn == 0) {
+    f32x4 asum[2] = {(f32x4){0.f, 0.f, 0.f, 0.f}, (f32x4){0.f, 0.f, 0.f, 0.f}};
+    pipe_tile<AK, BKM, 0, 256, NS, true>(p, tile_ov(p), smem, q.A, q.B, m0, n0, 0, q.K, acc, asum);
+    if ((lane & 15) == 0) {
+#pragma unroll
+      for (int e = 0; e < 2; ++e)
+#pragma unroll
+        for (int r = 0; r < 4; ++r) {
+          const int m = m0 + wm + ((w & 3) * 2 + e) * 16 + (lane >> 4) * 4 + r;
+          if (m < q.M) {
+            float v = asum[e][r];
+            if (q.beta != 0.f) v += q.beta * q.a_sum[m];
+            q.a_sum[m] = v;
+          }
+        }
+    }
+  } else {
+    pipe_tile<AK, BKM, 0, 256, NS>(p, tile_ov(p), smem, q.A, q.B, m0, n0, 0, q.K, acc);
+  }
   const EpiK ek = make_epik(p);
   epi_wave<EA_EPI_STORE, 8, 4>(p, ek, smem, 0, 0, 0, m0 + wm, n0 + wn, lane, w, acc);
 }
@@ -106,6 +125,20 @@
     const double b_ext = 2.0 * ((b_kmajor ? (double)e.N : (double)e.K) * e.ldb);
     EA_CHECK_ARG(a_ext < 4.0e9 && b_ext < 4.0e9);
     ntiles += (long)ea_cdiv(e.M, 256) * ea_cdiv(e.N, 256);
+    if (e.a_sum) {
+      EA_CHECK_ARG(((uintptr_t)e.a_sum % 4) == 0);
+      const uintptr_t lo = (uintptr_t)e.a_sum, hi = lo + 4 * (uintptr_t)e.M;
+      for (int j = 0; j < n; ++j) {
+        const ea_group_gemm& o = probs[j];
+        if (!o.C || o.M <= 0 || o.N <= 0) continue;
+        const uintptr_t clo = (uintptr_t)o.C, chi = clo + 4 * ((uintptr_t)(o.M - 1) * o.ldc + o.N);
+        EA_CHECK_ARG(!(lo < chi && clo < hi));
+        if (j != i && o.a_sum) {
+          const uintptr_t slo = (uintptr_t)o.a_sum;
+          EA_CHECK_ARG(!(lo < slo + 4 * (uintptr_t)o.M && slo < hi));
+        }
+      }
+    }
   }
   EA_CHECK_ARG(ntiles < (1L << 30) && grouped_ws_bytes(n, ntiles) <= ws_bytes);
   GroupProbD* table = (GroupProbD*)ws;
@@ -121,6 +154,7 @@
     d.tiles_n = ea_cdiv(e.N, 256);
     d.tile0 = tile0;
     d.beta = e.beta;
+    d.a_sum = e.a_sum;
     tile0 += ea_cdiv(e.M, 256) * d.tiles_n;
     if (c.n == EA_GROUP_CHUNK || i == n - 1) {
       hipLaunchKernelGGL(group_upload, dim3(1), dim3(256), 0, st, c, table, map);
diff --git a/espnet-1_amd/csrc/gemm_kern.h b/espnet-1_amd/csrc/gemm_kern.h
--- a/espnet-1_amd/csrc/gemm_kern.h
+++ b/espnet-1_amd/csrc/gemm_kern.h
@@ -1190,12 +1190,13 @@
 };
 EA_DEV TileOv tile_ov(const GemmP& p) { return TileOv{p.M, p.g.a, p.g.e, p.w1part, p.w1pos}; }
 
-template <bool AK, bool BKM, int MODE = 0, int BT = 256, int NS = 4>
+template <bool AK, bool BKM, int MODE = 0, int BT = 256, int NS = 4, bool ASUM = false>
 EA_DEV void pipe_tile(const GemmP& p, const TileOv& ov, char* smem, const bf16* A, const bf16* B, int m0, int n0, int kbeg,
-                      int kend, f32x4 (&acc)[PipeT<BT, NS>::MI][4]) {
+                      int kend, f32x4 (&acc)[PipeT<BT, NS>::MI][4], f32x4* asum = nullptr) {
   static_assert(MODE == 0 || (MODE == EA_CONV_FWD && AK && BKM) || (MODE == EA_CONV_DGRAD && AK) ||
                 (MODE == EA_CONV_WGRAD && !AK && !BKM), "conv gather layouts");
   static_assert(MODE == 0 || BT == 256, "conv gathers run on 256-wide tiles");
+  static_assert(!ASUM || (MODE == 0 && BT == 256), "A row sums: plain 256-wide tiles");
   using PC = PipeT<BT, NS>;
   constexpr int BK = PC::BK, NSLOT = PC::NSLOT, NW = PC::NW, NTT = PC::NTT, MI = PC::MI;
   constexpr int A_BYTES = PC::A_BYTES, B_BYTES = PC::B_BYTES, SLOT = PC::SLOT;
@@ -1356,6 +1357,19 @@
   lds_barrier();
   if (g1) lds_barrier();
   bf16x8 fa[MI], fb[4];
+  auto a_rowsum = [&]() {
+    if constexpr (ASUM) {
+      const int sj = w & 3;
+      bf16x8 ones;
+#pragma unroll
+      for (int e = 0; e < 8; ++e) ones[e] = (bf16)1.f;
+      auto pick = [](bool c, bf16x8 a, bf16x8 b) { return c ? a : b; };
+      const bf16x8 s0 = pick(sj == 0, fa[0], pick(sj == 1, fa[2], pick(sj == 2, fa[4], fa[6])));
+      const bf16x8 s1 = pick(sj == 0, fa[1], pick(sj == 1, fa[3], pick(sj == 2, fa[5], fa[7])));
+      asum[0] = __builtin_amdgcn_mfma_f32_16x16x32_bf16(s0, ones, asum[0], 0, 0, 0);
+      asum[1] = __builtin_amdgcn_mfma_f32_16x16x32_bf16(s1, ones, asum[1], 0, 0, 0);
+    }
+  };
   for (int sl = 0; sl < nsl; ++sl) {
     __builtin_amdgcn_sched_barrier(0);
     rd_b(sl, fb);
@@ -1379,6 +1393,7 @@
 #pragma unroll
       for (int j = 0; j < 4; ++j)
         acc[i][j] = __builtin_amdgcn_mfma_f32_16x16x32_bf16(fa[i], fb[j], acc[i][j], 0, 0, 0);
+    a_rowsum();
     __builtin_amdgcn_s_setprio(0);
     __builtin_amdgcn_sched_barrier(0);
     lds_barrier();
@@ -1428,6 +1443,7 @@
 #pragma unroll
       for (int j = 0; j < 4; ++j)
         acc[i][j] = __builtin_amdgcn_mfma_f32_16x16x32_bf16(fa[i], fb[j], acc[i][j], 0, 0, 0);
+    a_rowsum();
   }
 
   __syncthreads();
diff --git a/espnet-1_amd/espnet_amd/deferred.py b/espnet-1_amd/espnet_amd/deferred.py
--- a/espnet-1_amd/espnet_amd/deferred.py
+++ b/espnet-1_amd/espnet_amd/deferred.py
@@ -12,6 +12,7 @@
 GRAD_READY = None
 
 DEFER_WGRAD = os.environ.get("EA_DEFER_WGRAD", "1") != "0"
+WGRAD_BIAS = os.environ.get("EA_WGRAD_BIAS", "1") != "0"
 DEFER_BUDGET = int(float(os.environ.get("EA_DEFER_BUDGET_MB", "8192")) * 2 ** 20)
 
 
@@ -28,7 +29,7 @@
         self.pending = 0
         self.side_events = []
 
-    def add(self, dy, x, dw, *, M, N, K, lda, ldb, ldc, beta, post=None) -> bool:
+    def add(self, dy, x, dw, *, M, N, K, lda, ldb, ldc, beta, post=None, db=None, db_beta=None):
         if not (dy.dtype == torch.bfloat16 and x.dtype == torch.bfloat16 and dw.dtype == torch.float32):
             return False
         if (lda % 8 or ldb % 8 or dy.data_ptr() % 16 or x.data_ptr() % 16 or N % 4 or ldc % 4
@@ -38,19 +39,30 @@
             return False
         lo = dw.data_ptr()
         hi = lo + ((M - 1) * ldc + N) * 4
-        if any(lo < it[-1] and it[-2] < hi for it in self.items):
+        spans = [(lo, hi)]
+        if (db is not None and WGRAD_BIAS and db_beta == beta and db.dtype == torch.float32 and db.is_contiguous()
+                and db.numel() == M and db.data_ptr() % 4 == 0):
+            blo = db.data_ptr()
+            bhi = blo + 4 * M
+            if not (blo < hi and lo < bhi) and not REDUCE_Q.claimed(blo, bhi):
+                spans.append((blo, bhi))
+        if any(l_ < s[1] and s[0] < h for it in self.items for s in it[-1] for l_, h in spans):
             self.flush()
         if on_side():
             ev = torch.cuda.Event()
             ev.record()
             self.side_events.append(ev)
-        self.items.append((K, dy, x, dw, M, N, lda, ldb, ldc, beta, lo, hi))
+        fused = db if len(spans) > 1 else None
+        self.items.append((K, dy, x, dw, M, N, lda, ldb, ldc, beta, fused, spans))
         if post is not None:
             self.posts.append(post)
         self.pending += _nbytes(dy) + _nbytes(x)
         if self.pending > DEFER_BUDGET:
             self.flush()
-        return True
+        return "db" if fused is not None else True
+
+    def carries(self, lo, hi) -> bool:
+        return any(lo < s[1] and s[0] < hi for it in self.items for s in it[-1][1:])
 
     def flush(self):
         if not self.items:
@@ -73,8 +85,9 @@
                 t.record_stream(cur)
         arr = (GroupGemm * n)()
         ntiles = 0
-        for i, (K, dy, x, dw, M, N, lda, ldb, ldc, beta, _, _) in enumerate(items):
-            arr[i] = GroupGemm(dy.data_ptr(), x.data_ptr(), dw.data_ptr(), lda, ldb, ldc, M, N, K, beta)
+        for i, (K, dy, x, dw, M, N, lda, ldb, ldc, beta, db, _) in enumerate(items):
+            arr[i] = GroupGemm(dy.data_ptr(), x.data_ptr(), dw.data_ptr(), lda, ldb, ldc, M, N, K, beta,
+                               None if db is None else db.data_ptr())
             ntiles += ((M + 255) // 256) * ((N + 255) // 256)
         nbytes = ctypes.c_long(0)
         lib.ea_gemm_grouped_ws_bytes(n, ntiles, ctypes.addressof(nbytes))
@@ -106,11 +119,16 @@
         if self.pending > DEFER_BUDGET:
             self.flush()
 
+    def claimed(self, lo, hi) -> bool:
+        return any(lo < h and l_ < hi for l_, h in self.spans)
+
     def _claim(self, out, n):
         lo = out.data_ptr()
         hi = lo + 4 * n
-        if any(lo < h and l_ < hi for l_, h in self.spans):
-            self.flush()
+        if self.claimed(lo, hi):
+            self.flush()
+        if WGRAD_Q.carries(lo, hi):
+            WGRAD_Q.flush()
         self.spans.append((lo, hi))
 
     def add_colsum(self, x, rows, n, ld, out, accumulate) -> bool:
diff --git a/espnet-1_amd/espnet_amd/hip_ops.py b/espnet-1_amd/espnet_amd/hip_ops.py
--- a/espnet-1_amd/espnet_amd/hip_ops.py
+++ b/espnet-1_amd/espnet_amd/hip_ops.py
@@ -274,14 +274,17 @@
                 ldc=ldc, epi=epi)
 
 
-def linear_dw(dy, x, dw, *, accumulate=False, post=None):
+def linear_dw(dy, x, dw, *, accumulate=False, post=None, db=None, db_accumulate=True):
     R, N, lddy = _rows(dy)
     R2, K, ldx = _rows(x)
     if R != R2:
         raise HipError("row mismatch in linear_dw")
     beta = 1.0 if accumulate else 0.0
-    if WGRAD_Q.active and WGRAD_Q.add(dy, x, dw, M=N, N=K, K=R, lda=lddy, ldb=ldx, ldc=dw.stride(0), beta=beta,
-                                      post=post):
+    took = WGRAD_Q.active and WGRAD_Q.add(dy, x, dw, M=N, N=K, K=R, lda=lddy, ldb=ldx, ldc=dw.stride(0), beta=beta,
+                                          post=post, db=db, db_beta=1.0 if db_accumulate else 0.0)
+    if db is not None and took != "db":
+        colsum(dy, db, accumulate=db_accumulate)
+    if took:
         return dw
     gemm(dy, x, dw, M=N, N=K, K=R, a_kmajor=0, b_kmajor=0, lda=lddy, ldb=ldx,
          ldc=dw.stride(0), epi=make_epi(beta=beta))
diff --git a/espnet-1_amd/espnet_amd/layers/conformer.py b/espnet-1_amd/espnet_amd/layers/conformer.py
--- a/espnet-1_amd/espnet_amd/layers/conformer.py
+++ b/espnet-1_amd/espnet_amd/layers/conformer.py
@@ -145,8 +145,8 @@
     ops.linear_dx(dv, b.w(pre + ".w_2.weight"), dh,
                   epi=ops.make_epi(EPI_DACT, act=ACT_SWISH, aux=h, drop_p=p, seed=seed_in))
     with ops.wgrad(dh, xn):
-        ops.colsum(dh, b.g(pre + ".w_1.bias"))
-        ops.linear_dw(dh, xn, b.g(pre + ".w_1.weight"), accumulate=True)
+        ops.linear_dw(dh, xn, b.g(pre + ".w_1.weight"), accumulate=True,
+                      db=b.g(pre + ".w_1.bias"))
     dxn = empty(N, d, dtype=cd, device=dx.device)
     ops.linear_dx(dh, b.w(pre + ".w_1.weight"), dxn)
     ln_bwd(dxn, x_in, b, ln_name, mu, rs, dx, accumulate=True, drop=next_drop)
@@ -326,8 +326,8 @@
                               b.g(C + "depthwise_conv.bias").data_ptr(), 1, w, wn, ops.stream())
             lib.ea_glu_bwd(N, d, g2.data_ptr(), ops.dt(g2), dglu.data_ptr(), dg2.data_ptr(), ops.stream())
         with ops.wgrad(dg2, xn3):
-            ops.colsum(dg2, b.g(C + "pointwise_conv1.bias"))
-            ops.linear_dw(dg2, xn3, b.g(C + "pointwise_conv1.weight", shape=(2 * d, d)), accumulate=True)
+            ops.linear_dw(dg2, xn3, b.g(C + "pointwise_conv1.weight", shape=(2 * d, d)), accumulate=True,
+                          db=b.g(C + "pointwise_conv1.bias"))
         dxn3 = empty(N, d, dtype=cd, device=dev)
         ops.linear_dx(dg2, b.w(C + "pointwise_conv1.weight", shape=(2 * d, d)), dxn3)
         dv_att = dv_buf(N, d, cd, dev)
@@ -403,9 +403,9 @@
         if fork is None:
             dpp_wgrad()
         with ops.wgrad(dqkv, xn2):
-            ops.colsum(dqkv, b.g(A + "linear_q.bias", A + "linear_k.bias", A + "linear_v.bias", shape=(3 * d,)))
             ops.linear_dw(dqkv, xn2, b.g(A + "linear_q.weight", A + "linear_k.weight", A + "linear_v.weight",
-                                          shape=(3 * d, d)), accumulate=True)
+                                          shape=(3 * d, d)), accumulate=True,
+                          db=b.g(A + "linear_q.bias", A + "linear_k.bias", A + "linear_v.bias", shape=(3 * d,)))
         dxn2 = empty(N, d, dtype=cd, device=dev)
         ops.linear_dx(dqkv, qkv_w, dxn2)
         if fork is not None:
diff --git a/espnet-1_amd/espnet_amd/layers/decoder.py b/espnet-1_amd/espnet_amd/layers/decoder.py
--- a/espnet-1_amd/espnet_amd/layers/decoder.py
+++ b/espnet-1_amd/espnet_amd/layers/decoder.py
@@ -202,8 +202,8 @@
         dev = dlogits.device
         dlog = ops.cast(dlogits.reshape(N, V).contiguous(), cd)
         with ops.wgrad(dlog, xf):
-            ops.colsum(dlog, b.g("output_layer.bias"))
-            ops.linear_dw(dlog, xf, b.g("output_layer.weight"), accumulate=True)
+            ops.linear_dw(dlog, xf, b.g("output_layer.weight"), accumulate=True,
+                          db=b.g("output_layer.bias"))
         dxf = empty(N, d, dtype=cd, device=dev)
         ops.linear_dx(dlog, b.w("output_layer.weight"), dxf)
         dx = empty(N, d, device=dev)
@@ -228,8 +228,8 @@
             if fork is not None:
                 ops.flush_wgrad_side(after=fork)
             with ops.wgrad(dh, xn3):
-                ops.colsum(dh, b.g(ff + "w_1.bias"))
-                ops.linear_dw(dh, xn3, b.g(ff + "w_1.weight"), accumulate=True)
+                ops.linear_dw(dh, xn3, b.g(ff + "w_1.weight"), accumulate=True,
+                              db=b.g(ff + "w_1.bias"))
             dxn = empty(N, d, dtype=cd, device=dev)
             ops.linear_dx(dh, b.w(ff + "w_1.weight"), dxn)
             dv_src = dv_buf(N, d, cd, dev)
@@ -247,8 +247,8 @@
                      seed=sd(l, 3), cd=cd, dq=dq, lddq=d, dk_=dkv[:, 2 * d * l:], lddk=ldkv,
                      dv=dkv[:, 2 * d * l + d:], lddv=ldkv)
             with ops.wgrad(dq, xn2):
-                ops.colsum(dq, b.g(xa + "linear_q.bias"))
-                ops.linear_dw(dq, xn2, b.g(xa + "linear_q.weight"), accumulate=True)
+                ops.linear_dw(dq, xn2, b.g(xa + "linear_q.weight"), accumulate=True,
+                              db=b.g(xa + "linear_q.bias"))
             dxn = empty(N, d, dtype=cd, device=dev)
             ops.linear_dx(dq, b.w(xa + "linear_q.weight"), dxn)
             dv_self = dv_buf(N, d, cd, dev)
@@ -268,8 +268,8 @@
             wn = (sa + "linear_q.weight", sa + "linear_k.weight", sa + "linear_v.weight")
             bn = (sa + "linear_q.bias", sa + "linear_k.bias", sa + "linear_v.bias")
             with ops.wgrad(dqkv, xn1):
-                ops.colsum(dqkv, b.g(*bn, shape=(3 * d,)))
-                ops.linear_dw(dqkv, xn1, b.g(*wn, shape=(3 * d, d)), accumulate=True)
+                ops.linear_dw(dqkv, xn1, b.g(*wn, shape=(3 * d, d)), accumulate=True,
+                              db=b.g(*bn, shape=(3 * d,)))
             dxn = empty(N, d, dtype=cd, device=dev)
             ops.linear_dx(dqkv, b.w(*wn, shape=(3 * d, d)), dxn)
             dv_ff = dv_buf(N, d, cd, dev) if l > 0 else None
@@ -281,8 +281,8 @@
                          b.g("embed.0.weight").data_ptr(), ops.stream())
         kvw, kvb = _kv_names(nb)
         with ops.wgrad(dkv, mem):
-            ops.colsum(dkv, b.g(*kvb, shape=(ldkv,)))
-            ops.linear_dw(dkv, mem, b.g(*kvw, shape=(ldkv, d)), accumulate=True)
+            ops.linear_dw(dkv, mem, b.g(*kvw, shape=(ldkv, d)), accumulate=True,
+                          db=b.g(*kvb, shape=(ldkv,)))
         dmem = empty(Nm, d, device=dev)
         ops.linear_dx(dkv, b.w(*kvw, shape=(ldkv, d)), dmem)
         ops.grad_ready(b)
diff --git a/espnet-1_amd/espnet_amd/layers/ebranchformer.py b/espnet-1_amd/espnet_amd/layers/ebranchformer.py
--- a/espnet-1_amd/espnet_amd/layers/ebranchformer.py
+++ b/espnet-1_amd/espnet_amd/layers/ebranchformer.py
@@ -176,9 +176,9 @@
     if fork is None:
         dpp_wgrad()
     with ops.wgrad(dqkv, xn):
-        ops.colsum(dqkv, b.g(A + "linear_q.bias", A + "linear_k.bias", A + "linear_v.bias", shape=(3 * d,)))
         ops.linear_dw(dqkv, xn, b.g(A + "linear_q.weight", A + "linear_k.weight", A + "linear_v.weight",
-                                    shape=(3 * d, d)), accumulate=True)
+                                    shape=(3 * d, d)), accumulate=True,
+                      db=b.g(A + "linear_q.bias", A + "linear_k.bias", A + "linear_v.bias", shape=(3 * d,)))
     dxn = empty(N, d, dtype=cd, device=dev)
     ops.linear_dx(dqkv, qkv_w, dxn)
     if fork is not None:
@@ -289,8 +289,8 @@
         xnm, mum, rsm, h, gmu, grs, gout = s_mlp
         dv2 = dxc[:, d:]
         with ops.wgrad(dxc, gout):
-            ops.colsum(dv2, b.g(G + "channel_proj2.bias"))
-            ops.linear_dw(dv2, gout, b.g(G + "channel_proj2.weight"), accumulate=True)
+            ops.linear_dw(dv2, gout, b.g(G + "channel_proj2.weight"), accumulate=True,
+                          db=b.g(G + "channel_proj2.bias"))
         dgout = empty(N, C, dtype=cd, device=dev)
         ops.linear_dx(dv2, b.w(G + "channel_proj2.weight"), dgout)
         n_dln, n_ws = _long(), _long()
@@ -307,16 +307,16 @@
                         dln.data_ptr(), w, wn, ops.stream())
         del dln, dgout
         with ops.wgrad(dh, xnm):
-            ops.colsum(dh, b.g(G + "channel_proj1.0.bias"))
-            ops.linear_dw(dh, xnm, b.g(G + "channel_proj1.0.weight"), accumulate=True)
+            ops.linear_dw(dh, xnm, b.g(G + "channel_proj1.0.weight"), accumulate=True,
+                          db=b.g(G + "channel_proj1.0.bias"))
         dxnm = empty(N, d, dtype=cd, device=dev)
         ops.linear_dx(dh, b.w(G + "channel_proj1.0.weight"), dxnm)
         ln_bwd(dxnm, x1, b, "norm_mlp", mum, rsm, dx, accumulate=True)
         xna, mua, rsa, O, s_core = s_att
         dv1 = dxc[:, :d]
         with ops.wgrad(dxc, O):
-            ops.colsum(dv1, b.g("attn.linear_out.bias"))
-            ops.linear_dw(dv1, O, b.g("attn.linear_out.weight"), accumulate=True)
+            ops.linear_dw(dv1, O, b.g("attn.linear_out.weight"), accumulate=True,
+                          db=b.g("attn.linear_out.bias"))
         dO = empty(N, d, dtype=cd, device=dev)
         ops.linear_dx(dv1, b.w("attn.linear_out.weight"), dO)
         dxna = _attn_bwd(L, b, dO, xna, O, s_core, pos, olens, B, T, pa, sd(3))
diff --git a/espnet-1_amd/espnet_amd/layers/interctc.py b/espnet-1_amd/espnet_amd/layers/interctc.py
--- a/espnet-1_amd/espnet_amd/layers/interctc.py
+++ b/espnet-1_amd/espnet_amd/layers/interctc.py
@@ -85,8 +85,8 @@
             be = enc.conditioning_layer._b
             dxc = ops.cast(dxo, cd)
             with ops.wgrad(dxc, p):
-                ops.colsum(dxc, be.g("bias"))
-                ops.linear_dw(dxc, p, be.g("weight"), accumulate=True)
+                ops.linear_dw(dxc, p, be.g("weight"), accumulate=True,
+                              db=be.g("bias"))
             dp = empty(N, V, dtype=cd, device=dev)
             ops.linear_dx(dxc, be.w("weight"), dp)
         if lat is None and dp is None:
@@ -105,8 +105,8 @@
             lib.ea_interctc_dlogits(B, T, V, logits.data_ptr(), V, None, None, 0, None, 0, lse.data_ptr(), None, None,
                                     None, None, 0.0, dp.data_ptr(), V, dl.data_ptr(), ops.dt(dl), V, ops.stream())
         with ops.wgrad(dl, h):
-            ops.colsum(dl, bc.g("ctc_lo.bias"))
-            ops.linear_dw(dl, h, bc.g("ctc_lo.weight"), accumulate=True)
+            ops.linear_dw(dl, h, bc.g("ctc_lo.weight"), accumulate=True,
+                          db=bc.g("ctc_lo.bias"))
         dy = empty(N, d, device=dev)
         ops.linear_dx(dl, bc.w("ctc_lo.weight"), dy)
         dx = dxo.clone()
diff --git a/espnet-1_amd/espnet_amd/layers/losses.py b/espnet-1_amd/espnet_amd/layers/losses.py
--- a/espnet-1_amd/espnet_amd/layers/losses.py
+++ b/espnet-1_amd/espnet_amd/layers/losses.py
@@ -114,8 +114,8 @@
                                 nll.data_ptr(), gl.data_ptr(), 1.0 / B, dl.data_ptr(), ops.dt(dl), V,
                                 ops.stream())
             with ops.wgrad(dl, h):
-                ops.colsum(dl, b.g("ctc_lo.bias"))
-                ops.linear_dw(dl, h, b.g("ctc_lo.weight"), accumulate=True)
+                ops.linear_dw(dl, h, b.g("ctc_lo.weight"), accumulate=True,
+                              db=b.g("ctc_lo.bias"))
             ops.linear_dx(dl, b.w("ctc_lo.weight"), dh)
             if ctc.dropout_rate > 0:
                 ops.scale_dropout(dh, dh, p=ctc.dropout_rate, seed=ctc._seed)
diff --git a/espnet-1_amd/espnet_amd/layers/transformer.py b/espnet-1_amd/espnet_amd/layers/transformer.py
--- a/espnet-1_amd/espnet_amd/layers/transformer.py
+++ b/espnet-1_amd/espnet_amd/layers/transformer.py
@@ -105,8 +105,8 @@
         ops.linear_dx(dv, b.w("feed_forward.w_2.weight"), dh,
                       epi=ops.make_epi(EPI_DACT, act=ACT_RELU, aux=h, drop_p=p_ff, seed=sd(3)))
         with ops.wgrad(dh, xn2):
-            ops.colsum(dh, b.g("feed_forward.w_1.bias"))
-            ops.linear_dw(dh, xn2, b.g("feed_forward.w_1.weight"), accumulate=True)
+            ops.linear_dw(dh, xn2, b.g("feed_forward.w_1.weight"), accumulate=True,
+                          db=b.g("feed_forward.w_1.bias"))
         dxn = empty(N, d, dtype=cd, device=dev)
         ops.linear_dx(dh, b.w("feed_forward.w_1.weight"), dxn)
         ln_bwd(dxn, x1, b, "norm2", mu2, rs2, dx, accumulate=True)
@@ -121,8 +121,8 @@
                  ldv=3 * d, klen=olens, causal=getattr(L, "causal", False), scale=scale, p=pa, seed=sd(1), cd=cd, dq=dqkv, lddq=3 * d,
                  dk_=dqkv[:, d:], lddk=3 * d, dv=dqkv[:, 2 * d:], lddv=3 * d)
         with ops.wgrad(dqkv, xn1):
-            ops.colsum(dqkv, b.g(*_QKV_B, shape=(3 * d,)))
-            ops.linear_dw(dqkv, xn1, b.g(*_QKV_W, shape=(3 * d, d)), accumulate=True)
+            ops.linear_dw(dqkv, xn1, b.g(*_QKV_W, shape=(3 * d, d)), accumulate=True,
+                          db=b.g(*_QKV_B, shape=(3 * d,)))
         dxn = empty(N, d, dtype=cd, device=dev)
         ops.linear_dx(dqkv, b.w(*_QKV_W, shape=(3 * d, d)), dxn)
         ln_bwd(dxn, x0, b, "norm1", mu1, rs1, dx, accumulate=True)
diff --git a/include/espnet_amd.h b/include/espnet_amd.h
--- a/include/espnet_amd.h
+++ b/include/espnet_amd.h
@@ -73,6 +73,7 @@
   long lda, ldb, ldc;
   int M, N, K;
   float beta;
+  float* a_sum;
 } ea_group_gemm;
 int ea_gemm_grouped(int a_kmajor, int b_kmajor, int n, const ea_group_gemm* probs, void* ws, long ws_bytes,
                     void* stream);
```

Result: faster. 1901 utterances/s, median of 6 (+1.1%).
